# aliftffd/ViT-vs-Raw-IQ

Measured on AMD Instinct MI355X. Metric: IQ frames/sec training (fwd+loss+bwd+clip+AdamW), higher is better.
Workload: dtype bf16; 1 GPU; ViT-Tiny/16 224x224 C=1 19cls (BASELINE configs[1]); config_id=B, per_gpu_batch=256, global_batch=256, parallelism=dp1, hipgraph=True

## Files before the change

### include/iqvit.h

```cpp
#ifndef IQVIT_H
#define IQVIT_H
#include <stddef.h>
#include <stdint.h>

#ifdef __cplusplus
extern "C" {
#endif

typedef void* iq_stream_t;

enum { IQ_STATUS_OK = 0, IQ_STATUS_ARG = 1, IQ_STATUS_UNSUPPORTED = 2, IQ_STATUS_LAUNCH = 3 };

typedef struct iq_dropout {
  uint64_t seed;
  uint32_t step;
  uint32_t site;
  float p;
  const uint32_t* step_dev;
} iq_dropout_t;

int iq_ln_supported(int D);
int iq_ln_fwd(const void* z, const float* gamma, const float* beta, void* x, float* mean, float* rstd, int M, int D,
              float eps, iq_stream_t stream);
size_t iq_ln_bwd_ws_bytes(int D);
int iq_ln_bwd(const void* dx, const void* z, const float* mean, const float* rstd, const float* gamma, void* dz,
              void* dy, const iq_dropout_t* drop, float* dgamma, float* dbeta, float* ws, int accumulate, int M,
              int D, iq_stream_t stream);
int iq_ln_bwd_partial_rows(int M, int D);

typedef struct iq_epilogue {
  const float* bias;
  int relu;
  const float* pe;
  int tok, seq, cls_off;
  iq_dropout_t drop;
  const void* gate;
  int ldg;
  float gate_scale;
  const void* residual;
  int ldr;
} iq_epilogue_t;
int iq_gemm_bf16_nt(const void* A, int lda, const void* B, int ldb, void* C, int ldc, int M, int N, int K,
                    const iq_epilogue_t* epi, iq_stream_t stream);

int iq_gemm_ln_supported(int D, int K);
int iq_gemm_bf16_ln(const void* A, int lda, const void* W, int ldw, const float* bias, const void* residual, int ldr,
                    const iq_dropout_t* drop, const float* gamma, const float* beta, float eps, void* Z, void* X,
                    float* mean, float* rstd, int M, int D, int K, iq_stream_t stream);

int iq_gemm_lnbwd_supported(int D, int K);
int iq_gemm_lnbwd_partial_rows(int M);
int iq_gemm_bf16_lnbwd(const void* A, int lda, const void* Wt, int ldw, const void* residual, int ldr, const void* z,
                       const float* mean, const float* rstd, const float* gamma, const iq_dropout_t* drop, void* dz,
                       void* dy, float* partial, int M, int D, int K, iq_stream_t stream);

int iq_ffn_chain_supported(int S, int D, int F);
int iq_ffn_chain_bwd_partial_rows(int M);
size_t iq_ffn_chain_gate_bytes(int M, int F);
int iq_ffn_chain_bwd(const void* dO, const void* W2t, const void* gate_bits, float gate_scale, void* gH, const void* W1t,
                     const void* residual, const void* z1, const float* mean, const float* rstd, const float* gamma,
                     const iq_dropout_t* drop, void* dz, void* dy, float* partial, const void* Wot, void* dA, int frames, int S,
                     int D, int F, iq_stream_t stream);
int iq_qkv_dgrad_ffn_chain_bwd(const void* gQKV, const void* Wqkv_t, const void* residual0, const void* z2, const float* mean2,
                               const float* rstd2, const float* gamma2, const iq_dropout_t* drop2, void* dz2, void* dy2, float* partial2,
                               const void* W2t, const void* gate_bits, float gate_scale, void* gH, const void* W1t, const void* residual,
                               const void* z1, const float* mean, const float* rstd, const float* gamma, const iq_dropout_t* drop, void* dz,
                               void* dy, float* partial, const void* Wot, void* dA, int frames, int S, int D, int F, iq_stream_t stream);
int iq_ffn_chain_fwd(const void* X1, const void* W1, const float* b1, const iq_dropout_t* drop1, void* H, const void* W2,
                     const float* b2, const iq_dropout_t* drop2, const float* gamma, const float* beta, float eps, void* Z,
                     void* X, float* mean, float* rstd, void* gate_bits, int frames, int S, int D, int F, iq_stream_t stream);
int iq_attn_out_ffn_chain_fwd(const void* A, const void* Wo, const float* bo, const iq_dropout_t* drop0, const void* R,
                              const float* gamma1, const float* beta1, void* Z1, void* X1, float* mean1, float* rstd1,
                              const void* W1, const float* b1, const iq_dropout_t* drop1, void* H, const void* W2, const float* b2,
                              const iq_dropout_t* drop2, const float* gamma2, const float* beta2, float eps, void* Z2, void* X,
                              float* mean2, float* rstd2, void* gate_bits, const void* Wq, const float* bq, void* Yq, int frames,
                              int S, int D, int F, iq_stream_t stream);

size_t iq_wgrad_ws_bytes(int M, int N, int K);
int iq_gemm_bf16_wgrad(const void* dY, int ldy, const void* X, int ldx, float* dW, float* dbias, int M, int N, int K,
                       float* ws, size_t ws_bytes, int accumulate, iq_stream_t stream);

typedef struct iq_wgrad_problem {
  const void* dY;
  int ldy;
  const void* X;
  int ldx;
  float* dW;
  float* dbias;
  int N, K;
} iq_wgrad_problem_t;
typedef struct iq_reduce_seg {
  const float* partials;
  int rows;
  int64_t row_stride;
  float* out;
  int64_t n;
} iq_reduce_seg_t;
size_t iq_wgrad_grouped_ws_bytes(const iq_wgrad_problem_t* probs, int nprob, int M, int max_workgroups);
int iq_gemm_bf16_wgrad_grouped(const iq_wgrad_problem_t* probs, int nprob, int M, float* ws, size_t ws_bytes,
                               int accumulate, int max_workgroups, const iq_reduce_seg_t* extra, int nextra,
                               iq_stream_t stream);

int iq_attn_supported(int S, int dh);
int iq_attn_fwd(const void* qkv, void* out, float* lse, int B, int S, int H, int dh, iq_stream_t stream);
int iq_attn_bwd(const void* qkv, const void* out, const void* dout, const float* lse, void* dqkv, int B, int S, int H,
                int dh, iq_stream_t stream);
int iq_attn_fwd_masked(const void* qkv, void* out, float* lse, const uint8_t* mask, long mask_hstride, int B, int S,
                       int H, int dh, iq_stream_t stream);
int iq_attn_bwd_masked(const void* qkv, const void* out, const void* dout, const float* lse, void* dqkv,
                       const uint8_t* mask, long mask_hstride, int B, int S, int H, int dh, iq_stream_t stream);
int iq_attn_probs(const void* qkv, const float* lse, float* out, long out_bstride, int B, int S, int H, int dh,
                  int rows, int heads, iq_stream_t stream);
int iq_attn_grad_probs(const void* qkv, const float* lse, const void* dout, float* out, long out_bstride, int B, int S,
                       int H, int dh, int rows, int heads, int positive, iq_stream_t stream);
int iq_attn_relevance_step(const void* qkv, const float* lse, const void* dout, const float* r_in, float* r_out, int B,
                           int S, int H, int dh, iq_stream_t stream);

int iq_frames_preprocess(const float* raw, float* out, int n_frames, int len, int take, const float* stats,
                         iq_stream_t stream);
int iq_patchify(const float* src, void* patches, int kind, int B, int C, int H, int W, int p, int Kpad,
                iq_stream_t stream);
int iq_cls_rows(const float* cls, const float* pe, void* x0, int B, int S, int D, const iq_dropout_t* drop,
                iq_stream_t stream);
int iq_embed_bwd_gather(const void* dx0, void* demb, float* dcls, int B, int S, int tok, int D, int has_cls,
                        const iq_dropout_t* drop, int accumulate, iq_stream_t stream);
int iq_embed_dgrad(const void* demb, const void* w_bf16, int Kpad, float* dsrc, int kind, int B, int C, int H, int W, int p,
                   int D, iq_stream_t stream);
int iq_linf_step(float* x_adv, const float* grad, const float* x0, float alpha, float eps, float lo, float hi, size_t n,
                 iq_stream_t stream);

int iq_head_fwd(const void* x, const float* ln_g, const float* ln_b, const float* W, const float* b, float* featn,
                float* hstat, float* logits, int B, int S, int D, int K, int pool, iq_stream_t stream);
int iq_ce_fwd_bwd(const float* logits, const int64_t* labels, int B, int K, float smoothing, float denom,
                  float* loss_sum, int32_t* n_correct, float* dlogits, iq_stream_t stream);
int iq_head_bwd(const float* dlogits, const float* featn, const float* hstat, const float* ln_g, const float* ln_b,
                const float* W, float* dW, float* db, float* dln_g, float* dln_b, void* dx, int B, int S, int D, int K,
                int pool, int accumulate, iq_stream_t stream);

size_t iq_gradnorm_ws_bytes(size_t n);
int iq_gradnorm_sq(const float* g, size_t n, float grad_scale, float* ws, float* out, iq_stream_t stream);
int iq_adamw_step(float* p, const float* g, float* m, float* v, void* shadow_bf16, size_t n, float lr, float beta1,
                  float beta2, float eps, float weight_decay, int step, const float* gnorm_sq, float max_norm,
                  float grad_scale, const float* dyn, iq_stream_t stream);
int iq_counter_add(uint32_t* ctr_u32, uint32_t inc_u32, float* ctr_f32, float inc_f32, iq_stream_t stream);
int iq_cast_bf16(const float* src, void* dst, size_t n, iq_stream_t stream);
int iq_transpose_cast_bf16(const float* src, void* dst, int rows, int cols, iq_stream_t stream);

typedef struct iq_model_cfg {
  int kind;
  int in_channels;
  int img_h, img_w, patch;
  int seq_length, conv_k, use_cls;
  int num_classes, d_model, n_head, n_layers, ffn_hidden;
  float drop_prob;
} iq_model_cfg_t;

typedef struct iq_model iq_model_t;

int iq_model_create(const iq_model_cfg_t* cfg, iq_model_t** out);
void iq_model_destroy(iq_model_t* m);
const char* iq_model_last_error(const iq_model_t* m);
int iq_model_tokens(const iq_model_t* m);
size_t iq_model_param_floats(const iq_model_t* m);
int iq_model_param_entries(const iq_model_t* m);
int iq_model_param_entry(const iq_model_t* m, int i, char* name, int name_cap, size_t* offset, int* ndim, int* dims);
size_t iq_model_shadow_bytes(const iq_model_t* m);
size_t iq_model_workspace_bytes(const iq_model_t* m, int batch, int training);
int iq_model_bind(iq_model_t* m, float* params, float* grads, const float* pe, void* shadow);
int iq_model_bind_step_counter(iq_model_t* m, uint32_t* counter);
int iq_model_refresh_shadow(iq_model_t* m, iq_stream_t stream);
int iq_model_refresh_transposed(iq_model_t* m, iq_stream_t stream);
int iq_model_forward(iq_model_t* m, const float* src, int batch, void* workspace, size_t ws_bytes, int training,
                     uint64_t seed, uint32_t step, float* enc_out, float* logits, iq_stream_t stream);
int iq_model_backward(iq_model_t* m, const float* dlogits, const float* denc, int batch, void* workspace,
                      size_t ws_bytes, int accumulate, int stage_hi, int stage_lo, iq_stream_t stream);
int iq_model_grad_range(const iq_model_t* m, int stage_hi, int stage_lo, size_t* off, size_t* len);
#define IQ_BWD_PARAM_GRADS 1
int iq_model_backward_input(iq_model_t* m, const float* dlogits, const float* denc, int batch, void* workspace,
                            size_t ws_bytes, float* dsrc, int flags, iq_stream_t stream);
int iq_model_attention(iq_model_t* m, const void* workspace, size_t ws_bytes, int batch, int layer, int rows,
                       int heads, float* out, long out_bstride, iq_stream_t stream);
int iq_model_attention_rollout(iq_model_t* m, const void* workspace, size_t ws_bytes, int batch, float alpha,
                               float* out, iq_stream_t stream);
int iq_model_attention_relevance(iq_model_t* m, const float* dlogits, int batch, void* workspace, size_t ws_bytes,
                                 float* rel, float* const* maps, int rows, int heads, int positive, long out_bstride,
                                 iq_stream_t stream);

#define IQ_PROF_FAMILIES 8
int iq_prof_enable(int on);
int iq_prof_collect(double* ms, long long* count);
size_t iq_prof_kernels(char* out, size_t cap, int reset);

#ifdef __cplusplus
}
#endif
#endif
```

### vit-vs-raw-iq_amd/_native.py

```python
from __future__ import annotations

import ctypes as C
import os

_HERE = os.path.dirname(os.path.abspath(__file__))
LIB_PATH = os.environ.get("IQ_LIBIQVIT") or os.path.join(_HERE, "libiqvit.so")

BWD_PARAM_GRADS = 1

STATUS = {0: "ok", 1: "invalid argument", 2: "unsupported shape/configuration", 3: "HIP launch error"}


class IqError(RuntimeError):
    pass


class Dropout(C.Structure):
    _fields_ = [("seed", C.c_uint64), ("step", C.c_uint32), ("site", C.c_uint32), ("p", C.c_float),
                ("step_dev", C.c_void_p)]


class Epilogue(C.Structure):
    _fields_ = [("bias", C.c_void_p), ("relu", C.c_int), ("pe", C.c_void_p), ("tok", C.c_int), ("seq", C.c_int),
                ("cls_off", C.c_int), ("drop", Dropout), ("gate", C.c_void_p), ("ldg", C.c_int),
                ("gate_scale", C.c_float), ("residual", C.c_void_p), ("ldr", C.c_int)]


class WgradProblem(C.Structure):
    _fields_ = [("dY", C.c_void_p), ("ldy", C.c_int), ("X", C.c_void_p), ("ldx", C.c_int), ("dW", C.c_void_p),
                ("dbias", C.c_void_p), ("N", C.c_int), ("K", C.c_int)]


class ReduceSeg(C.Structure):
    _fields_ = [("partials", C.c_void_p), ("rows", C.c_int), ("row_stride", C.c_int64), ("out", C.c_void_p),
                ("n", C.c_int64)]


class ModelCfg(C.Structure):
    _fields_ = [("kind", C.c_int), ("in_channels", C.c_int), ("img_h", C.c_int), ("img_w", C.c_int),
                ("patch", C.c_int), ("seq_length", C.c_int), ("conv_k", C.c_int), ("use_cls", C.c_int),
                ("num_classes", C.c_int), ("d_model", C.c_int), ("n_head", C.c_int), ("n_layers", C.c_int),
                ("ffn_hidden", C.c_int), ("drop_prob", C.c_float)]


_P, _I, _Z, _F = C.c_void_p, C.c_int, C.c_size_t, C.c_float
_U64, _U32 = C.c_uint64, C.c_uint32

SIGNATURES = {
    "iq_ln_supported": (_I, [_I]),
    "iq_ln_fwd": (_I, [_P, _P, _P, _P, _P, _P, _I, _I, _F, _P]),
    "iq_ln_bwd_ws_bytes": (_Z, [_I]),
    "iq_ln_bwd_partial_rows": (_I, [_I, _I]),
    "iq_ln_bwd": (_I, [_P, _P, _P, _P, _P, _P, _P, C.POINTER(Dropout), _P, _P, _P, _I, _I, _I, _P]),
    "iq_gemm_bf16_nt": (_I, [_P, _I, _P, _I, _P, _I, _I, _I, _I, C.POINTER(Epilogue), _P]),
    "iq_gemm_ln_supported": (_I, [_I, _I]),
    "iq_gemm_bf16_ln": (_I, [_P, _I, _P, _I, _P, _P, _I, C.POINTER(Dropout), _P, _P, _F, _P, _P, _P, _P, _I, _I, _I, _P]),
    "iq_gemm_lnbwd_supported": (_I, [_I, _I]),
    "iq_gemm_lnbwd_partial_rows": (_I, [_I]),
    "iq_gemm_bf16_lnbwd": (_I, [_P, _I, _P, _I, _P, _I, _P, _P, _P, _P, C.POINTER(Dropout), _P, _P, _P, _I, _I, _I, _P]),
    "iq_ffn_chain_supported": (_I, [_I, _I, _I]),
    "iq_ffn_chain_bwd_partial_rows": (_I, [_I]),
    "iq_ffn_chain_bwd": (_I, [_P, _P, _P, _F, _P, _P, _P, _P, _P, _P, _P, C.POINTER(Dropout), _P, _P, _P, _P, _P, _I, _I, _I, _I, _P]),
    "iq_qkv_dgrad_ffn_chain_bwd": (_I, [_P, _P, _P, _P, _P, _P, _P, C.POINTER(Dropout), _P, _P, _P,
                                        _P, _P, _F, _P, _P, _P, _P, _P, _P, _P, C.POINTER(Dropout), _P, _P, _P, _P, _P, _I, _I, _I, _I, _P]),
    "iq_ffn_chain_gate_bytes": (_Z, [_I, _I]),
    "iq_ffn_chain_fwd": (_I, [_P, _P, _P, C.POINTER(Dropout), _P, _P, _P, C.POINTER(Dropout), _P, _P, _F, _P, _P, _P, _P, _P, _I, _I,
                              _I, _I, _P]),
    "iq_attn_out_ffn_chain_fwd": (_I, [_P, _P, _P, C.POINTER(Dropout), _P, _P, _P, _P, _P, _P, _P,
                                       _P, _P, C.POINTER(Dropout), _P, _P, _P, C.POINTER(Dropout), _P, _P, _F, _P, _P, _P, _P, _P,
                                       _P, _P, _P, _I, _I, _I, _I, _P]),
    "iq_wgrad_ws_bytes": (_Z, [_I, _I, _I]),
    "iq_gemm_bf16_wgrad": (_I, [_P, _I, _P, _I, _P, _P, _I, _I, _I, _P, _Z, _I, _P]),
    "iq_wgrad_grouped_ws_bytes": (_Z, [_P, _I, _I, _I]),
    "iq_gemm_bf16_wgrad_grouped": (_I, [_P, _I, _I, _P, _Z, _I, _I, _P, _I, _P]),
    "iq_attn_supported": (_I, [_I, _I]),
    "iq_attn_fwd": (_I, [_P, _P, _P, _I, _I, _I, _I, _P]),
    "iq_attn_bwd": (_I, [_P, _P, _P, _P, _P, _I, _I, _I, _I, _P]),
    "iq_attn_fwd_masked": (_I, [_P, _P, _P, _P, C.c_long, _I, _I, _I, _I, _P]),
    "iq_attn_bwd_masked": (_I, [_P, _P, _P, _P, _P, _P, C.c_long, _I, _I, _I, _I, _P]),
    "iq_attn_probs": (_I, [_P, _P, _P, C.c_long, _I, _I, _I, _I, _I, _I, _P]),
    "iq_attn_grad_probs": (_I, [_P, _P, _P, _P, C.c_long, _I, _I, _I, _I, _I, _I, _I, _P]),
    "iq_attn_relevance_step": (_I, [_P, _P, _P, _P, _P, _I, _I, _I, _I, _P]),
    "iq_frames_preprocess": (_I, [_P, _P, _I, _I, _I, C.POINTER(C.c_float), _P]),
    "iq_patchify": (_I, [_P, _P, _I, _I, _I, _I, _I, _I, _I, _P]),
    "iq_cls_rows": (_I, [_P, _P, _P, _I, _I, _I, C.POINTER(Dropout), _P]),
    "iq_embed_bwd_gather": (_I, [_P, _P, _P, _I, _I, _I, _I, _I, C.POINTER(Dropout), _I, _P]),
    "iq_embed_dgrad": (_I, [_P, _P, _I, _P, _I, _I, _I, _I, _I, _I, _I, _P]),
    "iq_linf_step": (_I, [_P, _P, _P, _F, _F, _F, _F, _Z, _P]),
    "iq_head_fwd": (_I, [_P, _P, _P, _P, _P, _P, _P, _P, _I, _I, _I, _I, _I, _P]),
    "iq_ce_fwd_bwd": (_I, [_P, _P, _I, _I, _F, _F, _P, _P, _P, _P]),
    "iq_head_bwd": (_I, [_P, _P, _P, _P, _P, _P, _P, _P, _P, _P, _P, _I, _I, _I, _I, _I, _I, _P]),
    "iq_gradnorm_ws_bytes": (_Z, [_Z]),
    "iq_gradnorm_sq": (_I, [_P, _Z, _F, _P, _P, _P]),
    "iq_adamw_step": (_I, [_P, _P, _P, _P, _P, _Z, _F, _F, _F, _F, _F, _I, _P, _F, _F, _P, _P]),
    "iq_counter_add": (_I, [_P, _U32, _P, _F, _P]),
    "iq_cast_bf16": (_I, [_P, _P, _Z, _P]),
    "iq_transpose_cast_bf16": (_I, [_P, _P, _I, _I, _P]),
    "iq_model_create": (_I, [C.POINTER(ModelCfg), C.POINTER(_P)]),
    "iq_model_destroy": (None, [_P]),
    "iq_model_last_error": (C.c_char_p, [_P]),
    "iq_model_tokens": (_I, [_P]),
    "iq_model_param_floats": (_Z, [_P]),
    "iq_model_param_entries": (_I, [_P]),
    "iq_model_param_entry": (_I, [_P, _I, C.c_char_p, _I, C.POINTER(_Z), C.POINTER(_I), C.POINTER(_I)]),
    "iq_model_shadow_bytes": (_Z, [_P]),
    "iq_model_workspace_bytes": (_Z, [_P, _I, _I]),
    "iq_model_bind": (_I, [_P, _P, _P, _P, _P]),
    "iq_model_bind_step_counter": (_I, [_P, _P]),
    "iq_model_refresh_shadow": (_I, [_P, _P]),
    "iq_model_refresh_transposed": (_I, [_P, _P]),
    "iq_model_forward": (_I, [_P, _P, _I, _P, _Z, _I, _U64, _U32, _P, _P, _P]),
    "iq_model_backward": (_I, [_P, _P, _P, _I, _P, _Z, _I, _I, _I, _P]),
    "iq_model_grad_range": (_I, [_P, _I, _I, C.POINTER(_Z), C.POINTER(_Z)]),
    "iq_model_backward_input": (_I, [_P, _P, _P, _I, _P, _Z, _P, _I, _P]),
    "iq_model_attention": (_I, [_P, _P, _Z, _I, _I, _I, _I, _P, C.c_long, _P]),
    "iq_model_attention_rollout": (_I, [_P, _P, _Z, _I, _F, _P, _P]),
    "iq_model_attention_relevance": (_I, [_P, _P, _I, _P, _Z, _P, C.POINTER(_P), _I, _I, _I, C.c_long, _P]),
    "iq_prof_enable": (_I, [_I]),
    "iq_prof_collect": (_I, [C.POINTER(C.c_double), C.POINTER(C.c_longlong)]),
    "iq_prof_kernels": (_Z, [C.c_char_p, _Z, _I]),
}

_lib = None


def lib():
    global _lib
    if _lib is None:
        if not os.path.exists(LIB_PATH):
            raise IqError(
                f"{LIB_PATH} not found: the HIP extension is not built. Run "
                "`python -c 'import __graft_entry__ as g; g.build()'` (or `make -C vit-vs-raw-iq_amd/csrc`). "
                "There is no CPU fallback.")
        L = C.CDLL(LIB_PATH)
        for name, (res, args) in SIGNATURES.items():
            fn = getattr(L, name)
            fn.restype = res
            fn.argtypes = args
        _lib = L
    return _lib


def check(rc, what, model=None):
    if rc != 0:
        detail = ""
        if model is not None:
            msg = lib().iq_model_last_error(model)
            if msg:
                detail = ": " + msg.decode()
        raise IqError(f"{what} failed: {STATUS.get(rc, rc)}{detail}")


def ptr(t):
    return None if t is None else t.data_ptr()


def stream_handle():
    import torch
    return torch.cuda.current_stream().cuda_stream
```

### vit-vs-raw-iq_amd/csrc/common.h

```cpp
#pragma once
#include <hip/hip_runtime.h>
#include <stdint.h>

typedef __bf16 bf16;
typedef __attribute__((ext_vector_type(8))) __bf16 bf16x8;
typedef __attribute__((ext_vector_type(4))) __bf16 bf16x4;
typedef __attribute__((ext_vector_type(4))) short s16x4;
typedef __attribute__((ext_vector_type(8))) short s16x8;
typedef __attribute__((ext_vector_type(4))) float f32x4;
typedef __attribute__((ext_vector_type(4))) uint32_t u32x4;

#define IQ_OK 0
#define IQ_ERR_ARG 1
#define IQ_ERR_UNSUPPORTED 2
#define IQ_ERR_LAUNCH 3

#define IQ_WAVE 64

static inline int iq_launch_status() {
  hipError_t e = hipGetLastError();
  return e == hipSuccess ? IQ_OK : IQ_ERR_LAUNCH;
}

__device__ __forceinline__ float bf2f(bf16 v) { return (float)v; }
__device__ __forceinline__ bf16 f2bf(float v) { return (bf16)v; }

__device__ __forceinline__ void unpack8(const bf16x8& v, float* f) {
#pragma unroll
  for (int i = 0; i < 8; ++i) f[i] = (float)v[i];
}
__device__ __forceinline__ bf16x8 pack8(const float* f) {
  bf16x8 v;
#pragma unroll
  for (int i = 0; i < 8; ++i) v[i] = (bf16)f[i];
  return v;
}

struct IqRng {
  uint64_t seed;
  uint32_t step;
  uint32_t site;
  const uint32_t* step_dev;
};

__device__ __forceinline__ IqRng rng_resolve(IqRng r) {
  if (r.step_dev) r.step = *r.step_dev;
  return r;
}

#ifndef IQ_PHILOX_ROUNDS
#define IQ_PHILOX_ROUNDS 7
#endif
__device__ __forceinline__ u32x4 philox4x32(uint32_t c0, uint32_t c1, uint32_t c2, uint32_t c3,
                                            uint32_t k0, uint32_t k1) {
  const uint32_t M0 = 0xD2511F53u, M1 = 0xCD9E8D57u, W0 = 0x9E3779B9u, W1 = 0xBB67AE85u;
#pragma unroll
  for (int r = 0; r < IQ_PHILOX_ROUNDS; ++r) {
    const uint64_t p0 = (uint64_t)M0 * (uint64_t)c0;
    const uint64_t p1 = (uint64_t)M1 * (uint64_t)c2;
    const uint32_t n0 = (uint32_t)(p1 >> 32) ^ c1 ^ k0, n1 = (uint32_t)p1;
    const uint32_t n2 = (uint32_t)(p0 >> 32) ^ c3 ^ k1, n3 = (uint32_t)p0;
    c0 = n0; c1 = n1; c2 = n2; c3 = n3;
    k0 += W0; k1 += W1;
  }
  u32x4 o = {c0, c1, c2, c3};
  return o;
}

__device__ __forceinline__ uint32_t dropout_keep8(const IqRng& r, uint64_t group, uint32_t thresh) {
  u32x4 b = philox4x32((uint32_t)group, (uint32_t)(group >> 32), r.site, r.step,
                          (uint32_t)r.seed, (uint32_t)(r.seed >> 32));
  uint32_t m = 0;
#pragma unroll
  for (int i = 0; i < 4; ++i) {
    m |= ((b[i] & 0xFFFFu) >= thresh ? 1u : 0u) << (2 * i);
    m |= ((b[i] >> 16) >= thresh ? 1u : 0u) << (2 * i + 1);
  }
  return m;
}

__host__ __device__ inline uint32_t dropout_thresh(float p) {
  float t = p * 65536.0f + 0.5f;
  if (t < 0.f) t = 0.f;
  if (t > 65535.f) t = 65535.f;
  return (uint32_t)t;
}
__host__ __device__ inline float dropout_scale(float p) {
  uint32_t t = dropout_thresh(p);
  return 65536.0f / (65536.0f - (float)t);
}

__device__ __forceinline__ int xcd_remap(int bid, int nwg) {
  const int NX = 8;
  int q = nwg / NX, r = nwg % NX;
  int xcd = bid % NX, idx = bid / NX;
  int base = (xcd < r) ? xcd * (q + 1) : r * (q + 1) + (xcd - r) * q;
  return base + idx;
}

__device__ __forceinline__ float wave_sum(float v) {
#pragma unroll
  for (int o = 32; o > 0; o >>= 1) v += __shfl_xor(v, o, 64);
  return v;
}
__device__ __forceinline__ float wave_max(float v) {
#pragma unroll
  for (int o = 32; o > 0; o >>= 1) v = fmaxf(v, __shfl_xor(v, o, 64));
  return v;
}
```

### vit-vs-raw-iq_amd/csrc/misc.hip

```cpp
#include "common.h"
#include "iqvit.h"
#include "prof.h"

namespace {

__global__ void patchify_kernel(const float* __restrict__ src, bf16* __restrict__ dst, int kind, int B, int C, int H,
                                int W, int p, int tok, int P, int Kpad) {
  const long nchunk = (long)B * tok * (Kpad / 8);
  for (long id = (long)blockIdx.x * blockDim.x + threadIdx.x; id < nchunk; id += (long)gridDim.x * blockDim.x) {
    const int ch = (int)(id % (Kpad / 8));
    const long row = id / (Kpad / 8);
    const int b = (int)(row / tok), t = (int)(row % tok);
    float v[8];
    if (kind == 0 && (p & 7) == 0 && (W & 3) == 0 && ch * 8 < P) {
      const int k = ch * 8, gw = W / p;
      const int c = k / (p * p), rem = k % (p * p), py = rem / p, px = rem % p;
      const int gy = t / gw, gx = t % gw;
      const float* sp = src + (((long)b * C + c) * H + gy * p + py) * W + gx * p + px;
      const f32x4 a = *reinterpret_cast<const f32x4*>(sp), bq = *reinterpret_cast<const f32x4*>(sp + 4);
      v[0] = a[0]; v[1] = a[1]; v[2] = a[2]; v[3] = a[3]; v[4] = bq[0]; v[5] = bq[1]; v[6] = bq[2]; v[7] = bq[3];
      *reinterpret_cast<bf16x8*>(dst + row * Kpad + ch * 8) = pack8(v);
      continue;
    }
#pragma unroll
    for (int e = 0; e < 8; ++e) {
      const int k = ch * 8 + e;
      float x = 0.f;
      if (k < P) {
        if (kind == 0) {
          const int gw = W / p;
          const int c = k / (p * p), rem = k % (p * p), py = rem / p, px = rem % p;
          const int gy = t / gw, gx = t % gw;
          x = src[(((long)b * C + c) * H + gy * p + py) * W + gx * p + px];
        } else {
          const int c = k / p, j = k % p;
          x = src[((long)b * C + c) * H + (long)t * p + j];
        }
      }
      v[e] = x;
    }
    *reinterpret_cast<bf16x8*>(dst + row * Kpad + ch * 8) = pack8(v);
  }
}

__global__ void cls_rows_kernel(const float* __restrict__ cls, const float* __restrict__ pe, bf16* __restrict__ x0,
                                int B, int S, int D, int drop_on, IqRng rng, uint32_t thresh, float dscale) {
  const int nch = D / 8;
  const int id = blockIdx.x * blockDim.x + threadIdx.x;
  if (id >= B * nch) return;
  if (drop_on) rng = rng_resolve(rng);
  const int b = id / nch, ch = id % nch;
  float v[8];
#pragma unroll
  for (int e = 0; e < 8; ++e) v[e] = cls[ch * 8 + e] + pe[ch * 8 + e];
  const long off = (long)b * S * D + ch * 8;
  if (drop_on) {
    const uint32_t keep = dropout_keep8(rng, (uint64_t)off >> 3, thresh);
#pragma unroll
    for (int e = 0; e < 8; ++e) v[e] = ((keep >> e) & 1u) ? v[e] * dscale : 0.f;
  }
  *reinterpret_cast<bf16x8*>(x0 + off) = pack8(v);
}

__global__ void embed_bwd_gather_kernel(const bf16* __restrict__ dx0, bf16* __restrict__ demb, int B, int S, int tok,
                                        int D, int cls_off, int drop_on, IqRng rng, uint32_t thresh, float dscale) {
  const int nch = D / 8;
  const long n = (long)B * tok * nch;
  if (drop_on) rng = rng_resolve(rng);
  for (long id = (long)blockIdx.x * blockDim.x + threadIdx.x; id < n; id += (long)gridDim.x * blockDim.x) {
    const int ch = (int)(id % nch);
    const long row = id / nch;
    const int b = (int)(row / tok), t = (int)(row % tok);
    const long off = ((long)b * S + cls_off + t) * D + ch * 8;
    bf16x8 v = *reinterpret_cast<const bf16x8*>(dx0 + off);
    if (drop_on) {
      const uint32_t keep = dropout_keep8(rng, (uint64_t)off >> 3, thresh);
      float f[8];
      unpack8(v, f);
#pragma unroll
      for (int e = 0; e < 8; ++e) f[e] = ((keep >> e) & 1u) ? f[e] * dscale : 0.f;
      v = pack8(f);
    }
    *reinterpret_cast<bf16x8*>(demb + row * D + ch * 8) = v;
  }
}

__global__ __launch_bounds__(256) void dcls_kernel(const bf16* __restrict__ dx0, float* __restrict__ dcls, int B, int S, int D,
                                                   int drop_on, IqRng rng, uint32_t thresh, float dscale, int accumulate) {
  __shared__ float part[4][8];
  const int ch = blockIdx.x, lane = threadIdx.x & 63, wave = threadIdx.x >> 6;
  if (drop_on) rng = rng_resolve(rng);
  float s[8] = {0.f, 0.f, 0.f, 0.f, 0.f, 0.f, 0.f, 0.f};
  for (int b = threadIdx.x; b < B; b += 256) {
    const long off = (long)b * S * D + ch * 8;
    float v[8];
    unpack8(*reinterpret_cast<const bf16x8*>(dx0 + off), v);
    uint32_t keep = 0xffu;
    if (drop_on) keep = dropout_keep8(rng, (uint64_t)off >> 3, thresh);
#pragma unroll
    for (int e = 0; e < 8; ++e) s[e] += ((keep >> e) & 1u) ? (drop_on ? v[e] * dscale : v[e]) : 0.f;
  }
#pragma unroll
  for (int e = 0; e < 8; ++e) {
    const float t = wave_sum(s[e]);
    if (lane == 0) part[wave][e] = t;
  }
  __syncthreads();
  if (threadIdx.x < 8) {
    const float t = part[0][threadIdx.x] + part[1][threadIdx.x] + part[2][threadIdx.x] + part[3][threadIdx.x];
    float* dst = dcls + ch * 8 + threadIdx.x;
    *dst = accumulate ? *dst + t : t;
  }
}

__global__ __launch_bounds__(64) void head_fwd_kernel(const bf16* __restrict__ x, const float* __restrict__ ln_g,
                                                      const float* __restrict__ ln_b, const float* __restrict__ W,
                                                      const float* __restrict__ bias, float* __restrict__ feat_hat,
                                                      float* __restrict__ hstat, float* __restrict__ logits, int S,
                                                      int D, int K, int pool) {
  const int b = blockIdx.x, lane = threadIdx.x;
  const bf16* xb = x + (long)b * S * D;
  float* fh = feat_hat + (long)b * D;
  float s1 = 0.f;
  for (int d = lane; d < D; d += 64) {
    float f;
    if (pool == 0) {
      f = (float)xb[d];
    } else {
      f = 0.f;
      for (int s = 0; s < S; ++s) f += (float)xb[(long)s * D + d];
      f /= (float)S;
    }
    fh[d] = f;
    s1 += f;
  }
  if (ln_g) {
    const float mean = wave_sum(s1) / (float)D;
    float s2 = 0.f;
    for (int d = lane; d < D; d += 64) { const float c = fh[d] - mean; s2 += c * c; }
    const float rstd = 1.0f / sqrtf(wave_sum(s2) / (float)D + 1e-5f);
    for (int d = lane; d < D; d += 64) fh[d] = (fh[d] - mean) * rstd;
    if (lane == 0) { hstat[2 * b] = mean; hstat[2 * b + 1] = rstd; }
  }
  __syncthreads();
  if (D % 4 == 0 && D <= 1024) {
    __shared__ float fs[1024];
    for (int d = lane; d < D; d += 64) fs[d] = ln_g ? ln_g[d] * fh[d] + ln_b[d] : fh[d];
    __syncthreads();
    int lpk = 64;
    while (lpk * 4 > D) lpk >>= 1;
    if (lpk >= 1) {
      const int kpar = 64 / lpk, kk = lane / lpk, dl = lane % lpk;
      for (int k0 = 0; k0 < K; k0 += kpar * 4) {
        float a[4] = {0.f, 0.f, 0.f, 0.f};
#pragma unroll
        for (int u = 0; u < 4; ++u) {
          const int k = min(k0 + u * kpar + kk, K - 1);
          for (int d = 4 * dl; d < D; d += 4 * lpk) {
            const f32x4 w = *reinterpret_cast<const f32x4*>(W + (long)k * D + d);
            const f32x4 f = *reinterpret_cast<const f32x4*>(fs + d);
            a[u] += w[0] * f[0] + w[1] * f[1] + w[2] * f[2] + w[3] * f[3];
          }
        }
#pragma unroll
        for (int u = 0; u < 4; ++u) {
          float t = a[u];
          for (int o = lpk >> 1; o > 0; o >>= 1) t += __shfl_xor(t, o, 64);
          const int k = k0 + u * kpar + kk;
          if (dl == 0 && k < K) logits[(long)b * K + k] = t + bias[k];
        }
      }
      return;
    }
  }
  for (int k = 0; k < K; ++k) {
    float a = 0.f;
    for (int d = lane; d < D; d += 64) {
      const float f = ln_g ? ln_g[d] * fh[d] + ln_b[d] : fh[d];
      a += f * W[(long)k * D + d];
    }
    a = wave_sum(a);
    if (lane == 0) logits[(long)b * K + k] = a + bias[k];
  }
}

template <int KMAX>
__global__ __launch_bounds__(256) void ce_kernel(const float* __restrict__ logits, const int64_t* __restrict__ labels,
                                                 int B, int K, float smoothing, float denom,
                                                 float* __restrict__ loss_sum, int32_t* __restrict__ n_correct,
                                                 float* __restrict__ dlogits) {
  __shared__ float sl[256];
  __shared__ int sc[256];
  float lacc = 0.f;
  int cacc = 0;
  for (int b = threadIdx.x; b < B; b += blockDim.x) {
    const float* z = logits + (long)b * K;
    const int y = (int)labels[b];
    const bool y_ok = y >= 0 && y < K;
    if constexpr (KMAX > 0) {
      float zr[KMAX];
#pragma unroll
      for (int k = 0; k < KMAX; ++k) zr[k] = k < K ? z[k] : -3.0e38f;
      float mx = zr[0];
      int am = 0;
#pragma unroll
      for (int k = 1; k < KMAX; ++k)
        if (zr[k] > mx) { mx = zr[k]; am = k; }
      float se = 0.f, sz = 0.f, zy = 0.f;
      float ek[KMAX];
#pragma unroll
      for (int k = 0; k < KMAX; ++k) {
        ek[k] = k < K ? expf(zr[k] - mx) : 0.f;
        se += ek[k];
        sz += k < K ? zr[k] : 0.f;
        zy = k == y ? zr[k] : zy;
      }
      const float lse = mx + logf(se);
      const float sum_logp = sz - (float)K * lse;
      const float nll = y_ok ? -(zy - lse) : __builtin_nanf("");
      lacc += (1.0f - smoothing) * nll + smoothing * (-sum_logp / (float)K);
      cacc += (am == y) ? 1 : 0;
      if (dlogits) {
        const float inv = 1.0f / se;
#pragma unroll
        for (int k = 0; k < KMAX; ++k) {
          if (k < K) {
            const float tgt = (k == y ? 1.0f - smoothing : 0.f) + smoothing / (float)K;
            dlogits[(long)b * K + k] = y_ok ? (ek[k] * inv - tgt) / denom : __builtin_nanf("");
          }
        }
      }
    } else {
      float mx = z[0];
      int am = 0;
      for (int k = 1; k < K; ++k)
        if (z[k] > mx) { mx = z[k]; am = k; }
      float se = 0.f;
      for (int k = 0; k < K; ++k) se += expf(z[k] - mx);
      const float lse = mx + logf(se);
      float sum_logp = 0.f;
      for (int k = 0; k < K; ++k) sum_logp += z[k] - lse;
      const float nll = y_ok ? -(z[y] - lse) : __builtin_nanf("");
      lacc += (1.0f - smoothing) * nll + smoothing * (-sum_logp / (float)K);
      cacc += (am == y) ? 1 : 0;
      if (dlogits) {
        for (int k = 0; k < K; ++k) {
          const float pk = expf(z[k] - lse);
          const float tgt = (k == y ? 1.0f - smoothing : 0.f) + smoothing / (float)K;
          dlogits[(long)b * K + k] = y_ok ? (pk - tgt) / denom : __builtin_nanf("");
        }
      }
    }
  }
  sl[threadIdx.x] = lacc;
  sc[threadIdx.x] = cacc;
  __syncthreads();
  for (int o = 128; o > 0; o >>= 1) {
    if ((int)threadIdx.x < o) { sl[threadIdx.x] += sl[threadIdx.x + o]; sc[threadIdx.x] += sc[threadIdx.x + o]; }
    __syncthreads();
  }
  if (threadIdx.x == 0) {
    if (loss_sum) *loss_sum += sl[0];
    if (n_correct) *n_correct += sc[0];
  }
}

__global__ __launch_bounds__(256) void head_bwd_dx_kernel(const float* __restrict__ dlogits, const float* __restrict__ feat_hat,
                                                         const float* __restrict__ hstat, const float* __restrict__ ln_g,
                                                         const float* __restrict__ W, bf16* __restrict__ dx, int S,
                                                         int D, int K, int pool) {
  extern __shared__ float df[];
  const int b = blockIdx.x, lane = threadIdx.x & 63;
  const float* dl = dlogits + (long)b * K;
  const float* fh = feat_hat + (long)b * D;
  if (threadIdx.x < 64) {
    float s1 = 0.f, s2 = 0.f;
    for (int d = lane; d < D; d += 64) {
      float a = 0.f;
      for (int k = 0; k < K; ++k) a += dl[k] * W[(long)k * D + d];
      if (ln_g) {
        a *= ln_g[d];
        s1 += a;
        s2 += a * fh[d];
      }
      df[d] = a;
    }
    if (ln_g) {
      const float c1 = wave_sum(s1) / (float)D, c2 = wave_sum(s2) / (float)D;
      const float rstd = hstat[2 * b + 1];
      for (int d = lane; d < D; d += 64) df[d] = rstd * (df[d] - c1 - fh[d] * c2);
    }
  }
  __syncthreads();
  bf16* dxb = dx + (long)b * S * D;
  const float inv = 1.0f / (float)S;
  for (long i = threadIdx.x; i < (long)S * (D / 8); i += 256) {
    const int s = (int)(i / (D / 8)), ch = (int)(i % (D / 8));
    float v[8];
#pragma unroll
    for (int e = 0; e < 8; ++e) v[e] = pool == 0 ? (s == 0 ? df[ch * 8 + e] : 0.f) : df[ch * 8 + e] * inv;
    *reinterpret_cast<bf16x8*>(dxb + (long)s * D + ch * 8) = pack8(v);
  }
}

__global__ __launch_bounds__(256) void head_bwd_w_kernel(const float* __restrict__ dlogits, const float* __restrict__ feat_hat,
                                                         const float* __restrict__ ln_g, const float* __restrict__ ln_b,
                                                         const float* __restrict__ W, float* __restrict__ dW, float* __restrict__ db,
                                                         float* __restrict__ dln_g, float* __restrict__ dln_b, int B, int D, int K,
                                                         int accumulate) {
  __shared__ float sa[8][33], sb[8][33];
  const int ol = threadIdx.x & 31, sl = threadIdx.x >> 5;
  const int id = blockIdx.x * 32 + ol;
  const int k = id / D, d = id % D;
  const bool live = k < K || (k == K && ln_g);
  float a = 0.f, b2 = 0.f;
  if (live) {
    if (k < K) {
      const float g = ln_g ? ln_g[d] : 1.f, be = ln_g ? ln_b[d] : 0.f;
#pragma unroll 4
      for (int b = sl; b < B; b += 8) {
        const float dl = dlogits[(long)b * K + k];
        a += dl * (g * feat_hat[(long)b * D + d] + be);
        b2 += dl;
      }
    } else {
      for (int b = sl; b < B; b += 8) {
        float dfn = 0.f;
        for (int kk = 0; kk < K; ++kk) dfn += dlogits[(long)b * K + kk] * W[(long)kk * D + d];
        a += dfn * feat_hat[(long)b * D + d];
        b2 += dfn;
      }
    }
  }
  sa[sl][ol] = a;
  sb[sl][ol] = b2;
  __syncthreads();
  if (sl == 0 && live) {
    float ta = 0.f, tb = 0.f;
#pragma unroll
    for (int i = 0; i < 8; ++i) { ta += sa[i][ol]; tb += sb[i][ol]; }
    if (k < K) {
      dW[(long)k * D + d] = accumulate ? dW[(long)k * D + d] + ta : ta;
      if (d == 0) db[k] = accumulate ? db[k] + tb : tb;
    } else {
      dln_g[d] = accumulate ? dln_g[d] + ta : ta;
      dln_b[d] = accumulate ? dln_b[d] + tb : tb;
    }
  }
}

template <int KMAX>
__global__ __launch_bounds__(256) void head_bwd_w2_kernel(const float* __restrict__ dlogits, const float* __restrict__ feat_hat,
                                                          const float* __restrict__ ln_g, const float* __restrict__ ln_b,
                                                          const float* __restrict__ W, float* __restrict__ dW, float* __restrict__ db,
                                                          float* __restrict__ dln_g, float* __restrict__ dln_b, int B, int D, int K,
                                                          int accumulate) {
  __shared__ float sT[8][KMAX][33];
  __shared__ float sS[8][KMAX];
  __shared__ float sdl[64][KMAX];
  const int ol = threadIdx.x & 31, sl = threadIdx.x >> 5;
  const int d = blockIdx.x * 32 + ol;
  const bool live = d < D;
  float T[KMAX], sd[KMAX];
#pragma unroll
  for (int k = 0; k < KMAX; ++k) { T[k] = 0.f; sd[k] = 0.f; }
  for (int b0 = 0; b0 < B; b0 += 64) {
    __syncthreads();
    for (int i = threadIdx.x; i < 64 * KMAX; i += 256) {
      const int bb = i / KMAX, k = i - bb * KMAX;
      sdl[bb][k] = (b0 + bb < B && k < K) ? dlogits[(long)(b0 + bb) * K + k] : 0.f;
    }
    __syncthreads();
    float fv[8];
#pragma unroll
    for (int i = 0; i < 8; ++i) {
      const int bb = sl + 8 * i;
      fv[i] = (live && b0 + bb < B) ? feat_hat[(long)(b0 + bb) * D + d] : 0.f;
    }
#pragma unroll
    for (int i = 0; i < 8; ++i) {
      const int bb = sl + 8 * i;
#pragma unroll
      for (int k = 0; k < KMAX; ++k) {
        const float dl = sdl[bb][k];
        T[k] += dl * fv[i];
        sd[k] += dl;
      }
    }
  }
#pragma unroll
  for (int k = 0; k < KMAX; ++k) {
    sT[sl][k][ol] = T[k];
    if (ol == 0) sS[sl][k] = sd[k];
  }
  __syncthreads();
  if (sl == 0 && live) {
    const float g = ln_g ? ln_g[d] : 1.f, be = ln_g ? ln_b[d] : 0.f;
    float lg = 0.f, lb = 0.f;
    for (int k = 0; k < K; ++k) {
      float t = 0.f, sk = 0.f;
#pragma unroll
      for (int i = 0; i < 8; ++i) { t += sT[i][k][ol]; sk += sS[i][k]; }
      const float v = g * t + be * sk;
      dW[(long)k * D + d] = accumulate ? dW[(long)k * D + d] + v : v;
      if (d == 0) db[k] = accumulate ? db[k] + sk : sk;
      const float w = W[(long)k * D + d];
      lg += w * t;
      lb += w * sk;
    }
    if (ln_g) {
      dln_g[d] = accumulate ? dln_g[d] + lg : lg;
      dln_b[d] = accumulate ? dln_b[d] + lb : lb;
    }
  }
}

constexpr int GN_BLOCKS = 1024;

__global__ __launch_bounds__(256) void gradnorm_partial_kernel(const float* __restrict__ g, size_t n, float scale,
                                                               float* __restrict__ partial) {
  __shared__ float sm[4];
  float s = 0.f;
  const size_t n4 = n / 4;
  for (size_t i = (size_t)blockIdx.x * blockDim.x + threadIdx.x; i < n4; i += (size_t)gridDim.x * blockDim.x) {
    const f32x4 v = reinterpret_cast<const f32x4*>(g)[i];
    s += v[0] * v[0] + v[1] * v[1] + v[2] * v[2] + v[3] * v[3];
  }
  if (blockIdx.x == 0 && threadIdx.x < (n & 3)) { const float v = g[n4 * 4 + threadIdx.x]; s += v * v; }
  s = wave_sum(s);
  if ((threadIdx.x & 63) == 0) sm[threadIdx.x >> 6] = s;
  __syncthreads();
  if (threadIdx.x == 0) partial[blockIdx.x] = (sm[0] + sm[1] + sm[2] + sm[3]) * scale * scale;
}
__global__ __launch_bounds__(256) void gradnorm_final_kernel(const float* __restrict__ partial, int n, float* __restrict__ out) {
  __shared__ float sm[4];
  float s = 0.f;
  for (int i = threadIdx.x; i < n; i += 256) s += partial[i];
  s = wave_sum(s);
  if ((threadIdx.x & 63) == 0) sm[threadIdx.x >> 6] = s;
  __syncthreads();
  if (threadIdx.x == 0) out[0] = sm[0] + sm[1] + sm[2] + sm[3];
}

struct AdamParams {
  float lr, b1, b2, eps, wd, max_norm, grad_scale;
  int step;
  const float* gnorm_sq;
  const float* dyn;
};

__global__ __launch_bounds__(256) void adamw_kernel(float* __restrict__ p, const float* __restrict__ g,
                                                    float* __restrict__ m, float* __restrict__ v,
                                                    bf16* __restrict__ shadow, size_t n, AdamParams a) {
  float lr = a.lr;
  int step = a.step;
  if (a.dyn) { lr = a.dyn[0]; step = (int)a.dyn[1]; }
  float coef = a.grad_scale;
  if (a.gnorm_sq && a.max_norm > 0.f) {
    const float total = sqrtf(a.gnorm_sq[0]);
    coef *= fminf(1.0f, a.max_norm / (total + 1e-6f));
  }
  const float bc1 = 1.0f - powf(a.b1, (float)step);
  const float bc2 = 1.0f - powf(a.b2, (float)step);
  const float step_size = lr / bc1, inv_sqrt_bc2 = 1.0f / sqrtf(bc2), decay = 1.0f - lr * a.wd;
  const size_t n4 = n / 4;
  for (size_t i = (size_t)blockIdx.x * blockDim.x + threadIdx.x; i < n4; i += (size_t)gridDim.x * blockDim.x) {
    f32x4 pv = reinterpret_cast<f32x4*>(p)[i];
    const f32x4 gv = reinterpret_cast<const f32x4*>(g)[i];
    f32x4 mv = reinterpret_cast<f32x4*>(m)[i];
    f32x4 vv = reinterpret_cast<f32x4*>(v)[i];
    bf16x4 sh;
#pragma unroll
    for (int e = 0; e < 4; ++e) {
      const float gg = gv[e] * coef;
      float x = pv[e] * decay;
      mv[e] = a.b1 * mv[e] + (1.0f - a.b1) * gg;
      vv[e] = a.b2 * vv[e] + (1.0f - a.b2) * gg * gg;
      const float den = sqrtf(vv[e]) * inv_sqrt_bc2 + a.eps;
      x -= step_size * (mv[e] / den);
      pv[e] = x;
      sh[e] = (bf16)x;
    }
    reinterpret_cast<f32x4*>(p)[i] = pv;
    reinterpret_cast<f32x4*>(m)[i] = mv;
    reinterpret_cast<f32x4*>(v)[i] = vv;
    if (shadow) reinterpret_cast<bf16x4*>(shadow)[i] = sh;
  }
}

__global__ void counter_add_kernel(uint32_t* cu, uint32_t iu, float* cf, float incf) {
  if (threadIdx.x == 0 && blockIdx.x == 0) {
    if (cu) *cu += iu;
    if (cf) *cf += incf;
  }
}

__global__ __launch_bounds__(256) void cast_kernel(const float* __restrict__ src, bf16* __restrict__ dst, size_t n) {
  const size_t n4 = n / 4;
  for (size_t i = (size_t)blockIdx.x * blockDim.x + threadIdx.x; i < n4; i += (size_t)gridDim.x * blockDim.x) {
    const f32x4 v = reinterpret_cast<const f32x4*>(src)[i];
    bf16x4 o;
#pragma unroll
    for (int e = 0; e < 4; ++e) o[e] = (bf16)v[e];
    reinterpret_cast<bf16x4*>(dst)[i] = o;
  }
  if (blockIdx.x == 0 && threadIdx.x < (n & 3)) dst[n4 * 4 + threadIdx.x] = (bf16)src[n4 * 4 + threadIdx.x];
}

__global__ __launch_bounds__(256) void transpose_cast_kernel(const float* __restrict__ src, bf16* __restrict__ dst,
                                                             int rows, int cols) {
  __shared__ float t[32][33];
  const int bx = blockIdx.x * 32, by = blockIdx.y * 32;
  const int tx = threadIdx.x & 31, ty = threadIdx.x >> 5;
  for (int i = ty; i < 32; i += 8) {
    const int r = by + i, c = bx + tx;
    t[i][tx] = (r < rows && c < cols) ? src[(long)r * cols + c] : 0.f;
  }
  __syncthreads();
  for (int i = ty; i < 32; i += 8) {
    const int c = bx + i, r = by + tx;
    if (c < cols && r < rows) dst[(long)c * rows + r] = (bf16)t[tx][i];
  }
}

inline int grid_for(size_t n, int per_block, int cap) {
  size_t b = (n + per_block - 1) / per_block;
  if (b > (size_t)cap) b = cap;
  if (b < 1) b = 1;
  return (int)b;
}

inline void fill_rng(const iq_dropout_t* d, int* on, IqRng* r, uint32_t* th, float* sc) {
  *on = 0; r->seed = 0; r->step = 0; r->site = 0; r->step_dev = nullptr; *th = 0; *sc = 1.f;
  if (d && d->p > 0.f) {
    *on = 1; r->seed = d->seed; r->step = d->step; r->site = d->site; r->step_dev = d->step_dev;
    *th = dropout_thresh(d->p); *sc = dropout_scale(d->p);
  }
}

}

extern "C" int iq_patchify(const float* src, void* patches, int kind, int B, int C, int H, int W, int p, int Kpad,
                           iq_stream_t stream) {
  IQ_PROF(IQ_FAM_MISC, stream);
  if (B <= 0) return IQ_OK;
  if (!src || !patches || C <= 0 || H <= 0 || p <= 0 || (Kpad % 8)) return IQ_ERR_ARG;
  int tok, P;
  if (kind == 0) {
    if (W <= 0) return IQ_ERR_ARG;
    tok = (H / p) * (W / p); P = C * p * p;
  } else if (kind == 1) {
    tok = H / p; P = C * p;
  } else {
    return IQ_ERR_ARG;
  }
  if (tok <= 0 || Kpad < P) return IQ_ERR_ARG;
  const size_t n = (size_t)B * tok * (Kpad / 8);
  patchify_kernel<<<grid_for(n, 256, 4096), 256, 0, (hipStream_t)stream>>>(src, (bf16*)patches, kind, B, C, H, W, p, tok,
                                                                          P, Kpad);
  return iq_launch_status();
}

extern "C" int iq_cls_rows(const float* cls, const float* pe, void* x0, int B, int S, int D, const iq_dropout_t* drop,
                           iq_stream_t stream) {
  IQ_PROF(IQ_FAM_MISC, stream);
  if (B <= 0) return IQ_OK;
  if (!cls || !pe || !x0 || (D % 8)) return IQ_ERR_ARG;
  int on; IqRng r; uint32_t th; float sc;
  fill_rng(drop, &on, &r, &th, &sc);
  const int n = B * (D / 8);
  cls_rows_kernel<<<(n + 255) / 256, 256, 0, (hipStream_t)stream>>>(cls, pe, (bf16*)x0, B, S, D, on, r, th, sc);
  return iq_launch_status();
}

extern "C" int iq_embed_bwd_gather(const void* dx0, void* demb, float* dcls, int B, int S, int tok, int D, int has_cls,
                                   const iq_dropout_t* drop, int accumulate, iq_stream_t stream) {
  IQ_PROF(IQ_FAM_MISC, stream);
  if (B <= 0) return IQ_OK;
  if (!dx0 || !demb || (D % 8) || (has_cls && !dcls)) return IQ_ERR_ARG;
  int on; IqRng r; uint32_t th; float sc;
  fill_rng(drop, &on, &r, &th, &sc);
  const size_t n = (size_t)B * tok * (D / 8);
  hipStream_t st = (hipStream_t)stream;
  embed_bwd_gather_kernel<<<grid_for(n, 256, 4096), 256, 0, st>>>((const bf16*)dx0, (bf16*)demb, B, S, tok, D,
                                                                  has_cls ? 1 : 0, on, r, th, sc);
  if (has_cls) dcls_kernel<<<D / 8, 256, 0, st>>>((const bf16*)dx0, dcls, B, S, D, on, r, th, sc, accumulate);
  return iq_launch_status();
}

extern "C" int iq_head_fwd(const void* x, const float* ln_g, const float* ln_b, const float* W, const float* b,
                           float* featn, float* hstat, float* logits, int B, int S, int D, int K, int pool,
                           iq_stream_t stream) {
  IQ_PROF(IQ_FAM_MISC, stream);
  if (B <= 0) return IQ_OK;
  if (!x || !W || !b || !featn || !logits || (ln_g && (!ln_b || !hstat))) return IQ_ERR_ARG;
  head_fwd_kernel<<<B, 64, 0, (hipStream_t)stream>>>((const bf16*)x, ln_g, ln_b, W, b, featn, hstat, logits, S, D, K, pool);
  return iq_launch_status();
}

extern "C" int iq_ce_fwd_bwd(const float* logits, const int64_t* labels, int B, int K, float smoothing, float denom,
                             float* loss_sum, int32_t* n_correct, float* dlogits, iq_stream_t stream) {
  IQ_PROF(IQ_FAM_MISC, stream);
  if (B <= 0) return IQ_OK;
  if (!logits || !labels || K <= 0 || denom <= 0.f) return IQ_ERR_ARG;
  if (K <= 32) ce_kernel<32><<<1, 256, 0, (hipStream_t)stream>>>(logits, labels, B, K, smoothing, denom, loss_sum, n_correct, dlogits);
  else ce_kernel<0><<<1, 256, 0, (hipStream_t)stream>>>(logits, labels, B, K, smoothing, denom, loss_sum, n_correct, dlogits);
  return iq_launch_status();
}

extern "C" int iq_head_bwd(const float* dlogits, const float* featn, const float* hstat, const float* ln_g,
                           const float* ln_b, const float* W, float* dW, float* db, float* dln_g, float* dln_b,
                           void* dx, int B, int S, int D, int K, int pool, int accumulate, iq_stream_t stream) {
  IQ_PROF(IQ_FAM_MISC, stream);
  if (B <= 0) return IQ_OK;
  if (!dlogits || !featn || !W || !dW || !db || !dx || (D % 8)) return IQ_ERR_ARG;
  if (ln_g && (!ln_b || !hstat || !dln_g || !dln_b)) return IQ_ERR_ARG;
  hipStream_t st = (hipStream_t)stream;
  head_bwd_dx_kernel<<<B, 256, D * sizeof(float), st>>>(dlogits, featn, hstat, ln_g, W, (bf16*)dx, S, D, K, pool);
  if (K <= 32) {
    head_bwd_w2_kernel<32><<<(D + 31) / 32, 256, 0, st>>>(dlogits, featn, ln_g, ln_b, W, dW, db, dln_g, dln_b, B, D, K, accumulate);
  } else {
    const int n = (K + 1) * D;
    head_bwd_w_kernel<<<(n + 31) / 32, 256, 0, st>>>(dlogits, featn, ln_g, ln_b, W, dW, db, dln_g, dln_b, B, D, K, accumulate);
  }
  return iq_launch_status();
}

extern "C" size_t iq_gradnorm_ws_bytes(size_t n) { (void)n; return GN_BLOCKS * sizeof(float); }

extern "C" int iq_gradnorm_sq(const float* g, size_t n, float grad_scale, float* ws, float* out, iq_stream_t stream) {
  IQ_PROF(IQ_FAM_OPT, stream);
  if (!g || !ws || !out || ((uintptr_t)g & 15)) return IQ_ERR_ARG;
  hipStream_t st = (hipStream_t)stream;
  const int nb = grid_for(n / 4 + 1, 256 * 4, GN_BLOCKS);
  gradnorm_partial_kernel<<<nb, 256, 0, st>>>(g, n, grad_scale, ws);
  gradnorm_final_kernel<<<1, 256, 0, st>>>(ws, nb, out);
  return iq_launch_status();
}

extern "C" int iq_adamw_step(float* p, const float* g, float* m, float* v, void* shadow_bf16, size_t n, float lr,
                             float beta1, float beta2, float eps, float weight_decay, int step, const float* gnorm_sq,
                             float max_norm, float grad_scale, const float* dyn, iq_stream_t stream) {
  IQ_PROF(IQ_FAM_OPT, stream);
  if (!p || !g || !m || !v || (n % 4)) return IQ_ERR_ARG;
  if (((uintptr_t)p | (uintptr_t)g | (uintptr_t)m | (uintptr_t)v) & 15) return IQ_ERR_ARG;
  if (step < 1 && !dyn) return IQ_ERR_ARG;
  AdamParams a = {lr, beta1, beta2, eps, weight_decay, max_norm, grad_scale, step, gnorm_sq, dyn};
  adamw_kernel<<<grid_for(n / 4, 256, 2048), 256, 0, (hipStream_t)stream>>>(p, g, m, v, (bf16*)shadow_bf16, n, a);
  return iq_launch_status();
}

extern "C" int iq_counter_add(uint32_t* ctr_u32, uint32_t inc_u32, float* ctr_f32, float inc_f32, iq_stream_t stream) {
  counter_add_kernel<<<1, 64, 0, (hipStream_t)stream>>>(ctr_u32, inc_u32, ctr_f32, inc_f32);
  return iq_launch_status();
}

extern "C" int iq_cast_bf16(const float* src, void* dst, size_t n, iq_stream_t stream) {
  IQ_PROF(IQ_FAM_MISC, stream);
  if (n == 0) return IQ_OK;
  if (!src || !dst || ((uintptr_t)src & 15) || ((uintptr_t)dst & 7)) return IQ_ERR_ARG;
  cast_kernel<<<grid_for(n / 4 + 1, 256, 2048), 256, 0, (hipStream_t)stream>>>(src, (bf16*)dst, n);
  return iq_launch_status();
}

extern "C" int iq_transpose_cast_bf16(const float* src, void* dst, int rows, int cols, iq_stream_t stream) {
  IQ_PROF(IQ_FAM_MISC, stream);
  if (rows <= 0 || cols <= 0) return IQ_OK;
  if (!src || !dst) return IQ_ERR_ARG;
  dim3 grid((cols + 31) / 32, (rows + 31) / 32);
  transpose_cast_kernel<<<grid, 256, 0, (hipStream_t)stream>>>(src, (bf16*)dst, rows, cols);
  return iq_launch_status();
}

__global__ __launch_bounds__(256) void frames_preprocess_kernel(const float* __restrict__ raw, float* __restrict__ out, long n_samp,
                                                                int len, int take, float i_mean, float i_std, float q_mean,
                                                                float q_std) {
  for (long id = (long)blockIdx.x * blockDim.x + threadIdx.x; id < n_samp; id += (long)gridDim.x * blockDim.x) {
    const long f = id / take;
    const int t = (int)(id - f * take);
    const float2 v = *reinterpret_cast<const float2*>(raw + (f * len + t) * 2);
    out[f * 2 * take + t] = (v.x - i_mean) / i_std;
    out[f * 2 * take + take + t] = (v.y - q_mean) / q_std;
  }
}

extern "C" int iq_frames_preprocess(const float* raw, float* out, int n_frames, int len, int take, const float* stats,
                                    iq_stream_t stream) {
  if (n_frames <= 0) return IQ_OK;
  if (!raw || !out || !stats || len <= 0 || take <= 0 || take > len) return IQ_ERR_ARG;
  if (!(stats[1] > 0.f) || !(stats[3] > 0.f)) return IQ_ERR_ARG;
  if ((uintptr_t)raw & 7) return IQ_ERR_ARG;
  hipStream_t st = (hipStream_t)stream;
  IQ_PROF(IQ_FAM_MISC, st);
  const long n = (long)n_frames * take;
  long nb = (n + 255) / 256;
  if (nb > 8192) nb = 8192;
  frames_preprocess_kernel<<<(int)nb, 256, 0, st>>>(raw, out, n, len, take, stats[0], stats[1], stats[2], stats[3]);
  return iq_launch_status();
}

int head_bwd_dx_launch(const float* dlogits, const float* featn, const float* hstat, const float* ln_g, const float* W, void* dx,
                       int B, int S, int D, int K, int pool, hipStream_t st) {
  IQ_PROF(IQ_FAM_MISC, st);
  if (B <= 0) return IQ_OK;
  head_bwd_dx_kernel<<<B, 256, D * sizeof(float), st>>>(dlogits, featn, hstat, ln_g, W, (bf16*)dx, S, D, K, pool);
  return iq_launch_status();
}

int embed_bwd_gather_launch(const void* dx0, void* demb, int B, int S, int tok, int D, int has_cls, const iq_dropout_t* drop,
                            hipStream_t st) {
  IQ_PROF(IQ_FAM_MISC, st);
  if (B <= 0) return IQ_OK;
  int on; IqRng r; uint32_t th; float sc;
  fill_rng(drop, &on, &r, &th, &sc);
  const size_t n = (size_t)B * tok * (D / 8);
  embed_bwd_gather_kernel<<<grid_for(n, 256, 4096), 256, 0, st>>>((const bf16*)dx0, (bf16*)demb, B, S, tok, D, has_cls ? 1 : 0,
                                                                  on, r, th, sc);
  return iq_launch_status();
}

__global__ __launch_bounds__(256) void linf_step_kernel(float* __restrict__ x, const float* __restrict__ g, const float* __restrict__ x0,
                                                        float alpha, float eps, float lo, float hi, int has_lo, int has_hi, long n) {
  for (long i = (long)blockIdx.x * blockDim.x + threadIdx.x; i < n; i += (long)gridDim.x * blockDim.x) {
    const float gv = g[i];
    const float s = gv > 0.f ? 1.f : gv < 0.f ? -1.f : 0.f;
    float v = __fadd_rn(x[i], __fmul_rn(alpha, s));
    const float c = x0[i];
    v = fminf(fmaxf(v, __fsub_rn(c, eps)), __fadd_rn(c, eps));
    if (has_lo) v = fmaxf(v, lo);
    if (has_hi) v = fminf(v, hi);
    x[i] = v;
  }
}

extern "C" int iq_linf_step(float* x_adv, const float* grad, const float* x0, float alpha, float eps, float lo, float hi, size_t n,
                            iq_stream_t stream) {
  if (!x_adv || !grad || !x0) return IQ_ERR_ARG;
  if (!(alpha >= 0.f) || !(eps >= 0.f) || !(alpha < INFINITY) || !(eps < INFINITY)) return IQ_ERR_ARG;
  const bool has_lo = lo == lo, has_hi = hi == hi;
  if (has_lo && has_hi && lo > hi) return IQ_ERR_ARG;
  if (n == 0) return IQ_OK;
  hipStream_t st = (hipStream_t)stream;
  IQ_PROF(IQ_FAM_MISC, st);
  linf_step_kernel<<<grid_for(n, 256, 8192), 256, 0, st>>>(x_adv, grad, x0, alpha, eps, lo, hi, has_lo ? 1 : 0, has_hi ? 1 : 0,
                                                           (long)n);
  return iq_launch_status();
}
```

### vit-vs-raw-iq_amd/csrc/model.hip

```cpp
#include <hip/hip_runtime.h>
#include <stdio.h>
#include <stdlib.h>
#include <string.h>

#include <string>
#include <vector>

#include "attn_maps.h"
#include "common.h"
#include "iqvit.h"
#include "prof.h"

int head_bwd_dx_launch(const float* dlogits, const float* featn, const float* hstat, const float* ln_g, const float* W, void* dx,
                       int B, int S, int D, int K, int pool, hipStream_t st);
int embed_bwd_gather_launch(const void* dx0, void* demb, int B, int S, int tok, int D, int has_cls, const iq_dropout_t* drop,
                            hipStream_t st);

namespace {

struct Entry {
  std::string name;
  size_t off;
  int ndim;
  int dims[4];
};

struct LayerOff {
  size_t wqkv, bqkv, wo, bo, g1, be1, w1, b1, w2, b2, g2, be2, end;
  size_t t_wqkv, t_wo, t_w1, t_w2;
};

inline size_t align_up(size_t v, size_t a) { return (v + a - 1) / a * a; }

struct WsPlan {
  size_t step_ctr, patches, x0, head_feat, head_stat;
  struct L { size_t qkv, att, lse, z1, mean1, rstd1, x1, hid, gate, z2, mean2, rstd2, x2; };
  std::vector<L> layers;
  size_t gA, gB, gAtt, demb, wgrad_ws, wgrad_ws_bytes, ln_part[2], embw_scratch;
  size_t gZ, gY, gZ1, gY1, gH, gQKV;
  size_t total;
};

__global__ void bf16_to_f32_kernel(const bf16* __restrict__ s, float* __restrict__ d, size_t n8) {
  for (size_t i = (size_t)blockIdx.x * blockDim.x + threadIdx.x; i < n8; i += (size_t)gridDim.x * blockDim.x) {
    const bf16x8 v = reinterpret_cast<const bf16x8*>(s)[i];
    f32x4 a = {(float)v[0], (float)v[1], (float)v[2], (float)v[3]};
    f32x4 b = {(float)v[4], (float)v[5], (float)v[6], (float)v[7]};
    reinterpret_cast<f32x4*>(d)[2 * i] = a;
    reinterpret_cast<f32x4*>(d)[2 * i + 1] = b;
  }
}
__global__ void f32_into_bf16_kernel(const float* __restrict__ s, bf16* __restrict__ d, size_t n8, int add) {
  for (size_t i = (size_t)blockIdx.x * blockDim.x + threadIdx.x; i < n8; i += (size_t)gridDim.x * blockDim.x) {
    const f32x4 a = reinterpret_cast<const f32x4*>(s)[2 * i], b = reinterpret_cast<const f32x4*>(s)[2 * i + 1];
    float f[8] = {a[0], a[1], a[2], a[3], b[0], b[1], b[2], b[3]};
    if (add) {
      const bf16x8 o = reinterpret_cast<const bf16x8*>(d)[i];
#pragma unroll
      for (int e = 0; e < 8; ++e) f[e] += (float)o[e];
    }
    reinterpret_cast<bf16x8*>(d)[i] = pack8(f);
  }
}
__global__ void cast_pad_kernel(const float* __restrict__ s, bf16* __restrict__ d, int rows, int cols, int ld) {
  const long n = (long)rows * ld;
  for (long i = (long)blockIdx.x * blockDim.x + threadIdx.x; i < n; i += (long)gridDim.x * blockDim.x) {
    const int r = (int)(i / ld), c = (int)(i % ld);
    d[i] = (bf16)(c < cols ? s[(long)r * cols + c] : 0.f);
  }
}
__global__ void unpad_kernel(const float* __restrict__ s, float* __restrict__ d, int rows, int cols, int ld, int add) {
  const long n = (long)rows * cols;
  for (long i = (long)blockIdx.x * blockDim.x + threadIdx.x; i < n; i += (long)gridDim.x * blockDim.x) {
    const int r = (int)(i / cols), c = (int)(i % cols);
    const float v = s[(long)r * ld + c];
    d[i] = add ? d[i] + v : v;
  }
}
struct TransDesc { unsigned long long src_off, dst_off; int rows, cols, tile0, tiles_x; };
__global__ __launch_bounds__(256) void transpose_table_kernel(const float* __restrict__ params, unsigned char* __restrict__ shadow,
                                                              const TransDesc* __restrict__ tab, int nent) {
  __shared__ float t[32][33];
  int e = 0;
  while (e + 1 < nent && (int)blockIdx.x >= tab[e + 1].tile0) ++e;
  const TransDesc d = tab[e];
  const int local = blockIdx.x - d.tile0;
  const int bx = (local % d.tiles_x) * 32, by = (local / d.tiles_x) * 32;
  const float* src = params + d.src_off;
  bf16* dst = reinterpret_cast<bf16*>(shadow + d.dst_off);
  const int tx = threadIdx.x & 31, ty = threadIdx.x >> 5;
  for (int i = ty; i < 32; i += 8) {
    const int r = by + i, c = bx + tx;
    t[i][tx] = (r < d.rows && c < d.cols) ? src[(long)r * d.cols + c] : 0.f;
  }
  __syncthreads();
  for (int i = ty; i < 32; i += 8) {
    const int c = bx + i, r = by + tx;
    if (c < d.cols && r < d.rows) dst[(long)c * d.rows + r] = (bf16)t[tx][i];
  }
}

__global__ void rel_start_kernel(float* r, int n, int S, int cls) {
  for (int i = blockIdx.x * blockDim.x + threadIdx.x; i < n; i += gridDim.x * blockDim.x) {
    const int k = i % S;
    r[i] = cls ? (k == 0 ? 1.f : 0.f) : 1.0f / S;
  }
}

struct RelHook {
  float* const* maps;
  int rows, heads, positive;
  long bstride;
  float* rel;
  float* r[2];
};

__global__ void set_u32_kernel(uint32_t* p, uint32_t v, int bump) {
  if (threadIdx.x == 0 && blockIdx.x == 0) *p = bump ? *p + 1u : v;
}

inline int blocks_for(size_t n, int cap = 4096) {
  size_t b = (n + 255) / 256;
  if (b > (size_t)cap) b = cap;
  if (b < 1) b = 1;
  return (int)b;
}

}

struct iq_model {
  iq_model_cfg_t c;
  int S, tok, has_cls, P, Ppad, dh, pool, head_ln;
  std::vector<Entry> entries;
  size_t nparam;
  size_t emb_w, emb_b, cls, emb_end;
  std::vector<LayerOff> L;
  size_t hln_g, hln_b, head_w, head_b, head_begin;
  size_t sh_flat, sh_embw, sh_table, shadow_bytes;
  std::vector<TransDesc> ttab;
  int ttiles = 0;
  const void* table_uploaded_to = nullptr;
  float* params = nullptr;
  float* grads = nullptr;
  const float* pe = nullptr;
  unsigned char* shadow = nullptr;
  std::string err;
  uint32_t* step_ctr = nullptr;
  uint64_t last_seed = 0;
  bool last_tr = false;
  bool last_train_fwd = false;
  const void* fwd_ws = nullptr;
  int fwd_batch = 0;

  iq_dropout_t bwd_site(uint32_t id, const uint32_t* step_dev, bool tr) const {
    iq_dropout_t d;
    d.seed = last_seed; d.step = 0; d.site = id; d.p = tr ? c.drop_prob : 0.f; d.step_dev = step_dev;
    return d;
  }

  size_t add(const std::string& name, std::vector<int> dims, size_t& cur, bool aligned = true) {
    if (aligned) cur = align_up(cur, 64);
    Entry e;
    e.name = name; e.off = cur; e.ndim = (int)dims.size();
    size_t n = 1;
    for (int i = 0; i < 4; ++i) { e.dims[i] = i < e.ndim ? dims[i] : 1; n *= (size_t)e.dims[i]; }
    entries.push_back(e);
    cur += n;
    return e.off;
  }
  const bf16* sh(size_t off) const { return reinterpret_cast<const bf16*>(shadow + sh_flat) + off; }
  const bf16* sht(size_t byte_off) const { return reinterpret_cast<const bf16*>(shadow + byte_off); }
};

namespace {

int fail(iq_model* m, int code, const std::string& msg) {
  if (m) m->err = msg;
  return code;
}

WsPlan plan_ws(const iq_model* m, int B) {
  WsPlan w;
  const size_t D = m->c.d_model, F = m->c.ffn_hidden, S = m->S, H = m->c.n_head;
  const size_t M = (size_t)B * S, MT = (size_t)B * m->tok;
  size_t cur = 0;
  auto take = [&](size_t bytes) { size_t o = cur; cur = align_up(cur + bytes, 256); return o; };
  w.step_ctr = take(256);
  w.patches = take(MT * m->Ppad * 2);
  w.x0 = take(M * D * 2);
  w.head_feat = take((size_t)B * D * 4);
  w.head_stat = take((size_t)B * 2 * 4);
  w.layers.resize(m->c.n_layers);
  for (auto& l : w.layers) {
    l.qkv = take(M * 3 * D * 2);
    l.att = take(M * D * 2);
    l.lse = take((size_t)B * H * S * 4);
    l.z1 = take(M * D * 2);
    l.mean1 = take(M * 4);
    l.rstd1 = take(M * 4);
    l.x1 = take(M * D * 2);
    l.hid = take(M * F * 2);
    l.gate = take(iq_ffn_chain_gate_bytes((int)M, (int)F));
    l.z2 = take(M * D * 2);
    l.mean2 = take(M * 4);
    l.rstd2 = take(M * 4);
    l.x2 = take(M * D * 2);
  }
  w.gA = take(M * D * 2);
  w.gB = take(M * D * 2);
  w.gZ = take(M * D * 2);
  w.gY = take(M * D * 2);
  w.gZ1 = take(M * D * 2);
  w.gY1 = take(M * D * 2);
  w.gH = take(M * F * 2);
  w.gQKV = take(M * 3 * D * 2);
  w.gAtt = take(M * D * 2);
  w.demb = take(MT * D * 2);
  size_t wb = 0;
  auto mx = [&](size_t v) { if (v > wb) wb = v; };
  {
    iq_wgrad_problem_t g[4];
    memset(g, 0, sizeof(g));
    g[0].N = (int)D; g[0].K = (int)F;
    g[1].N = (int)F; g[1].K = (int)D;
    g[2].N = (int)D; g[2].K = (int)D;
    g[3].N = (int)(3 * D); g[3].K = (int)D;
    mx(iq_wgrad_grouped_ws_bytes(g, 4, (int)M, 0));
    for (int k = 0; k < 4; ++k) mx(iq_wgrad_grouped_ws_bytes(g + k, 1, (int)M, 0));
  }
  mx(iq_wgrad_ws_bytes((int)MT, (int)D, m->Ppad));
  w.wgrad_ws_bytes = wb;
  w.wgrad_ws = take(wb);
  size_t ln_rows_fused = (size_t)iq_gemm_lnbwd_partial_rows((int)M);
  if ((size_t)iq_ffn_chain_bwd_partial_rows((int)M) > ln_rows_fused) ln_rows_fused = (size_t)iq_ffn_chain_bwd_partial_rows((int)M);
  ln_rows_fused *= 2 * D * sizeof(float);
  const size_t ln_bytes = ln_rows_fused > iq_ln_bwd_ws_bytes((int)D) ? ln_rows_fused : iq_ln_bwd_ws_bytes((int)D);
  for (int k = 0; k < 2; ++k) w.ln_part[k] = take(ln_bytes);
  w.embw_scratch = take((size_t)D * m->Ppad * 4 + 256);
  w.total = cur;
  return w;
}

inline bool use_fused_ln(int D, int K) { return iq_gemm_ln_supported(D, K) && (D <= 192 || K <= 256); }

inline bool use_ffn_chain(int M, int S, int D, int F) {
  static const int tune = [] { const char* e = getenv("IQ_TUNE_FFN_CHAIN"); return e ? atoi(e) : -1; }();
  static const int min_rows = [] { const char* e = getenv("IQ_TUNE_FFN_CHAIN_MIN_ROWS"); return e ? atoi(e) : 8192; }();
  if (!iq_ffn_chain_supported(S, D, F) || tune == 0) return false;
  if (tune == 1) return true;
  return M >= min_rows;
}

inline int use_chain_pre(int M) {
  static const int tune = [] { const char* e = getenv("IQ_TUNE_CHAIN_PRE"); return e ? atoi(e) : -1; }();
  return tune >= 0 ? tune : M <= 32768 ? 3 : 2;
}

#define IQ_TRY(expr, what)                                                              \
  do {                                                                                  \
    int rc_ = (expr);                                                                   \
    if (rc_ != IQ_OK) return fail(m, rc_, std::string(what) + " failed (status " + std::to_string(rc_) + ")"); \
  } while (0)

iq_dropout_t site(const iq_model* m, uint64_t seed, const uint32_t* step_dev, uint32_t id, bool training) {
  iq_dropout_t d;
  d.seed = seed; d.step = 0; d.site = id; d.p = training ? m->c.drop_prob : 0.f; d.step_dev = step_dev;
  return d;
}

}

extern "C" int iq_model_create(const iq_model_cfg_t* cfg, iq_model_t** out) {
  if (!cfg || !out) return IQ_ERR_ARG;
  *out = nullptr;
  iq_model* m = new iq_model();
  m->c = *cfg;
  const iq_model_cfg_t& c = m->c;
  auto bad = [&](const char* msg) { fprintf(stderr, "iq_model_create: %s\n", msg); delete m; return IQ_ERR_UNSUPPORTED; };
  if (c.d_model <= 0 || c.n_head <= 0 || c.n_layers < 0 || c.ffn_hidden <= 0 || c.num_classes <= 0 || c.in_channels <= 0)
    { delete m; return IQ_ERR_ARG; }
  if (c.d_model % c.n_head) return bad("d_model must be divisible by n_head");
  m->dh = c.d_model / c.n_head;
  if (m->dh != 16 && m->dh != 32 && m->dh != 64) return bad("head dim (d_model/n_head) must be 16, 32 or 64");
  if (c.ffn_hidden % 8) return bad("ffn_hidden must be a multiple of 8");
  if (!iq_ln_supported(c.d_model)) return bad("d_model not supported by the LayerNorm kernel");
  if (!(c.drop_prob >= 0.f && c.drop_prob < 1.f)) return bad("drop_prob must be in [0,1)");
  if (c.kind == 0) {
    if (c.patch <= 0 || c.img_h < c.patch || c.img_w < c.patch) return bad("bad image / patch size");
    m->tok = (c.img_h / c.patch) * (c.img_w / c.patch);
    m->has_cls = 1;
    m->P = c.in_channels * c.patch * c.patch;
    m->pool = 0;
    m->head_ln = 0;
  } else if (c.kind == 1) {
    if (c.conv_k <= 0 || c.seq_length < c.conv_k || (c.seq_length % c.conv_k)) return bad("bad seq_length / segment_size");
    m->tok = c.seq_length / c.conv_k;
    m->has_cls = c.use_cls ? 1 : 0;
    m->P = c.in_channels * c.conv_k;
    m->pool = m->has_cls ? 0 : 1;
    m->head_ln = 1;
  } else {
    delete m;
    return IQ_ERR_ARG;
  }
  m->S = m->tok + m->has_cls;
  m->Ppad = (int)align_up((size_t)m->P, 32);
  if (!iq_attn_supported(m->S, m->dh)) return bad("sequence too long for the attention backward kernel at this head dim");

  const int D = c.d_model, F = c.ffn_hidden, K = c.num_classes;
  size_t cur = 0;
  const std::string emb = c.kind == 0 ? "encoder.patch_embedding.projection" : "encoder.sequence_embedding.projection";
  if (c.kind == 0) m->emb_w = m->add(emb + ".weight", {D, c.in_channels, c.patch, c.patch}, cur);
  else m->emb_w = m->add(emb + ".weight", {D, c.in_channels, c.conv_k}, cur);
  m->emb_b = m->add(emb + ".bias", {D}, cur);
  m->cls = 0;
  if (m->has_cls) m->cls = m->add("encoder.cls_token", {1, 1, D}, cur);
  cur = align_up(cur, 64);
  m->emb_end = cur;
  m->L.resize(c.n_layers);
  for (int i = 0; i < c.n_layers; ++i) {
    LayerOff& o = m->L[i];
    const std::string p = "encoder.layers." + std::to_string(i) + ".";
    o.wqkv = m->add(p + "attention.w_q.weight", {D, D}, cur);
    m->add(p + "attention.w_k.weight", {D, D}, cur, false);
    m->add(p + "attention.w_v.weight", {D, D}, cur, false);
    o.bqkv = m->add(p + "attention.w_q.bias", {D}, cur);
    m->add(p + "attention.w_k.bias", {D}, cur, false);
    m->add(p + "attention.w_v.bias", {D}, cur, false);
    o.wo = m->add(p + "attention.w_concat.weight", {D, D}, cur);
    o.bo = m->add(p + "attention.w_concat.bias", {D}, cur);
    o.g1 = m->add(p + "norm1.gamma", {D}, cur);
    o.be1 = m->add(p + "norm1.beta", {D}, cur);
    o.w1 = m->add(p + "ffn.linear1.weight", {F, D}, cur);
    o.b1 = m->add(p + "ffn.linear1.bias", {F}, cur);
    o.w2 = m->add(p + "ffn.linear2.weight", {D, F}, cur);
    o.b2 = m->add(p + "ffn.linear2.bias", {D}, cur);
    o.g2 = m->add(p + "norm2.gamma", {D}, cur);
    o.be2 = m->add(p + "norm2.beta", {D}, cur);
    cur = align_up(cur, 64);
    o.end = cur;
  }
  m->head_begin = cur;
  m->hln_g = m->hln_b = 0;
  if (m->head_ln) {
    m->hln_g = m->add("mlp_head.0.weight", {D}, cur);
    m->hln_b = m->add("mlp_head.0.bias", {D}, cur);
    m->head_w = m->add("mlp_head.1.weight", {K, D}, cur);
    m->head_b = m->add("mlp_head.1.bias", {K}, cur);
  } else {
    m->head_w = m->add("mlp_head.weight", {K, D}, cur);
    m->head_b = m->add("mlp_head.bias", {K}, cur);
  }
  m->nparam = align_up(cur, 64);

  size_t sb = 0;
  m->sh_flat = sb; sb = align_up(sb + m->nparam * 2, 256);
  m->sh_embw = sb; sb = align_up(sb + (size_t)D * m->Ppad * 2, 256);
  for (auto& o : m->L) {
    o.t_wqkv = sb; sb = align_up(sb + (size_t)3 * D * D * 2, 256);
    o.t_wo = sb; sb = align_up(sb + (size_t)D * D * 2, 256);
    o.t_w1 = sb; sb = align_up(sb + (size_t)F * D * 2, 256);
    o.t_w2 = sb; sb = align_up(sb + (size_t)D * F * 2, 256);
  }
  for (auto& o : m->L) {
    auto push = [&](size_t src, size_t dst, int rows, int cols) {
      TransDesc d;
      d.src_off = src; d.dst_off = dst; d.rows = rows; d.cols = cols; d.tile0 = m->ttiles; d.tiles_x = (cols + 31) / 32;
      m->ttiles += d.tiles_x * ((rows + 31) / 32);
      m->ttab.push_back(d);
    };
    push(o.wqkv, o.t_wqkv, 3 * D, D);
    push(o.wo, o.t_wo, D, D);
    push(o.w1, o.t_w1, F, D);
    push(o.w2, o.t_w2, D, F);
  }
  m->sh_table = sb; sb = align_up(sb + m->ttab.size() * sizeof(TransDesc) + 64, 256);
  m->shadow_bytes = sb;
  *out = m;
  return IQ_OK;
}

extern "C" void iq_model_destroy(iq_model_t* m) {
  if (!m) return;
  delete m;
}
extern "C" const char* iq_model_last_error(const iq_model_t* m) { return m ? m->err.c_str() : "null model"; }
extern "C" int iq_model_tokens(const iq_model_t* m) { return m ? m->S : 0; }
extern "C" size_t iq_model_param_floats(const iq_model_t* m) { return m ? m->nparam : 0; }
extern "C" int iq_model_param_entries(const iq_model_t* m) { return m ? (int)m->entries.size() : 0; }
extern "C" int iq_model_param_entry(const iq_model_t* m, int i, char* name, int name_cap, size_t* offset, int* ndim,
                                    int* dims) {
  if (!m || i < 0 || i >= (int)m->entries.size() || !name || name_cap <= 0 || !offset || !ndim || !dims) return IQ_ERR_ARG;
  const Entry& e = m->entries[i];
  snprintf(name, (size_t)name_cap, "%s", e.name.c_str());
  *offset = e.off;
  *ndim = e.ndim;
  for (int k = 0; k < 4; ++k) dims[k] = e.dims[k];
  return IQ_OK;
}
extern "C" size_t iq_model_shadow_bytes(const iq_model_t* m) { return m ? m->shadow_bytes : 0; }
extern "C" size_t iq_model_workspace_bytes(const iq_model_t* m, int batch, int training) {
  (void)training;
  if (!m || batch <= 0) return 0;
  return plan_ws(m, batch).total;
}

extern "C" int iq_model_bind(iq_model_t* m, float* params, float* grads, const float* pe, void* shadow) {
  if (!m) return IQ_ERR_ARG;
  if (!params || !pe || !shadow) return fail(m, IQ_ERR_ARG, "bind: params, pe and shadow are required");
  if (((uintptr_t)params | (uintptr_t)grads | (uintptr_t)shadow) & 255) return fail(m, IQ_ERR_ARG, "bind: buffers must be 256 B aligned");
  m->params = params; m->grads = grads; m->pe = pe; m->shadow = (unsigned char*)shadow;
  if (m->table_uploaded_to != shadow && !m->ttab.empty()) {
    if (hipMemcpy(m->shadow + m->sh_table, m->ttab.data(), m->ttab.size() * sizeof(TransDesc), hipMemcpyHostToDevice) != hipSuccess)
      return fail(m, IQ_ERR_LAUNCH, "bind: uploading the transpose table failed");
    m->table_uploaded_to = shadow;
  }
  return IQ_OK;
}

extern "C" int iq_model_bind_step_counter(iq_model_t* m, uint32_t* counter) {
  if (!m) return IQ_ERR_ARG;
  if ((uintptr_t)counter & 3) return fail(m, IQ_ERR_ARG, "bind_step_counter: counter must be 4 B aligned");
  m->step_ctr = counter;
  return IQ_OK;
}

static int refresh_impl(iq_model_t* m, bool cast_flat, iq_stream_t stream) {
  if (!m || !m->params || !m->shadow) return fail(m, IQ_ERR_ARG, "refresh_shadow: model not bound");
  hipStream_t st = (hipStream_t)stream;
  const int D = m->c.d_model;
  if (cast_flat) IQ_TRY(iq_cast_bf16(m->params, m->shadow + m->sh_flat, m->nparam, stream), "cast params");
  IQ_PROF(IQ_FAM_MISC, st);
  cast_pad_kernel<<<blocks_for((size_t)D * m->Ppad), 256, 0, st>>>(m->params + m->emb_w, (bf16*)(m->shadow + m->sh_embw), D,
                                                                  m->P, m->Ppad);
  if (m->ttiles > 0)
    transpose_table_kernel<<<m->ttiles, 256, 0, st>>>(m->params, m->shadow, (const TransDesc*)(m->shadow + m->sh_table),
                                                     (int)m->ttab.size());
  return iq_launch_status();
}

extern "C" int iq_model_refresh_shadow(iq_model_t* m, iq_stream_t stream) { return refresh_impl(m, true, stream); }
extern "C" int iq_model_refresh_transposed(iq_model_t* m, iq_stream_t stream) { return refresh_impl(m, false, stream); }

extern "C" int iq_model_forward(iq_model_t* m, const float* src, int batch, void* workspace, size_t ws_bytes,
                                int training, uint64_t seed, uint32_t step, float* enc_out, float* logits,
                                iq_stream_t stream) {
  if (!m) return IQ_ERR_ARG;
  if (!m->params || !m->shadow || !m->pe) return fail(m, IQ_ERR_ARG, "forward: model not bound");
  if (!src || !workspace || batch <= 0) return fail(m, IQ_ERR_ARG, "forward: bad arguments");
  if ((uintptr_t)workspace & 255) return fail(m, IQ_ERR_ARG, "forward: workspace must be 256 B aligned");
  const WsPlan w = plan_ws(m, batch);
  if (ws_bytes < w.total) return fail(m, IQ_ERR_ARG, "forward: workspace too small");
  hipStream_t st = (hipStream_t)stream;
  unsigned char* ws = (unsigned char*)workspace;
  const iq_model_cfg_t& c = m->c;
  const int D = c.d_model, F = c.ffn_hidden, S = m->S, H = c.n_head, B = batch;
  const int M = B * S, MT = B * m->tok;
  const bool tr = training != 0 && c.drop_prob > 0.f;
  uint32_t* step_dev = m->step_ctr ? m->step_ctr : (uint32_t*)(ws + w.step_ctr);
  m->last_tr = tr;
  m->last_train_fwd = true;
  if (tr) {
    set_u32_kernel<<<1, 64, 0, st>>>(step_dev, step, step == 0xFFFFFFFFu ? 1 : 0);
    m->last_seed = seed;
  }
  const float* P = m->params;
  m->fwd_ws = nullptr;

  if (c.kind == 0) IQ_TRY(iq_patchify(src, ws + w.patches, 0, B, c.in_channels, c.img_h, c.img_w, c.patch, m->Ppad, stream), "patchify");
  else IQ_TRY(iq_patchify(src, ws + w.patches, 1, B, c.in_channels, c.seq_length, 0, c.conv_k, m->Ppad, stream), "patchify");
  const iq_dropout_t d0 = site(m, seed, step_dev, 0, tr);
  if (m->has_cls) IQ_TRY(iq_cls_rows(P + m->cls, m->pe, ws + w.x0, B, S, D, &d0, stream), "cls rows");
  {
    iq_epilogue_t e;
    memset(&e, 0, sizeof(e));
    e.bias = P + m->emb_b; e.pe = m->pe; e.tok = m->tok; e.seq = S; e.cls_off = m->has_cls; e.drop = d0;
    IQ_TRY(iq_gemm_bf16_nt(ws + w.patches, m->Ppad, m->shadow + m->sh_embw, m->Ppad, ws + w.x0, D, MT, D, m->Ppad, &e, stream),
           "embedding GEMM");
  }
  const unsigned char* x = ws + w.x0;
  bool qkv_done = false;
  for (int l = 0; l < c.n_layers; ++l) {
    const LayerOff& o = m->L[l];
    const WsPlan::L& a = w.layers[l];
    iq_epilogue_t e;
    if (!qkv_done) {
      memset(&e, 0, sizeof(e));
      e.bias = P + o.bqkv;
      IQ_TRY(iq_gemm_bf16_nt(x, D, m->sh(o.wqkv), D, ws + a.qkv, 3 * D, M, 3 * D, D, &e, stream), "qkv GEMM");
    }
    qkv_done = false;
    IQ_TRY(iq_attn_fwd(ws + a.qkv, ws + a.att, (float*)(ws + a.lse), B, S, H, m->dh, stream), "attention fwd");
    const iq_dropout_t dr1 = site(m, seed, step_dev, 1 + 3 * l, tr);
    const iq_dropout_t drh = site(m, seed, step_dev, 2 + 3 * l, tr);
    const iq_dropout_t dr2 = site(m, seed, step_dev, 3 + 3 * l, tr);
    if (use_ffn_chain(M, S, D, F) && use_chain_pre(M)) {
      const bool next = l + 1 < c.n_layers && use_chain_pre(M) >= 2;
      IQ_TRY(iq_attn_out_ffn_chain_fwd(ws + a.att, m->sh(o.wo), P + o.bo, &dr1, x, P + o.g1, P + o.be1, ws + a.z1, ws + a.x1,
                                       (float*)(ws + a.mean1), (float*)(ws + a.rstd1), m->sh(o.w1), P + o.b1, &drh, ws + a.hid,
                                       m->sh(o.w2), P + o.b2, &dr2, P + o.g2, P + o.be2, 1e-12f, ws + a.z2, ws + a.x2,
                                       (float*)(ws + a.mean2), (float*)(ws + a.rstd2), ws + a.gate,
                                       next ? m->sh(m->L[l + 1].wqkv) : nullptr, next ? P + m->L[l + 1].bqkv : nullptr,
                                       next ? ws + w.layers[l + 1].qkv : nullptr, B, S, D, F, stream),
             "out-proj + norm1 + ffn chain + norm2 (+ next q,k,v)");
      qkv_done = next;
      x = ws + a.x2;
      continue;
    }
    if (use_fused_ln(D, D)) {
      IQ_TRY(iq_gemm_bf16_ln(ws + a.att, D, m->sh(o.wo), D, P + o.bo, x, D, &dr1, P + o.g1, P + o.be1, 1e-12f, ws + a.z1,
                             ws + a.x1, (float*)(ws + a.mean1), (float*)(ws + a.rstd1), M, D, D, stream), "out-proj GEMM + norm1");
    } else {
      memset(&e, 0, sizeof(e));
      e.bias = P + o.bo; e.drop = dr1; e.residual = x; e.ldr = D;
      IQ_TRY(iq_gemm_bf16_nt(ws + a.att, D, m->sh(o.wo), D, ws + a.z1, D, M, D, D, &e, stream), "out-proj GEMM");
      IQ_TRY(iq_ln_fwd(ws + a.z1, P + o.g1, P + o.be1, ws + a.x1, (float*)(ws + a.mean1), (float*)(ws + a.rstd1), M, D, 1e-12f, stream), "norm1");
    }
    if (use_ffn_chain(M, S, D, F)) {
      IQ_TRY(iq_ffn_chain_fwd(ws + a.x1, m->sh(o.w1), P + o.b1, &drh, ws + a.hid, m->sh(o.w2), P + o.b2, &dr2, P + o.g2, P + o.be2,
                              1e-12f, ws + a.z2, ws + a.x2, (float*)(ws + a.mean2), (float*)(ws + a.rstd2), ws + a.gate, B, S, D, F, stream),
             "ffn chain + norm2");
    } else {
      memset(&e, 0, sizeof(e));
      e.bias = P + o.b1; e.relu = 1; e.drop = drh;
      IQ_TRY(iq_gemm_bf16_nt(ws + a.x1, D, m->sh(o.w1), D, ws + a.hid, F, M, F, D, &e, stream), "ffn1 GEMM");
      if (use_fused_ln(D, F)) {
        IQ_TRY(iq_gemm_bf16_ln(ws + a.hid, F, m->sh(o.w2), F, P + o.b2, ws + a.x1, D, &dr2, P + o.g2, P + o.be2, 1e-12f,
                               ws + a.z2, ws + a.x2, (float*)(ws + a.mean2), (float*)(ws + a.rstd2), M, D, F, stream), "ffn2 GEMM + norm2");
      } else {
        memset(&e, 0, sizeof(e));
        e.bias = P + o.b2; e.drop = dr2; e.residual = ws + a.x1; e.ldr = D;
        IQ_TRY(iq_gemm_bf16_nt(ws + a.hid, F, m->sh(o.w2), F, ws + a.z2, D, M, D, F, &e, stream), "ffn2 GEMM");
        IQ_TRY(iq_ln_fwd(ws + a.z2, P + o.g2, P + o.be2, ws + a.x2, (float*)(ws + a.mean2), (float*)(ws + a.rstd2), M, D, 1e-12f, stream), "norm2");
      }
    }
    x = ws + a.x2;
  }
  if (logits) {
    IQ_TRY(iq_head_fwd(x, m->head_ln ? P + m->hln_g : nullptr, m->head_ln ? P + m->hln_b : nullptr, P + m->head_w,
                       P + m->head_b, (float*)(ws + w.head_feat), (float*)(ws + w.head_stat), logits, B, S, D,
                       c.num_classes, m->pool, stream), "head");
  }
  if (enc_out) bf16_to_f32_kernel<<<blocks_for((size_t)M * D / 8), 256, 0, st>>>((const bf16*)x, enc_out, (size_t)M * D / 8);
  const int rc = iq_launch_status();
  if (rc == IQ_OK) { m->fwd_ws = workspace; m->fwd_batch = batch; }
  return rc;
}

static int maps_check(iq_model_t* m, const void* workspace, size_t ws_bytes, int batch, const char* what, WsPlan* w) {
  if (!workspace || batch <= 0) return fail(m, IQ_ERR_ARG, std::string(what) + ": bad arguments");
  if (!m->fwd_ws) return fail(m, IQ_ERR_ARG, std::string(what) + ": no forward has run in a workspace");
  if (m->fwd_ws != workspace) return fail(m, IQ_ERR_ARG, std::string(what) + ": the last forward ran in another workspace");
  if (m->fwd_batch != batch)
    return fail(m, IQ_ERR_ARG, std::string(what) + ": the last forward in this workspace had batch " + std::to_string(m->fwd_batch) +
                                   ", not " + std::to_string(batch));
  *w = plan_ws(m, batch);
  if (ws_bytes < w->total) return fail(m, IQ_ERR_ARG, std::string(what) + ": workspace too small");
  return IQ_OK;
}

extern "C" int iq_model_attention(iq_model_t* m, const void* workspace, size_t ws_bytes, int batch, int layer, int rows,
                                  int heads, float* out, long out_bstride, iq_stream_t stream) {
  if (!m) return IQ_ERR_ARG;
  WsPlan w;
  const int rc = maps_check(m, workspace, ws_bytes, batch, "attention", &w);
  if (rc != IQ_OK) return rc;
  if (layer < 0 || layer >= m->c.n_layers) return fail(m, IQ_ERR_ARG, "attention: layer index out of range");
  if (rows < 0 || rows > 2 || heads < 0 || heads > 1) return fail(m, IQ_ERR_ARG, "attention: rows must be 0, 1 or 2 and heads 0 or 1");
  if (!out) return fail(m, IQ_ERR_ARG, "attention: out is NULL");
  const int S = m->S, H = m->c.n_head;
  if (out_bstride < (long)(heads ? 1 : H) * S * (rows == 0 ? S : 1)) return fail(m, IQ_ERR_ARG, "attention: out_bstride too small");
  const unsigned char* ws = (const unsigned char*)workspace;
  const WsPlan::L& a = w.layers[layer];
  IQ_TRY(iq_attn_probs(ws + a.qkv, (const float*)(ws + a.lse), out, out_bstride, batch, S, H, m->dh, rows, heads, stream),
         "attention probabilities");
  return IQ_OK;
}

extern "C" int iq_model_attention_rollout(iq_model_t* m, const void* workspace, size_t ws_bytes, int batch, float alpha,
                                          float* out, iq_stream_t stream) {
  if (!m) return IQ_ERR_ARG;
  WsPlan w;
  const int rc = maps_check(m, workspace, ws_bytes, batch, "attention rollout", &w);
  if (rc != IQ_OK) return rc;
  if (!(alpha >= 0.f && alpha <= 1.f)) return fail(m, IQ_ERR_ARG, "attention rollout: alpha must be in [0, 1]");
  if (!out) return fail(m, IQ_ERR_ARG, "attention rollout: out is NULL");
  const unsigned char* ws = (const unsigned char*)workspace;
  const int L = m->c.n_layers;
  const long qs = L > 1 ? (long)(w.layers[1].qkv - w.layers[0].qkv) : 0, ls = L > 1 ? (long)(w.layers[1].lse - w.layers[0].lse) : 0;
  for (int l = 0; l < L; ++l)
    if ((long)(w.layers[l].qkv - w.layers[0].qkv) != l * qs || (long)(w.layers[l].lse - w.layers[0].lse) != l * ls)
      return fail(m, IQ_ERR_UNSUPPORTED, "attention rollout: workspace layers are not evenly spaced");
  const size_t q0 = L ? w.layers[0].qkv : 0, l0 = L ? w.layers[0].lse : 0;
  IQ_TRY(attn_rollout_launch(ws + q0, qs, ws + l0, ls, L, out, batch, m->S, m->c.n_head, m->dh, m->has_cls, alpha,
                             (hipStream_t)stream),
         "attention rollout");
  return IQ_OK;
}

extern "C" int iq_model_grad_range(const iq_model_t* m, int stage_hi, int stage_lo, size_t* off, size_t* len) {
  if (!m || !off || !len) return IQ_ERR_ARG;
  const int Lr = m->c.n_layers;
  if (stage_lo < 0 || stage_hi > Lr + 1 || stage_lo > stage_hi) return IQ_ERR_ARG;
  auto begin = [&](int s) { return s == 0 ? (size_t)0 : (s <= Lr ? (s == 1 ? m->emb_end : m->L[s - 2].end) : m->head_begin); };
  auto end = [&](int s) { return s == 0 ? m->emb_end : (s <= Lr ? m->L[s - 1].end : m->nparam); };
  *off = begin(stage_lo);
  *len = end(stage_hi) - *off;
  return IQ_OK;
}

static int backward_impl(iq_model_t* m, const float* dlogits, const float* denc, int batch, void* workspace, size_t ws_bytes,
                         int accumulate, int stage_hi, int stage_lo, bool pgrads, iq_stream_t stream,
                         const RelHook* rh = nullptr) {
  if (!m->params || (pgrads && !m->grads) || !m->shadow) return fail(m, IQ_ERR_ARG, "backward: model not bound (grads required)");
  if (!workspace || batch <= 0) return fail(m, IQ_ERR_ARG, "backward: bad arguments");
  const iq_model_cfg_t& c = m->c;
  const int Lr = c.n_layers;
  if (stage_lo < 0 || stage_hi > Lr + 1 || stage_lo > stage_hi) return fail(m, IQ_ERR_ARG, "backward: bad stage range");
  const WsPlan w = plan_ws(m, batch);
  if (ws_bytes < w.total) return fail(m, IQ_ERR_ARG, "backward: workspace too small");
  hipStream_t st = (hipStream_t)stream;
  unsigned char* ws = (unsigned char*)workspace;
  const int D = c.d_model, F = c.ffn_hidden, S = m->S, H = c.n_head, B = batch, K = c.num_classes;
  const int M = B * S, MT = B * m->tok;
  const bool tr = m->last_tr;
  const uint32_t* step_dev = m->step_ctr ? m->step_ctr : (const uint32_t*)(ws + w.step_ctr);
  const float* P = m->params;
  float* G = m->grads;
  float* wws = (float*)(ws + w.wgrad_ws);
  const float dscale = tr ? dropout_scale(c.drop_prob) : 1.f;

  if (stage_hi == Lr + 1) {
    if (!dlogits && !denc) return fail(m, IQ_ERR_ARG, "backward: dlogits or denc required at the head stage");
    if (dlogits && !pgrads) {
      IQ_TRY(head_bwd_dx_launch(dlogits, (const float*)(ws + w.head_feat), (const float*)(ws + w.head_stat),
                                m->head_ln ? P + m->hln_g : nullptr, P + m->head_w, ws + w.gA, B, S, D, K, m->pool, st), "head bwd (dx)");
    } else if (dlogits) {
      IQ_TRY(iq_head_bwd(dlogits, (const float*)(ws + w.head_feat), (const float*)(ws + w.head_stat),
                         m->head_ln ? P + m->hln_g : nullptr, m->head_ln ? P + m->hln_b : nullptr, P + m->head_w,
                         G + m->head_w, G + m->head_b, m->head_ln ? G + m->hln_g : nullptr,
                         m->head_ln ? G + m->hln_b : nullptr, ws + w.gA, B, S, D, K, m->pool, accumulate, stream), "head bwd");
    } else if (!accumulate && pgrads) {
      (void)hipMemsetAsync(G + m->head_begin, 0, (m->nparam - m->head_begin) * sizeof(float), st);
    }
    if (denc) f32_into_bf16_kernel<<<blocks_for((size_t)M * D / 8), 256, 0, st>>>(denc, (bf16*)(ws + w.gA), (size_t)M * D / 8, dlogits ? 1 : 0);
  }
  const bool fuse1 = iq_gemm_lnbwd_supported(D, F) != 0, fuse2 = iq_gemm_lnbwd_supported(D, 3 * D) != 0;
  bool deferred = false;
  for (int sidx = (stage_hi > Lr ? Lr : stage_hi); sidx >= 1 && sidx >= stage_lo; --sidx) {
    const int l = sidx - 1;
    const LayerOff& o = m->L[l];
    const WsPlan::L& a = w.layers[l];
    const unsigned char* xin = l == 0 ? ws + w.x0 : ws + w.layers[l - 1].x2;
    unsigned char *gZ = ws + w.gZ, *gY = ws + w.gY, *gZ1 = ws + w.gZ1, *gY1 = ws + w.gY1;
    unsigned char *gH = ws + w.gH, *gQKV = ws + w.gQKV;
    iq_epilogue_t e;
    float* lp2 = (float*)(ws + w.ln_part[0]);
    float* lp1 = (float*)(ws + w.ln_part[1]);
    const bool norm2_here = l == Lr - 1 || !fuse2;
    if (norm2_here) {
      const iq_dropout_t dr2 = m->bwd_site(3 + 3 * l, step_dev, tr);
      IQ_TRY(iq_ln_bwd(ws + w.gA, ws + a.z2, (const float*)(ws + a.mean2), (const float*)(ws + a.rstd2), P + o.g2,
                       gZ, gY, &dr2, nullptr, nullptr, lp2, accumulate, M, D, stream), "norm2 bwd");
    }
    const unsigned char* dO2 = tr ? gY : gZ;
    const unsigned char* dAo = tr ? gY1 : gZ1;
    const iq_wgrad_problem_t wg[4] = {
        {dO2, D, ws + a.hid, F, G + o.w2, G + o.b2, D, F},
        {gH, F, ws + a.x1, D, G + o.w1, G + o.b1, F, D},
        {dAo, D, ws + a.att, D, G + o.wo, G + o.bo, D, D},
        {gQKV, 3 * D, xin, D, G + o.wqkv, G + o.bqkv, 3 * D, D}};
    const int rows2 = norm2_here ? iq_ln_bwd_partial_rows(M, D) : deferred ? iq_ffn_chain_bwd_partial_rows(M) : iq_gemm_lnbwd_partial_rows(M);
    const bool chain = fuse1 && m->last_train_fwd && use_ffn_chain(M, S, D, F);
    const int rows1 = chain ? iq_ffn_chain_bwd_partial_rows(M) : fuse1 ? iq_gemm_lnbwd_partial_rows(M) : iq_ln_bwd_partial_rows(M, D);
    const iq_reduce_seg_t lnseg[4] = {{lp2, rows2, 2L * D, G + o.g2, D}, {lp2 + D, rows2, 2L * D, G + o.be2, D},
                                      {lp1, rows1, 2L * D, G + o.g1, D}, {lp1 + D, rows1, 2L * D, G + o.be1, D}};
    const iq_dropout_t dr1 = m->bwd_site(1 + 3 * l, step_dev, tr);
    const bool post = chain && use_chain_pre(M) >= 2;
    if (chain && deferred) {
      const LayerOff& ou = m->L[l + 1];
      const iq_dropout_t dr2b = m->bwd_site(3 + 3 * l, step_dev, tr);
      IQ_TRY(iq_qkv_dgrad_ffn_chain_bwd(gQKV, m->sht(ou.t_wqkv), gZ1, ws + a.z2, (const float*)(ws + a.mean2), (const float*)(ws + a.rstd2),
                                        P + o.g2, &dr2b, gZ, gY, lp2, m->sht(o.t_w2), ws + a.gate, dscale, gH, m->sht(o.t_w1), gZ, ws + a.z1,
                                        (const float*)(ws + a.mean1), (const float*)(ws + a.rstd1), P + o.g1, &dr1, gZ1, gY1, lp1,
                                        m->sht(o.t_wo), ws + w.gAtt, B, S, D, F, stream),
             "qkv dgrad of the layer above + norm2 bwd + ffn chain bwd + norm1 bwd + out-proj dgrad");
    } else if (chain) {
      IQ_TRY(iq_ffn_chain_bwd(dO2, m->sht(o.t_w2), ws + a.gate, dscale, gH, m->sht(o.t_w1), gZ, ws + a.z1, (const float*)(ws + a.mean1),
                              (const float*)(ws + a.rstd1), P + o.g1, &dr1, gZ1, gY1, lp1, post ? m->sht(o.t_wo) : nullptr,
                              post ? ws + w.gAtt : nullptr, B, S, D, F, stream), "ffn chain bwd + norm1 bwd (+ out-proj dgrad)");
    } else {
      memset(&e, 0, sizeof(e));
      e.gate = ws + a.hid; e.ldg = F; e.gate_scale = dscale;
      IQ_TRY(iq_gemm_bf16_nt(dO2, D, m->sht(o.t_w2), D, gH, F, M, F, D, &e, stream), "ffn2 dgrad");
      if (fuse1) {
        IQ_TRY(iq_gemm_bf16_lnbwd(gH, F, m->sht(o.t_w1), F, gZ, D, ws + a.z1, (const float*)(ws + a.mean1),
                                  (const float*)(ws + a.rstd1), P + o.g1, &dr1, gZ1, gY1, lp1, M, D, F, stream), "ffn1 dgrad + norm1 bwd");
      } else {
        memset(&e, 0, sizeof(e));
        e.residual = gZ; e.ldr = D;
        IQ_TRY(iq_gemm_bf16_nt(gH, F, m->sht(o.t_w1), F, ws + w.gB, D, M, D, F, &e, stream), "ffn1 dgrad");
        IQ_TRY(iq_ln_bwd(ws + w.gB, ws + a.z1, (const float*)(ws + a.mean1), (const float*)(ws + a.rstd1), P + o.g1,
                         gZ1, gY1, &dr1, nullptr, nullptr, lp1, accumulate, M, D, stream), "norm1 bwd");
      }
    }
    if (!post) IQ_TRY(iq_gemm_bf16_nt(dAo, D, m->sht(o.t_wo), D, ws + w.gAtt, D, M, D, D, nullptr, stream), "out-proj dgrad");
    if (rh) {
      const float* lse = (const float*)(ws + a.lse);
      if (rh->maps && rh->maps[l])
        IQ_TRY(iq_attn_grad_probs(ws + a.qkv, lse, ws + w.gAtt, rh->maps[l], rh->bstride, B, S, H, m->dh, rh->rows, rh->heads,
                                  rh->positive, stream), "gradient-weighted attention map");
      if (rh->rel) {
        const int i = Lr - 1 - l;
        IQ_TRY(attn_relevance_step_launch(ws + a.qkv, lse, ws + w.gAtt, i ? rh->r[(i - 1) & 1] : nullptr, l ? rh->r[i & 1] : rh->rel,
                                          B, S, H, m->dh, i ? 0 : m->has_cls ? 1 : 2, st), "relevance step");
      }
      if (l == 0) break;
    }
    IQ_TRY(iq_attn_bwd(ws + a.qkv, ws + a.att, ws + w.gAtt, (const float*)(ws + a.lse), gQKV, B, S, H, m->dh, stream), "attention bwd");
    if (pgrads) IQ_TRY(iq_gemm_bf16_wgrad_grouped(wg, 4, M, wws, w.wgrad_ws_bytes, accumulate, 0, lnseg, 4, stream), "layer weight gradients");
    deferred = l > 0 && fuse2 && chain && post && use_chain_pre(M) >= 3 && sidx - 1 >= stage_lo;
    if (deferred) continue;
    if (l > 0 && fuse2) {
      const LayerOff& ob = m->L[l - 1];
      const WsPlan::L& ab = w.layers[l - 1];
      const iq_dropout_t dr2b = m->bwd_site(3 + 3 * (l - 1), step_dev, tr);
      IQ_TRY(iq_gemm_bf16_lnbwd(gQKV, 3 * D, m->sht(o.t_wqkv), 3 * D, gZ1, D, ws + ab.z2, (const float*)(ws + ab.mean2),
                                (const float*)(ws + ab.rstd2), P + ob.g2, &dr2b, gZ, gY, lp2, M, D, 3 * D, stream),
             "qkv dgrad + norm2 bwd of the layer below");
    } else {
      memset(&e, 0, sizeof(e));
      e.residual = gZ1; e.ldr = D;
      IQ_TRY(iq_gemm_bf16_nt(gQKV, 3 * D, m->sht(o.t_wqkv), 3 * D, ws + w.gA, D, M, D, 3 * D, &e, stream), "qkv dgrad");
    }
  }
  if (stage_lo == 0) {
    const iq_dropout_t dr0 = m->bwd_site(0, step_dev, tr);
    if (!pgrads) {
      IQ_TRY(embed_bwd_gather_launch(ws + w.gA, ws + w.demb, B, S, m->tok, D, m->has_cls, &dr0, st), "embedding bwd gather");
      return iq_launch_status();
    }
    IQ_TRY(iq_embed_bwd_gather(ws + w.gA, ws + w.demb, m->has_cls ? G + m->cls : nullptr, B, S, m->tok, D, m->has_cls,
                               &dr0, accumulate, stream), "embedding bwd gather");
    if (m->Ppad == m->P) {
      IQ_TRY(iq_gemm_bf16_wgrad(ws + w.demb, D, ws + w.patches, m->Ppad, G + m->emb_w, G + m->emb_b, MT, D, m->Ppad, wws,
                                w.wgrad_ws_bytes, accumulate, stream), "embedding wgrad");
    } else {
      float* scratch = (float*)(ws + w.embw_scratch);
      if (accumulate) (void)hipMemsetAsync(scratch, 0, (size_t)D * m->Ppad * sizeof(float), st);
      IQ_TRY(iq_gemm_bf16_wgrad(ws + w.demb, D, ws + w.patches, m->Ppad, scratch, G + m->emb_b, MT, D, m->Ppad, wws,
                                w.wgrad_ws_bytes, accumulate, stream), "embedding wgrad");
      unpad_kernel<<<blocks_for((size_t)D * m->P), 256, 0, st>>>(scratch, G + m->emb_w, D, m->P, m->Ppad, accumulate);
    }
  }
  return iq_launch_status();
}

extern "C" int iq_model_backward(iq_model_t* m, const float* dlogits, const float* denc, int batch, void* workspace,
                                 size_t ws_bytes, int accumulate, int stage_hi, int stage_lo, iq_stream_t stream) {
  if (!m) return IQ_ERR_ARG;
  return backward_impl(m, dlogits, denc, batch, workspace, ws_bytes, accumulate, stage_hi, stage_lo, true, stream);
}

extern "C" int iq_model_backward_input(iq_model_t* m, const float* dlogits, const float* denc, int batch, void* workspace,
                                       size_t ws_bytes, float* dsrc, int flags, iq_stream_t stream) {
  if (!m) return IQ_ERR_ARG;
  if (flags & ~IQ_BWD_PARAM_GRADS) return fail(m, IQ_ERR_ARG, "backward_input: unknown flags");
  if (!dsrc) return fail(m, IQ_ERR_ARG, "backward_input: dsrc is NULL");
  if (!dlogits && !denc) return fail(m, IQ_ERR_ARG, "backward_input: dlogits or denc required");
  const bool pgrads = (flags & IQ_BWD_PARAM_GRADS) != 0;
  if (!m->params || !m->shadow || !m->pe) return fail(m, IQ_ERR_ARG, "backward_input: model not bound");
  if (pgrads && !m->grads) return fail(m, IQ_ERR_ARG, "backward_input: IQ_BWD_PARAM_GRADS needs a bound gradient buffer");
  WsPlan w;
  const int rc = maps_check(m, workspace, ws_bytes, batch, "backward_input", &w);
  if (rc != IQ_OK) return rc;
  const int rb = backward_impl(m, dlogits, denc, batch, workspace, ws_bytes, 0, m->c.n_layers + 1, 0, pgrads, stream);
  if (rb != IQ_OK) return rb;
  const iq_model_cfg_t& c = m->c;
  unsigned char* ws = (unsigned char*)workspace;
  const int kind = c.kind, H = kind == 0 ? c.img_h : c.seq_length, W = kind == 0 ? c.img_w : 0, p = kind == 0 ? c.patch : c.conv_k;
  IQ_TRY(iq_embed_dgrad(ws + w.demb, m->shadow + m->sh_embw, m->Ppad, dsrc, kind, batch, c.in_channels, H, W, p, c.d_model, stream),
         "embedding data gradient");
  return IQ_OK;
}

extern "C" int iq_model_attention_relevance(iq_model_t* m, const float* dlogits, int batch, void* workspace, size_t ws_bytes,
                                            float* rel, float* const* maps, int rows, int heads, int positive, long out_bstride,
                                            iq_stream_t stream) {
  if (!m) return IQ_ERR_ARG;
  if (!m->params || !m->shadow || !m->pe) return fail(m, IQ_ERR_ARG, "attention relevance: model not bound");
  if (!dlogits) return fail(m, IQ_ERR_ARG, "attention relevance: dlogits is NULL");
  WsPlan w;
  const int rc = maps_check(m, workspace, ws_bytes, batch, "attention relevance", &w);
  if (rc != IQ_OK) return rc;
  if (rows < 0 || rows > 2 || heads < 0 || heads > 1)
    return fail(m, IQ_ERR_ARG, "attention relevance: rows must be 0, 1 or 2 and heads 0 or 1");
  if (positive < 0 || positive > 1) return fail(m, IQ_ERR_ARG, "attention relevance: positive must be 0 or 1");
  const int L = m->c.n_layers, S = m->S, H = m->c.n_head;
  bool any_map = false;
  for (int l = 0; maps && l < L; ++l) any_map = any_map || maps[l];
  if (!rel && !any_map) return fail(m, IQ_ERR_ARG, "attention relevance: rel and every map are NULL");
  if (any_map && out_bstride < (long)(heads ? 1 : H) * S * (rows == 0 ? S : 1))
    return fail(m, IQ_ERR_ARG, "attention relevance: out_bstride too small");
  RelHook h;
  h.maps = maps; h.rows = rows; h.heads = heads; h.positive = positive; h.bstride = out_bstride; h.rel = rel;
  h.r[0] = (float*)((unsigned char*)workspace + w.demb);
  h.r[1] = h.r[0] + (size_t)batch * S;
  if (2 * (size_t)batch * S * sizeof(float) > (size_t)batch * m->tok * m->c.d_model * 2)
    return fail(m, IQ_ERR_UNSUPPORTED, "attention relevance: no room for the relevance vectors");
  if (L == 0) {
    if (rel) rel_start_kernel<<<blocks_for((size_t)batch * S), 256, 0, (hipStream_t)stream>>>(rel, batch * S, S, m->has_cls);
    return iq_launch_status() == IQ_OK ? IQ_OK : fail(m, IQ_ERR_LAUNCH, "attention relevance: start vector launch failed");
  }
  return backward_impl(m, dlogits, nullptr, batch, workspace, ws_bytes, 0, L + 1, 1, false, stream, &h);
}
```

### vit-vs-raw-iq_amd/modules.py

```python
from __future__ import annotations

import ctypes as C
import math
import weakref
from typing import Dict, Optional

import torch
from torch import nn
from torch.autograd.function import once_differentiable

from . import _native as N
from . import functional as NF


class LayerNorm(nn.Module):

    def __init__(self, d_model, eps=1e-12):
        super().__init__()
        self.gamma = nn.Parameter(torch.ones(d_model))
        self.beta = nn.Parameter(torch.zeros(d_model))
        self.eps = eps

    def forward(self, x):
        return NF.layer_norm(x, self.gamma, self.beta, self.eps)


class ScaleDotProductAttention(nn.Module):

    def forward(self, q, k, v, mask=None, e=1e-12, need_score=True):
        out = NF.attention(q, k, v, mask)
        score = NF.attention_probabilities(q, k, mask) if need_score else None
        return out, score


class MultiHeadAttention(nn.Module):

    def __init__(self, d_model, n_head):
        super().__init__()
        self.n_head = n_head
        self.attention = ScaleDotProductAttention()
        self.w_q = nn.Linear(d_model, d_model)
        self.w_k = nn.Linear(d_model, d_model)
        self.w_v = nn.Linear(d_model, d_model)
        self.w_concat = nn.Linear(d_model, d_model)

    def forward(self, q, k, v, mask=None):
        q = NF.linear(q, self.w_q.weight, self.w_q.bias)
        k = NF.linear(k, self.w_k.weight, self.w_k.bias)
        v = NF.linear(v, self.w_v.weight, self.w_v.bias)
        q, k, v = self.split(q), self.split(k), self.split(v)
        out, _ = self.attention(q, k, v, mask=mask, need_score=False)
        out = self.concat(out)
        return NF.linear(out, self.w_concat.weight, self.w_concat.bias)

    def split(self, tensor):
        batch_size, length, d_model = tensor.size()
        d_tensor = d_model // self.n_head
        return tensor.view(batch_size, length, self.n_head, d_tensor).transpose(1, 2)

    def concat(self, tensor):
        batch_size, head, length, d_tensor = tensor.size()
        return tensor.transpose(1, 2).contiguous().view(batch_size, length, head * d_tensor)


class PositionwiseFeedForward(nn.Module):

    def __init__(self, d_model, hidden, drop_prob=0.1):
        super().__init__()
        self.linear1 = nn.Linear(d_model, hidden)
        self.linear2 = nn.Linear(hidden, d_model)
        self.relu = nn.ReLU()
        self.dropout = nn.Dropout(p=drop_prob)

    def forward(self, x):
        x = NF.linear(x, self.linear1.weight, self.linear1.bias, relu=True)
        x = self.dropout(x)
        return NF.linear(x, self.linear2.weight, self.linear2.bias)


class EncoderLayer(nn.Module):

    def __init__(self, d_model, ffn_hidden, n_head, drop_prob):
        super().__init__()
        self.attention = MultiHeadAttention(d_model=d_model, n_head=n_head)
        self.norm1 = LayerNorm(d_model=d_model)
        self.dropout1 = nn.Dropout(p=drop_prob)
        self.ffn = PositionwiseFeedForward(d_model=d_model, hidden=ffn_hidden, drop_prob=drop_prob)
        self.norm2 = LayerNorm(d_model=d_model)
        self.dropout2 = nn.Dropout(p=drop_prob)

    def forward(self, x, src_mask=None):
        _x = x
        x = self.attention(q=x, k=x, v=x, mask=src_mask)
        x = self.dropout1(x)
        x = self.norm1(x + _x)
        _x = x
        x = self.ffn(x)
        x = self.dropout2(x)
        return self.norm2(x + _x)


class PatchEmbedding(nn.Module):

    def __init__(self, in_channels, patch_size, embedding_dim):
        super().__init__()
        self.projection = nn.Conv2d(in_channels, embedding_dim, kernel_size=patch_size, stride=patch_size)
        self._patch = patch_size

    def forward(self, x):
        return NF.patch_embed(x, self.projection.weight, self.projection.bias, 0, self._patch)


class SequenceEmbedding(nn.Module):

    def __init__(self, in_channels=2, embedding_dim=256, method="conv1d", segment_size=None):
        super().__init__()
        self.in_channels = in_channels
        self.embedding_dim = embedding_dim
        self.method = method
        self.segment_size = segment_size
        if method == "conv1d":
            self.projection = nn.Conv1d(in_channels, embedding_dim, kernel_size=1)
        elif method == "segment":
            if segment_size is None:
                raise ValueError("segment_size is required for 'segment' method")
            self.projection = nn.Conv1d(in_channels, embedding_dim, kernel_size=segment_size, stride=segment_size)
        else:
            raise ValueError(f"Unknown method: {method}. Use 'conv1d' or 'segment'")

    def forward(self, x):
        k = 1 if self.method == "conv1d" else self.segment_size
        return NF.patch_embed(x, self.projection.weight, self.projection.bias, 1, k)


class PositionalEncodingViT(nn.Module):

    def __init__(self, d_model, max_len=5000, device="cpu"):
        super().__init__()
        enc = torch.zeros(max_len, d_model)
        pos = torch.arange(0, max_len).float().unsqueeze(1)
        two_i = torch.arange(0, d_model, step=2).float()
        den = torch.pow(10000.0, two_i / d_model)
        enc[:, 0::2] = torch.sin(pos / den)
        enc[:, 1::2] = torch.cos(pos / den)
        self.register_buffer("encoding", enc)

    def forward(self, x):
        return x + self.encoding[: x.size(1), :].unsqueeze(0)


class PositionalEncodingRawIQ(nn.Module):

    def __init__(self, d_model, max_len=5000, device="cpu", dropout=0.0):
        super().__init__()
        enc = torch.zeros(max_len, d_model)
        position = torch.arange(0, max_len, dtype=torch.float32).unsqueeze(1)
        div_term = torch.exp(torch.arange(0, d_model, 2, dtype=torch.float32) * -(math.log(10000.0) / d_model))
        enc[:, 0::2] = torch.sin(position * div_term)
        enc[:, 1::2] = torch.cos(position * div_term)
        self.register_buffer("encoding", enc)
        self.dropout = nn.Dropout(p=dropout) if dropout > 0 else None

    def forward(self, x):
        seq_len = x.size(1)
        if seq_len > self.encoding.size(0):
            raise ValueError(f"Sequence length {seq_len} exceeds maximum length {self.encoding.size(0)}. "
                             "Increase max_len parameter.")
        x = x + self.encoding[:seq_len, :].unsqueeze(0)
        return self.dropout(x) if self.dropout is not None else x


class NativePlan:
    _count = 0

    def __init__(self, owner: nn.Module, cfg: N.ModelCfg, prefix_strip: str = ""):
        self._owner = weakref.ref(owner)
        self.cfg = cfg
        self.strip = prefix_strip
        self.L = N.lib()
        h = C.c_void_p()
        rc = self.L.iq_model_create(C.byref(cfg), C.byref(h))
        if rc != 0:
            raise N.IqError(
                "configuration not supported by the MI355X kernels "
                f"(d_model={cfg.d_model}, n_head={cfg.n_head}, ffn_hidden={cfg.ffn_hidden}): requires "
                "d_model % n_head == 0, d_model/n_head in {16,32,64}, d_model % 8 == 0, ffn_hidden % 8 == 0 and a "
                "sequence that fits the attention kernel's LDS")
        self.h = h
        self.S = self.L.iq_model_tokens(h)
        self.nparam = self.L.iq_model_param_floats(h)
        self.entries = []
        name = C.create_string_buffer(256)
        off, nd, dims = C.c_size_t(), C.c_int(), (C.c_int * 4)()
        for i in range(self.L.iq_model_param_entries(h)):
            N.check(self.L.iq_model_param_entry(h, i, name, 256, C.byref(off), C.byref(nd), dims), "param_entry")
            self.entries.append((name.value.decode(), off.value, tuple(dims[k] for k in range(nd.value))))
        self.flat: Optional[torch.Tensor] = None
        self.gflat: Optional[torch.Tensor] = None
        self.shadow: Optional[torch.Tensor] = None
        self.ws: Optional[torch.Tensor] = None
        self.ws_batch = 0
        self.shadow_version = -1
        self.generation = 0
        NativePlan._count += 1
        self.seed = (torch.initial_seed() * 0x9E3779B97F4A7C15 + NativePlan._count * 0xD1B54A32D192ED03) & ((1 << 62) - 1)
        self.step = 0
        self.step_ctr: Optional[torch.Tensor] = None
        self.ctr_value = -1
        self._probe = None

    def __deepcopy__(self, memo):
        return None

    def __reduce__(self):
        return (type(None), ())

    def __del__(self):
        try:
            if getattr(self, "h", None):
                self.L.iq_model_destroy(self.h)
                self.h = None
        except Exception:
            pass

    def _named(self) -> Dict[str, nn.Parameter]:
        owner = self._owner()
        return dict(owner.named_parameters())

    def _pe(self) -> torch.Tensor:
        owner = self._owner()
        enc = owner.encoder if hasattr(owner, "encoder") else owner
        return enc.positional_encoding.encoding

    def bind(self, device: torch.device):
        named = self._named()
        flat = torch.zeros(self.nparam, dtype=torch.float32, device=device)
        first = None
        bound = []
        with torch.no_grad():
            for name, off, shape in self.entries:
                key = name[len(self.strip):] if self.strip and name.startswith(self.strip) else name
                p = named.get(key)
                if p is None:
                    continue
                if tuple(p.shape) != shape:
                    raise N.IqError(f"parameter {key} has shape {tuple(p.shape)}, native layout expects {shape}")
                n = p.numel()
                view = flat[off:off + n].view(shape)
                view.copy_(p.data.to(device=device, dtype=torch.float32))
                p.data = view
                bound.append(p)
                if first is None:
                    first = p
        self.flat = flat
        self._probe = first
        self._bound = bound
        pe = self._pe()
        if pe.device != device or pe.dtype != torch.float32 or not pe.is_contiguous():
            raise N.IqError("positional encoding buffer must be a contiguous fp32 tensor on the model's device")
        self.shadow = torch.empty(self.L.iq_model_shadow_bytes(self.h), dtype=torch.uint8, device=device)
        self.gflat = None
        self.shadow_version = -1
        self.step_ctr = torch.zeros(1, dtype=torch.int32, device=device)
        self.ctr_value = 0
        N.check(self.L.iq_model_bind_step_counter(self.h, N.ptr(self.step_ctr)), "iq_model_bind_step_counter", self.h)
        self._bind_native(None)

    def _bind_native(self, gflat):
        N.check(self.L.iq_model_bind(self.h, N.ptr(self.flat), N.ptr(gflat), N.ptr(self._pe()), N.ptr(self.shadow)),
                "iq_model_bind", self.h)
        self.gflat = gflat

    def is_bound(self, device=None) -> bool:
        p = self._probe
        return not (self.flat is None or (device is not None and self.flat.device != device) or p is None
                    or p.data.untyped_storage().data_ptr() != self.flat.untyped_storage().data_ptr())

    def ensure(self, device: torch.device):
        if not self.is_bound(device):
            self.bind(device)
        v = 0
        for q in self._bound:
            v += q._version
        if v != self.shadow_version:
            N.check(self.L.iq_model_refresh_shadow(self.h, N.stream_handle()), "refresh_shadow", self.h)
            self.shadow_version = v

    def mark_dirty(self):
        self.shadow_version = -1

    def workspace(self, batch: int, device) -> torch.Tensor:
        need = self.L.iq_model_workspace_bytes(self.h, batch, 1)
        if self.ws is None or self.ws.numel() < need or self.ws.device != device:
            self.ws = None
            self.ws = torch.empty(need, dtype=torch.uint8, device=device)
        self.ws_batch = batch
        return self.ws

    def forward(self, src: torch.Tensor, training: bool, want_logits: bool, want_enc: bool):
        dev = src.device
        self.ensure(dev)
        B = src.shape[0]
        ws = self.workspace(B, dev)
        logits = torch.empty(B, self.cfg.num_classes, dtype=torch.float32, device=dev) if want_logits else None
        enc = torch.empty(B, self.S, self.cfg.d_model, dtype=torch.float32, device=dev) if want_enc else None
        if training:
            self.step += 1
            self.ctr_value = self.step & 0x7FFFFFFF
        self.generation += 1
        N.check(self.L.iq_model_forward(self.h, N.ptr(src), B, N.ptr(ws), ws.numel(), 1 if training else 0,
                                        self.seed, self.step & 0x7FFFFFFF, N.ptr(enc), N.ptr(logits),
                                        N.stream_handle()), "iq_model_forward", self.h)
        return logits, enc

    def backward(self, batch: int, dlogits, denc, gflat: torch.Tensor, accumulate=False, stage_hi=None, stage_lo=0):
        if gflat is not self.gflat:
            self._bind_native(gflat)
        hi = self.cfg.n_layers + 1 if stage_hi is None else stage_hi
        N.check(self.L.iq_model_backward(self.h, N.ptr(dlogits), N.ptr(denc), batch, N.ptr(self.ws), self.ws.numel(),
                                         1 if accumulate else 0, hi, stage_lo, N.stream_handle()),
                "iq_model_backward", self.h)

    def backward_input(self, batch: int, dlogits, denc, dsrc: torch.Tensor, gflat=None):
        if gflat is not None and gflat is not self.gflat:
            self._bind_native(gflat)
        N.check(self.L.iq_model_backward_input(self.h, N.ptr(dlogits), N.ptr(denc), batch, N.ptr(self.ws), self.ws.numel(),
                                               N.ptr(dsrc), N.BWD_PARAM_GRADS if gflat is not None else 0,
                                               N.stream_handle()), "iq_model_backward_input", self.h)

    def grad_range(self, stage_hi: int, stage_lo: int):
        off, ln = C.c_size_t(), C.c_size_t()
        N.check(self.L.iq_model_grad_range(self.h, stage_hi, stage_lo, C.byref(off), C.byref(ln)), "grad_range")
        return off.value, ln.value

    def grad_views(self, gflat: torch.Tensor, params_in_order):
        index = {}
        for name, off, shape in self.entries:
            key = name[len(self.strip):] if self.strip and name.startswith(self.strip) else name
            index[key] = (off, shape)
        out = []
        for name, p in params_in_order:
            off, shape = index[name]
            out.append(gflat[off:off + p.numel()].view(shape))
        return out


class _PlanFn(torch.autograd.Function):

    @staticmethod
    def forward(ctx, plan: NativePlan, src, training, want, names, *params):
        logits, enc = plan.forward(src, training, want == "logits", want == "enc")
        ctx.plan = plan
        ctx.want = want
        ctx.names = names
        ctx.batch = src.shape[0]
        ctx.generation = plan.generation
        ctx.nparams = len(params)
        ctx.src_shape = src.shape
        ctx.set_materialize_grads(False)
        return logits if want == "logits" else enc

    @staticmethod
    def backward(ctx, gout):
        if torch.is_grad_enabled():
            raise RuntimeError("the fused model's backward is not differentiable: backward(create_graph=True) / "
                               "torch.autograd.grad(..., create_graph=True) through it is not supported (no double backward)")
        return _plan_backward(ctx, gout)


@once_differentiable
def _plan_backward(ctx, gout):
    plan: NativePlan = ctx.plan
    none = (None,) * 5
    if gout is None:
        return none + (None,) * ctx.nparams
    if ctx.generation != plan.generation:
        raise RuntimeError(
            "backward() after a later forward() on the same model: the native workspace holding the saved "
            "activations has been overwritten. Call backward before running the model again.")
    gout = gout.contiguous().float()
    dl, de = (gout, None) if ctx.want == "logits" else (None, gout)
    if ctx.needs_input_grad[1]:
        dsrc = torch.empty(ctx.src_shape, dtype=torch.float32, device=gout.device)
        if not any(ctx.needs_input_grad[5:]):
            plan.backward_input(ctx.batch, dl, de, dsrc)
            return (None, dsrc) + (None,) * (3 + ctx.nparams)
        gflat = torch.empty_like(plan.flat)
        plan.backward_input(ctx.batch, dl, de, dsrc, gflat)
        named = plan._named()
        return (None, dsrc, None, None, None) + tuple(plan.grad_views(gflat, [(n, named[n]) for n in ctx.names]))
    gflat = torch.empty_like(plan.flat)
    if ctx.want == "logits":
        plan.backward(ctx.batch, gout, None, gflat)
    else:
        plan.backward(ctx.batch, None, gout, gflat)
    named = plan._named()
    grads = plan.grad_views(gflat, [(n, named[n]) for n in ctx.names])
    return none + tuple(grads)


def _check_src(src, ndim, what):
    if not isinstance(src, torch.Tensor) or src.dim() != ndim:
        raise ValueError(f"expected a {ndim}-D tensor {what}, got {tuple(src.shape) if hasattr(src, 'shape') else src}")
    if not src.is_cuda:
        raise N.IqError(
            "this framework runs on MI355X only: the input is a CPU tensor and there is no CPU fallback "
            "(the CPU restatement used for parity checks lives in oracle/ and is test infrastructure)")
    return src.contiguous().float()


class _WeakLink:

    def __init__(self, target=None):
        self._ref = weakref.ref(target) if target is not None else None

    def __call__(self):
        return self._ref() if self._ref is not None else None

    def __deepcopy__(self, memo):
        return _WeakLink()

    def __reduce__(self):
        return (_WeakLink, ())


def _link(parent):
    object.__setattr__(parent.encoder, "_parent_ref", _WeakLink(parent))


def _parent_of(encoder):
    ref = getattr(encoder, "_parent_ref", None)
    parent = ref() if ref is not None else None
    return parent if parent is not None and getattr(parent, "encoder", None) is encoder else None


def _run(plan: NativePlan, owner: nn.Module, src, want, training=None):
    training = owner.training if training is None else bool(training)
    names, params = [], []
    for n, p in owner.named_parameters():
        names.append(n)
        params.append(p)
    needs_grad = torch.is_grad_enabled() and (src.requires_grad or any(p.requires_grad for p in params))
    if needs_grad:
        plan.ensure(src.device)
        return _PlanFn.apply(plan, src, training, want, tuple(names), *params)
    logits, enc = plan.forward(src, training, want == "logits", want == "enc")
    return logits if want == "logits" else enc


class EncoderViT(nn.Module):

    def __init__(self, in_channels, img_size_h, img_size_w, patch_size, d_model, ffn_hidden, n_head, n_layers,
                 drop_prob, device):
        super().__init__()
        self.device = device
        self.patch_embedding = PatchEmbedding(in_channels=in_channels, patch_size=patch_size, embedding_dim=d_model)
        num_patches = (img_size_h // patch_size) * (img_size_w // patch_size)
        self.positional_encoding = PositionalEncodingViT(d_model=d_model, max_len=num_patches + 1, device=device)
        self.cls_token = nn.Parameter(torch.randn(1, 1, d_model))
        self.layers = nn.ModuleList([EncoderLayer(d_model=d_model, ffn_hidden=ffn_hidden, n_head=n_head,
                                                  drop_prob=drop_prob) for _ in range(n_layers)])
        self.dropout = nn.Dropout(p=drop_prob)
        self._geom = dict(kind=0, in_channels=in_channels, img_h=img_size_h, img_w=img_size_w, patch=patch_size,
                          seq_length=0, conv_k=0, use_cls=1, d_model=d_model, n_head=n_head, n_layers=n_layers,
                          ffn_hidden=ffn_hidden, drop_prob=float(drop_prob))
        self._plan: Optional[NativePlan] = None

    def _cfg(self, num_classes=1):
        return N.ModelCfg(num_classes=num_classes, **self._geom)

    def _forward_layers(self, src, src_mask):
        x = self.patch_embedding(src)
        cls = self.cls_token.repeat(x.shape[0], 1, 1)
        x = torch.cat([cls, x], dim=1)
        x = self.dropout(self.positional_encoding(x))
        for layer in self.layers:
            x = layer(x, src_mask)
        return x

    def _expect(self, src):
        g = self._geom
        src = _check_src(src, 4, "(batch, in_channels, img_size_h, img_size_w)")
        if tuple(src.shape[1:]) != (g["in_channels"], g["img_h"], g["img_w"]):
            raise RuntimeError(f"input shape {tuple(src.shape)} does not match the model geometry "
                               f"(B, {g['in_channels']}, {g['img_h']}, {g['img_w']})")
        return src

    def forward(self, src, src_mask=None):
        if src_mask is not None:
            return self._forward_layers(src, src_mask)
        src = self._expect(src)
        parent = _parent_of(self)
        if parent is not None:
            return _run(parent.native_plan(), parent, src, "enc", training=self.training)
        if self._plan is None:
            self._plan = NativePlan(self, self._cfg(), prefix_strip="encoder.")
        return _run(self._plan, self, src, "enc")


class AMCTransformerViT(nn.Module):

    def __init__(self, in_channels, img_size_h, img_size_w, patch_size, num_classes, d_model, n_head, n_layers,
                 ffn_hidden, drop_prob, device):
        super().__init__()
        self.encoder = EncoderViT(in_channels=in_channels, img_size_h=img_size_h, img_size_w=img_size_w,
                                  patch_size=patch_size, d_model=d_model, n_head=n_head, ffn_hidden=ffn_hidden,
                                  drop_prob=drop_prob, n_layers=n_layers, device=device)
        self.mlp_head = nn.Linear(d_model, num_classes)
        self._num_classes = num_classes
        self._plan: Optional[NativePlan] = None
        _link(self)

    def __setstate__(self, state):
        super().__setstate__(state)
        _link(self)

    def native_plan(self) -> NativePlan:
        if self._plan is None:
            _link(self)
            self._plan = NativePlan(self, self.encoder._cfg(self._num_classes))
        return self._plan

    def forward(self, src):
        src = self.encoder._expect(src)
        return _run(self.native_plan(), self, src, "logits")


class EncoderRawIQ(nn.Module):

    def __init__(self, in_channels, seq_length, d_model, ffn_hidden, n_head, n_layers, drop_prob, device,
                 use_cls_token=True, embedding_type="conv1d", segment_size=64):
        super().__init__()
        self.device = device
        self.use_cls_token = use_cls_token
        self.embedding_type = embedding_type
        if embedding_type == "conv1d":
            self.sequence_embedding = SequenceEmbedding(in_channels=in_channels, embedding_dim=d_model, method="conv1d")
            num_tokens = seq_length
            conv_k = 1
        elif embedding_type == "segment":
            if seq_length % segment_size != 0:
                raise ValueError(f"seq_length ({seq_length}) must be divisible by segment_size ({segment_size})")
            self.sequence_embedding = SequenceEmbedding(in_channels=in_channels, embedding_dim=d_model,
                                                        segment_size=segment_size, method="segment")
            num_tokens = seq_length // segment_size
            conv_k = segment_size
        else:
            raise ValueError(f"Unknown embedding_type: {embedding_type}")
        max_len = num_tokens + (1 if use_cls_token else 0)
        self.positional_encoding = PositionalEncodingRawIQ(d_model=d_model, max_len=max_len, device=device, dropout=0.0)
        if use_cls_token:
            self.cls_token = nn.Parameter(torch.randn(1, 1, d_model))
        self.layers = nn.ModuleList([EncoderLayer(d_model=d_model, ffn_hidden=ffn_hidden, n_head=n_head,
                                                  drop_prob=drop_prob) for _ in range(n_layers)])
        self.dropout = nn.Dropout(p=drop_prob)
        self._geom = dict(kind=1, in_channels=in_channels, img_h=0, img_w=0, patch=0, seq_length=seq_length,
                          conv_k=conv_k, use_cls=1 if use_cls_token else 0, d_model=d_model, n_head=n_head,
                          n_layers=n_layers, ffn_hidden=ffn_hidden, drop_prob=float(drop_prob))
        self._plan: Optional[NativePlan] = None

    def _cfg(self, num_classes=1):
        return N.ModelCfg(num_classes=num_classes, **self._geom)

    def _forward_layers(self, src, src_mask):
        x = self.sequence_embedding(src)
        if self.use_cls_token:
            x = torch.cat([self.cls_token.repeat(x.shape[0], 1, 1), x], dim=1)
        x = self.dropout(self.positional_encoding(x))
        for layer in self.layers:
            x = layer(x, src_mask)
        return x

    def _expect(self, src):
        g = self._geom
        src = _check_src(src, 3, "(batch, in_channels, seq_length)")
        if src.shape[1] != g["in_channels"]:
            raise RuntimeError(f"expected {g['in_channels']} input channels, got {src.shape[1]}")
        n_tok = src.shape[2] // g["conv_k"] + g["use_cls"]
        max_len = self.positional_encoding.encoding.size(0)
        if n_tok > max_len:
            raise ValueError(f"Sequence length {n_tok} exceeds maximum length {max_len}. Increase max_len parameter.")
        if src.shape[2] != g["seq_length"]:
            raise RuntimeError(f"input length {src.shape[2]} does not match seq_length {g['seq_length']} the native "
                               "plan was built for")
        return src

    def forward(self, src, src_mask=None):
        if src_mask is not None:
            return self._forward_layers(src, src_mask)
        src = self._expect(src)
        parent = _parent_of(self)
        if parent is not None:
            return _run(parent.native_plan(), parent, src, "enc", training=self.training)
        if self._plan is None:
            self._plan = NativePlan(self, self._cfg(), prefix_strip="encoder.")
        return _run(self._plan, self, src, "enc")

    def get_cls_token_output(self, src, src_mask=None):
        if not self.use_cls_token:
            raise ValueError("CLS token is not enabled. Set use_cls_token=True")
        return self.forward(src, src_mask)[:, 0, :]

    def get_sequence_output(self, src, src_mask=None):
        x = self.forward(src, src_mask)
        return x[:, 1:, :] if self.use_cls_token else x


class AMCTransformerRawIQ(nn.Module):

    def __init__(self, in_channels, seq_length, num_classes, d_model, n_head, n_layers, ffn_hidden, drop_prob, device,
                 use_cls_token=True, embedding_type="segment", segment_size=64):
        super().__init__()
        self.use_cls_token = use_cls_token
        self.d_model = d_model
        self.encoder = EncoderRawIQ(in_channels=in_channels, seq_length=seq_length, d_model=d_model, n_head=n_head,
                                    ffn_hidden=ffn_hidden, drop_prob=drop_prob, n_layers=n_layers, device=device,
                                    use_cls_token=use_cls_token, embedding_type=embedding_type,
                                    segment_size=segment_size)
        self.mlp_head = nn.Sequential(nn.LayerNorm(d_model), nn.Linear(d_model, num_classes))
        self._num_classes = num_classes
        self._plan: Optional[NativePlan] = None
        _link(self)

    def __setstate__(self, state):
        super().__setstate__(state)
        _link(self)

    def native_plan(self) -> NativePlan:
        if self._plan is None:
            _link(self)
            self._plan = NativePlan(self, self.encoder._cfg(self._num_classes))
        return self._plan

    def forward(self, src):
        src = self.encoder._expect(src)
        return _run(self.native_plan(), self, src, "logits")
```

### vit-vs-raw-iq_amd/trainer.py

```python
from __future__ import annotations

import ctypes as C
import math
from typing import List, Optional, Sequence, Tuple

import torch
import torch.distributed as dist

from . import _native as N
from .modules import NativePlan


def make_buckets(n_layers: int, n_buckets: int) -> List[Tuple[int, int]]:
    stages = list(range(n_layers + 1, -1, -1))
    n_buckets = max(1, min(n_buckets, len(stages)))
    per = math.ceil(len(stages) / n_buckets)
    out = []
    for i in range(0, len(stages), per):
        chunk = stages[i:i + per]
        out.append((chunk[0], chunk[-1]))
    return out


class BucketReducer:

    def __init__(self, group=None):
        self.group = group
        self.pending = []

    @property
    def world(self) -> int:
        return dist.get_world_size(self.group) if dist.is_available() and dist.is_initialized() else 1

    def launch(self, flat: torch.Tensor, off: int, length: int):
        if self.world == 1 or length == 0:
            return
        self.pending.append(dist.all_reduce(flat[off:off + length], op=dist.ReduceOp.SUM, group=self.group,
                                            async_op=True))

    def wait(self):
        for w in self.pending:
            w.wait()
        self.pending = []


def shard_indices(n: int, rank: int, world: int, epoch: int, seed: int = 0) -> torch.Tensor:
    g = torch.Generator().manual_seed(seed * 1_000_003 + epoch)
    perm = torch.randperm(n, generator=g)
    per = math.ceil(n / world)
    total = per * world
    if total > n:
        perm = torch.cat([perm, perm[: total - n]])
    return perm[rank:total:world]


class FusedTrainer:

    def __init__(self, model, lr=1e-4, weight_decay=1e-3, betas=(0.9, 0.99), eps=1e-8, label_smoothing=0.1,
                 max_norm=1.0, device=None, group=None, n_buckets: int = 4, use_graph: bool = False,
                 dropout_seed: Optional[int] = None, sync_params: bool = True):
        self.model = model
        self.device = torch.device(device) if device is not None else next(model.parameters()).device
        if self.device.type != "cuda":
            raise N.IqError("FusedTrainer needs the model on an MI355X (cuda) device; there is no CPU fallback")
        self.plan: NativePlan = model.native_plan()
        self.L = N.lib()
        self.lr, self.wd, self.betas, self.eps = lr, weight_decay, betas, eps
        self.smoothing, self.max_norm = label_smoothing, max_norm
        self.reducer = BucketReducer(group)
        self.world = self.reducer.world
        self.rank = dist.get_rank(group) if self.world > 1 else 0
        if dropout_seed is not None:
            self.plan.seed = int(dropout_seed)
        self.plan.seed = (self.plan.seed + 0x9E3779B97F4A7C15 * self.rank) & ((1 << 63) - 1)
        with torch.cuda.device(self.device):
            self.plan.ensure(self.device)
            if self.world > 1 and sync_params:
                self._sync_parameters()
        n = self.plan.nparam
        d = self.device
        self.gflat = torch.zeros(n, dtype=torch.float32, device=d)
        self.exp_avg = torch.zeros(n, dtype=torch.float32, device=d)
        self.exp_avg_sq = torch.zeros(n, dtype=torch.float32, device=d)
        self.loss_sum = torch.zeros(1, dtype=torch.float32, device=d)
        self.n_correct = torch.zeros(1, dtype=torch.int32, device=d)
        self.gnorm_sq = torch.zeros(1, dtype=torch.float32, device=d)
        self.gn_ws = torch.empty(self.L.iq_gradnorm_ws_bytes(n), dtype=torch.uint8, device=d)
        self.dyn = torch.tensor([lr, 0.0], dtype=torch.float32, device=d)
        self.frames_seen = 0
        self.steps = 0
        self.buckets = make_buckets(self.plan.cfg.n_layers, n_buckets if self.world > 1 else 1)
        self.ranges = [self.plan.grad_range(hi, lo) for hi, lo in self.buckets]
        self.use_graph = bool(use_graph)
        self._slots = {}
        self._slot = None
        self._logits = None
        self._dlogits = None
        self._batch = 0

    def _sync_parameters(self):
        plan, g = self.plan, self.reducer.group
        dist.broadcast(plan.flat, src=dist.get_global_rank(g, 0) if g is not None else 0, group=g)
        plan.mark_dirty()
        plan.ensure(self.device)
        flat = plan.flat.double()
        sig = torch.stack([flat.sum(), flat.abs().sum(), (flat * flat).sum()])
        lo, hi = sig.clone(), sig.clone()
        dist.all_reduce(lo, op=dist.ReduceOp.MIN, group=g)
        dist.all_reduce(hi, op=dist.ReduceOp.MAX, group=g)
        if not torch.equal(lo, hi):
            raise N.IqError(f"rank {self.rank}: parameters differ across ranks after the start-up broadcast "
                            f"(checksums {sig.tolist()} vs min {lo.tolist()} / max {hi.tolist()})")

    def set_lr(self, lr: float):
        self.lr = float(lr)
        self.dyn[0] = self.lr

    MAX_SLOTS = 4

    @property
    def _graphs(self):
        return self._slot["graphs"] if self._slot is not None else None

    @_graphs.setter
    def _graphs(self, value):
        if value is None:
            for sl in self._slots.values():
                sl["graphs"] = None
        elif self._slot is not None:
            self._slot["graphs"] = value

    def _buffers(self, B: int):
        if self._batch != B:
            sl = self._slots.pop(B, None)
            if sl is None:
                K = self.plan.cfg.num_classes
                sl = {"logits": torch.empty(B, K, dtype=torch.float32, device=self.device),
                      "dlogits": torch.empty(B, K, dtype=torch.float32, device=self.device),
                      "static": None, "graphs": None, "captured": None}
                while len(self._slots) >= self.MAX_SLOTS:
                    self._slots.pop(next(iter(self._slots)))
            self._slots[B] = sl
            self._slot = sl
            self._logits, self._dlogits = sl["logits"], sl["dlogits"]
            self._batch = B
        self.plan.workspace(B, self.device)

    def _pointers(self):
        p = self.plan
        return (p.ws.data_ptr(), p.ws.numel(), p.flat.data_ptr(), p.shadow.data_ptr(), p.step_ctr.data_ptr(),
                self._logits.data_ptr(), self._dlogits.data_ptr(), self.gflat.data_ptr(), self._batch)

    def _segments(self, x: torch.Tensor, y: torch.Tensor, auto_step: bool):
        plan, L = self.plan, self.L
        B = x.shape[0]
        ws = plan.ws
        step_arg = 0xFFFFFFFF if auto_step else (self.steps + 1) & 0x7FFFFFFF

        def fwd_and_first_bucket():
            st = N.stream_handle()
            N.check(L.iq_model_forward(plan.h, x.data_ptr(), B, ws.data_ptr(), ws.numel(), 1, plan.seed, step_arg, None,
                                       self._logits.data_ptr(), st), "iq_model_forward", plan.h)
            N.check(L.iq_ce_fwd_bwd(self._logits.data_ptr(), y.data_ptr(), B, plan.cfg.num_classes, self.smoothing,
                                    float(B), self.loss_sum.data_ptr(), self.n_correct.data_ptr(),
                                    self._dlogits.data_ptr(), st), "iq_ce_fwd_bwd")
            bwd(0)()

        def bwd(i):
            hi, lo = self.buckets[i]

            def run():
                N.check(L.iq_model_backward(plan.h, self._dlogits.data_ptr(), None, B, ws.data_ptr(), ws.numel(), 0, hi,
                                            lo, N.stream_handle()), "iq_model_backward", plan.h)
            return run

        def optimizer():
            st = N.stream_handle()
            gscale = 1.0 / self.world
            N.check(L.iq_gradnorm_sq(self.gflat.data_ptr(), plan.nparam, gscale, self.gn_ws.data_ptr(),
                                     self.gnorm_sq.data_ptr(), st), "iq_gradnorm_sq")
            N.check(L.iq_counter_add(None, 0, self.dyn.data_ptr() + 4, 1.0, st), "iq_counter_add")
            N.check(L.iq_adamw_step(plan.flat.data_ptr(), self.gflat.data_ptr(), self.exp_avg.data_ptr(),
                                    self.exp_avg_sq.data_ptr(), plan.shadow.data_ptr(), plan.nparam, self.lr,
                                    self.betas[0], self.betas[1], self.eps, self.wd, 0, self.gnorm_sq.data_ptr(),
                                    self.max_norm, gscale, self.dyn.data_ptr(), st), "iq_adamw_step")
            N.check(L.iq_model_refresh_transposed(plan.h, st), "iq_model_refresh_transposed", plan.h)

        return [fwd_and_first_bucket] + [bwd(i) for i in range(1, len(self.buckets))] + [optimizer]

    def _run_segments(self, runners):
        nb = len(self.buckets)
        for i, run in enumerate(runners):
            if i == nb:
                self.reducer.wait()
            run()
            if i < nb:
                off, ln = self.ranges[i]
                self.reducer.launch(self.gflat, off, ln)

    def step(self, x: torch.Tensor, y: torch.Tensor):
        if not x.is_cuda or not y.is_cuda:
            raise N.IqError("FusedTrainer.step expects device tensors (batch resident in HBM)")
        x = x.contiguous().float()
        y = y.contiguous().long()
        B = x.shape[0]
        plan = self.plan
        if not plan.is_bound(self.device):
            plan.ensure(self.device)
        self._buffers(B)
        if self.gflat is not plan.gflat:
            plan._bind_native(self.gflat)
        plan.generation += 1
        if self.use_graph:
            sl = self._slot
            if sl["graphs"] is not None and sl["captured"] != self._pointers():
                sl["graphs"] = None
            if plan.ctr_value != self.steps:
                plan.step_ctr.fill_(self.steps)
                plan.ctr_value = self.steps
            if sl["graphs"] is None:
                if sl["static"] is None or sl["static"][0].shape != x.shape:
                    sl["static"] = (torch.empty_like(x), torch.empty_like(y))
                static = sl["static"]
                static[0].copy_(x)
                static[1].copy_(y)
                self._run_segments(self._segments(static[0], static[1], auto_step=True))
                torch.cuda.synchronize()
                graphs = []
                for seg in self._segments(static[0], static[1], auto_step=True):
                    g = torch.cuda.CUDAGraph()
                    with torch.cuda.graph(g, capture_error_mode="thread_local"):
                        seg()
                    graphs.append(g)
                sl["graphs"] = graphs
                sl["captured"] = self._pointers()
            else:
                sl["static"][0].copy_(x, non_blocking=True)
                sl["static"][1].copy_(y, non_blocking=True)
                self._run_segments([g.replay for g in sl["graphs"]])
        else:
            self._run_segments(self._segments(x, y, auto_step=False))
        self.steps += 1
        self.frames_seen += B
        plan.step = self.steps
        plan.ctr_value = self.steps

    def read_stats(self, reset=True):
        t = torch.tensor([float(self.loss_sum.item()), float(self.n_correct.item()), float(self.frames_seen)],
                         dtype=torch.float64, device=self.device)
        if self.world > 1:
            dist.all_reduce(t, group=self.reducer.group)
        loss, correct, frames = t.tolist()
        if reset:
            self.loss_sum.zero_()
            self.n_correct.zero_()
            self.frames_seen = 0
        return loss / max(frames, 1.0), correct / max(frames, 1.0), int(frames)

    @torch.no_grad()
    def evaluate(self, x: torch.Tensor, y: torch.Tensor, batch: int = 256):
        was = self.model.training
        self.model.eval()
        K = self.plan.cfg.num_classes
        ls = torch.zeros(1, device=self.device)
        nc = torch.zeros(1, dtype=torch.int32, device=self.device)
        for i in range(0, x.shape[0], batch):
            xb, yb = x[i:i + batch].to(self.device), y[i:i + batch].to(self.device).long()
            logits = self.model(xb)
            N.check(self.L.iq_ce_fwd_bwd(logits.data_ptr(), yb.data_ptr(), xb.shape[0], K, self.smoothing,
                                         float(xb.shape[0]), ls.data_ptr(), nc.data_ptr(), None, N.stream_handle()),
                    "iq_ce_fwd_bwd")
        self.model.train(was)
        t = torch.tensor([ls.item(), float(nc.item()), float(x.shape[0])], dtype=torch.float64, device=self.device)
        if self.world > 1:
            dist.all_reduce(t, group=self.reducer.group)
        loss, correct, frames = t.tolist()
        return loss / frames, correct / frames
```

Before: 51940 frames/s.

## Bind graph inputs via device pointer slot and fold small step kernels

Result: no change. 52230 frames/s, median of 6 (+0.6%).

```diff
diff --git a/include/iqvit.h b/include/iqvit.h
--- a/include/iqvit.h
+++ b/include/iqvit.h
@@ -122,6 +122,10 @@
                 iq_stream_t stream);
 int iq_cls_rows(const float* cls, const float* pe, void* x0, int B, int S, int D, const iq_dropout_t* drop,
                 iq_stream_t stream);
+int iq_embed_front(const float* src, const uint64_t* slot, void* patches, int kind, int B, int C, int H, int W, int p,
+                   int Kpad, const float* cls, const float* pe, void* x0, int S, int D, const iq_dropout_t* drop,
+                   uint32_t* step_ctr, uint32_t step, iq_stream_t stream);
+int iq_inputs_set(uint64_t* slot, const void* x, const void* y, iq_stream_t stream);
 int iq_embed_bwd_gather(const void* dx0, void* demb, float* dcls, int B, int S, int tok, int D, int has_cls,
                         const iq_dropout_t* drop, int accumulate, iq_stream_t stream);
 int iq_embed_dgrad(const void* demb, const void* w_bf16, int Kpad, float* dsrc, int kind, int B, int C, int H, int W, int p,
@@ -133,18 +137,23 @@
                 float* hstat, float* logits, int B, int S, int D, int K, int pool, iq_stream_t stream);
 int iq_ce_fwd_bwd(const float* logits, const int64_t* labels, int B, int K, float smoothing, float denom,
                   float* loss_sum, int32_t* n_correct, float* dlogits, iq_stream_t stream);
+int iq_ce_fwd_bwd_bound(const float* logits, const uint64_t* slot, int B, int K, float smoothing, float denom,
+                        float* loss_sum, int32_t* n_correct, float* dlogits, iq_stream_t stream);
 int iq_head_bwd(const float* dlogits, const float* featn, const float* hstat, const float* ln_g, const float* ln_b,
                 const float* W, float* dW, float* db, float* dln_g, float* dln_b, void* dx, int B, int S, int D, int K,
                 int pool, int accumulate, iq_stream_t stream);
 
 size_t iq_gradnorm_ws_bytes(size_t n);
 int iq_gradnorm_sq(const float* g, size_t n, float grad_scale, float* ws, float* out, iq_stream_t stream);
+int iq_gradnorm_sq_count(const float* g, size_t n, float grad_scale, float* ws, float* out, float* ctr_f32, float inc_f32,
+                         iq_stream_t stream);
 int iq_adamw_step(float* p, const float* g, float* m, float* v, void* shadow_bf16, size_t n, float lr, float beta1,
                   float beta2, float eps, float weight_decay, int step, const float* gnorm_sq, float max_norm,
                   float grad_scale, const float* dyn, iq_stream_t stream);
 int iq_counter_add(uint32_t* ctr_u32, uint32_t inc_u32, float* ctr_f32, float inc_f32, iq_stream_t stream);
 int iq_cast_bf16(const float* src, void* dst, size_t n, iq_stream_t stream);
 int iq_transpose_cast_bf16(const float* src, void* dst, int rows, int cols, iq_stream_t stream);
+int iq_transpose_bf16(const void* src, void* dst, int rows, int cols, iq_stream_t stream);
 
 typedef struct iq_model_cfg {
   int kind;
@@ -168,6 +177,7 @@
 size_t iq_model_workspace_bytes(const iq_model_t* m, int batch, int training);
 int iq_model_bind(iq_model_t* m, float* params, float* grads, const float* pe, void* shadow);
 int iq_model_bind_step_counter(iq_model_t* m, uint32_t* counter);
+int iq_model_bind_inputs(iq_model_t* m, const uint64_t* slot);
 int iq_model_refresh_shadow(iq_model_t* m, iq_stream_t stream);
 int iq_model_refresh_transposed(iq_model_t* m, iq_stream_t stream);
 int iq_model_forward(iq_model_t* m, const float* src, int batch, void* workspace, size_t ws_bytes, int training,
diff --git a/vit-vs-raw-iq_amd/_native.py b/vit-vs-raw-iq_amd/_native.py
--- a/vit-vs-raw-iq_amd/_native.py
+++ b/vit-vs-raw-iq_amd/_native.py
@@ -83,19 +83,24 @@
     "iq_attn_relevance_step": (_I, [_P, _P, _P, _P, _P, _I, _I, _I, _I, _P]),
     "iq_frames_preprocess": (_I, [_P, _P, _I, _I, _I, C.POINTER(C.c_float), _P]),
     "iq_patchify": (_I, [_P, _P, _I, _I, _I, _I, _I, _I, _I, _P]),
+    "iq_embed_front": (_I, [_P, _P, _P, _I, _I, _I, _I, _I, _I, _I, _P, _P, _P, _I, _I, C.POINTER(Dropout), _P, _U32, _P]),
+    "iq_inputs_set": (_I, [_P, _P, _P, _P]),
     "iq_cls_rows": (_I, [_P, _P, _P, _I, _I, _I, C.POINTER(Dropout), _P]),
     "iq_embed_bwd_gather": (_I, [_P, _P, _P, _I, _I, _I, _I, _I, C.POINTER(Dropout), _I, _P]),
     "iq_embed_dgrad": (_I, [_P, _P, _I, _P, _I, _I, _I, _I, _I, _I, _I, _P]),
     "iq_linf_step": (_I, [_P, _P, _P, _F, _F, _F, _F, _Z, _P]),
     "iq_head_fwd": (_I, [_P, _P, _P, _P, _P, _P, _P, _P, _I, _I, _I, _I, _I, _P]),
     "iq_ce_fwd_bwd": (_I, [_P, _P, _I, _I, _F, _F, _P, _P, _P, _P]),
+    "iq_ce_fwd_bwd_bound": (_I, [_P, _P, _I, _I, _F, _F, _P, _P, _P, _P]),
     "iq_head_bwd": (_I, [_P, _P, _P, _P, _P, _P, _P, _P, _P, _P, _P, _I, _I, _I, _I, _I, _I, _P]),
     "iq_gradnorm_ws_bytes": (_Z, [_Z]),
     "iq_gradnorm_sq": (_I, [_P, _Z, _F, _P, _P, _P]),
+    "iq_gradnorm_sq_count": (_I, [_P, _Z, _F, _P, _P, _P, _F, _P]),
     "iq_adamw_step": (_I, [_P, _P, _P, _P, _P, _Z, _F, _F, _F, _F, _F, _I, _P, _F, _F, _P, _P]),
     "iq_counter_add": (_I, [_P, _U32, _P, _F, _P]),
     "iq_cast_bf16": (_I, [_P, _P, _Z, _P]),
     "iq_transpose_cast_bf16": (_I, [_P, _P, _I, _I, _P]),
+    "iq_transpose_bf16": (_I, [_P, _P, _I, _I, _P]),
     "iq_model_create": (_I, [C.POINTER(ModelCfg), C.POINTER(_P)]),
     "iq_model_destroy": (None, [_P]),
     "iq_model_last_error": (C.c_char_p, [_P]),
@@ -107,6 +112,7 @@
     "iq_model_workspace_bytes": (_Z, [_P, _I, _I]),
     "iq_model_bind": (_I, [_P, _P, _P, _P, _P]),
     "iq_model_bind_step_counter": (_I, [_P, _P]),
+    "iq_model_bind_inputs": (_I, [_P, _P]),
     "iq_model_refresh_shadow": (_I, [_P, _P]),
     "iq_model_refresh_transposed": (_I, [_P, _P]),
     "iq_model_forward": (_I, [_P, _P, _I, _P, _Z, _I, _U64, _U32, _P, _P, _P]),
diff --git a/vit-vs-raw-iq_amd/csrc/common.h b/vit-vs-raw-iq_amd/csrc/common.h
--- a/vit-vs-raw-iq_amd/csrc/common.h
+++ b/vit-vs-raw-iq_amd/csrc/common.h
@@ -1,6 +1,7 @@
 #pragma once
 #include <hip/hip_runtime.h>
 #include <stdint.h>
+#include <stdlib.h>
 
 typedef __bf16 bf16;
 typedef __attribute__((ext_vector_type(8))) __bf16 bf16x8;
@@ -16,6 +17,11 @@
 #define IQ_ERR_LAUNCH 3
 
 #define IQ_WAVE 64
+
+static inline int iq_tune_step_tail() {
+  const char* e = getenv("IQ_TUNE_STEP_TAIL");
+  return e ? atoi(e) : 7;
+}
 
 static inline int iq_launch_status() {
   hipError_t e = hipGetLastError();
@@ -90,6 +96,44 @@
   return 65536.0f / (65536.0f - (float)t);
 }
 
+__device__ __forceinline__ void transpose64_tile(const bf16* __restrict__ src, bf16* __restrict__ dst, int rows, int cols, int bx,
+                                                 int by) {
+  __shared__ bf16 t[64][66];
+  const bool vin = (cols % 8) == 0 && ((uintptr_t)src & 15) == 0;
+  const bool vout = (rows % 8) == 0 && ((uintptr_t)dst & 15) == 0;
+  for (int i = threadIdx.x; i < 64 * 8; i += 256) {
+    const int r = i >> 3, c8 = (i & 7) * 8;
+    const int gr = by + r, gc = bx + c8;
+    bf16x8 v;
+    if (vin && gr < rows && gc < cols) {
+      v = *reinterpret_cast<const bf16x8*>(src + (long)gr * cols + gc);
+    } else {
+#pragma unroll
+      for (int e = 0; e < 8; ++e) v[e] = (gr < rows && gc + e < cols) ? src[(long)gr * cols + gc + e] : (bf16)0.f;
+    }
+    const uint32_t* u = reinterpret_cast<const uint32_t*>(&v);
+    uint32_t* d = reinterpret_cast<uint32_t*>(&t[r][c8]);
+#pragma unroll
+    for (int k = 0; k < 4; ++k) d[k] = u[k];
+  }
+  __syncthreads();
+  for (int i = threadIdx.x; i < 64 * 8; i += 256) {
+    const int c = i >> 3, r8 = (i & 7) * 8;
+    const int gc = bx + c, gr = by + r8;
+    if (gc >= cols || gr >= rows) continue;
+    bf16x8 v;
+#pragma unroll
+    for (int e = 0; e < 8; ++e) v[e] = t[r8 + e][c];
+    if (vout) {
+      *reinterpret_cast<bf16x8*>(dst + (long)gc * rows + gr) = v;
+    } else {
+#pragma unroll
+      for (int e = 0; e < 8; ++e)
+        if (gr + e < rows) dst[(long)gc * rows + gr + e] = v[e];
+    }
+  }
+}
+
 __device__ __forceinline__ int xcd_remap(int bid, int nwg) {
   const int NX = 8;
   int q = nwg / NX, r = nwg % NX;
diff --git a/vit-vs-raw-iq_amd/csrc/misc.hip b/vit-vs-raw-iq_amd/csrc/misc.hip
--- a/vit-vs-raw-iq_amd/csrc/misc.hip
+++ b/vit-vs-raw-iq_amd/csrc/misc.hip
@@ -4,10 +4,10 @@
 
 namespace {
 
-__global__ void patchify_kernel(const float* __restrict__ src, bf16* __restrict__ dst, int kind, int B, int C, int H,
-                                int W, int p, int tok, int P, int Kpad) {
+__device__ __forceinline__ void patchify_body(const float* __restrict__ src, bf16* __restrict__ dst, int kind, int B, int C, int H,
+                                              int W, int p, int tok, int P, int Kpad, int bid, int nb) {
   const long nchunk = (long)B * tok * (Kpad / 8);
-  for (long id = (long)blockIdx.x * blockDim.x + threadIdx.x; id < nchunk; id += (long)gridDim.x * blockDim.x) {
+  for (long id = (long)bid * blockDim.x + threadIdx.x; id < nchunk; id += (long)nb * blockDim.x) {
     const int ch = (int)(id % (Kpad / 8));
     const long row = id / (Kpad / 8);
     const int b = (int)(row / tok), t = (int)(row % tok);
@@ -43,12 +43,14 @@
   }
 }
 
-__global__ void cls_rows_kernel(const float* __restrict__ cls, const float* __restrict__ pe, bf16* __restrict__ x0,
-                                int B, int S, int D, int drop_on, IqRng rng, uint32_t thresh, float dscale) {
+__global__ void patchify_kernel(const float* __restrict__ src, bf16* __restrict__ dst, int kind, int B, int C, int H,
+                                int W, int p, int tok, int P, int Kpad) {
+  patchify_body(src, dst, kind, B, C, H, W, p, tok, P, Kpad, blockIdx.x, gridDim.x);
+}
+
+__device__ __forceinline__ void cls_chunk(const float* __restrict__ cls, const float* __restrict__ pe, bf16* __restrict__ x0,
+                                          int id, int S, int D, int drop_on, const IqRng& rng, uint32_t thresh, float dscale) {
   const int nch = D / 8;
-  const int id = blockIdx.x * blockDim.x + threadIdx.x;
-  if (id >= B * nch) return;
-  if (drop_on) rng = rng_resolve(rng);
   const int b = id / nch, ch = id % nch;
   float v[8];
 #pragma unroll
@@ -62,12 +64,62 @@
   *reinterpret_cast<bf16x8*>(x0 + off) = pack8(v);
 }
 
-__global__ void embed_bwd_gather_kernel(const bf16* __restrict__ dx0, bf16* __restrict__ demb, int B, int S, int tok,
-                                        int D, int cls_off, int drop_on, IqRng rng, uint32_t thresh, float dscale) {
+struct FrontTail {
+  const float* cls;
+  const float* pe;
+  bf16* x0;
+  int S, D, drop_on;
+  IqRng rng;
+  uint32_t thresh;
+  float dscale;
+  uint32_t* step_w;
+  uint32_t step_v;
+  int bump;
+};
+__global__ __launch_bounds__(256) void embed_front_kernel(const float* __restrict__ src, const uint64_t* __restrict__ slot,
+                                                          bf16* __restrict__ dst, int kind, int B, int C, int H, int W, int p,
+                                                          int tok, int P, int Kpad, int npb, FrontTail f) {
+  if ((int)blockIdx.x < npb) {
+    if (!src) src = reinterpret_cast<const float*>(slot[0]);
+    patchify_body(src, dst, kind, B, C, H, W, p, tok, P, Kpad, blockIdx.x, npb);
+    return;
+  }
+  __shared__ uint32_t s_step;
+  IqRng rng = f.rng;
+  if (f.step_w) {
+    if (threadIdx.x == 0) {
+      const uint32_t s = f.bump ? *f.step_w + 1u : f.step_v;
+      *f.step_w = s;
+      s_step = s;
+    }
+    __syncthreads();
+    if (rng.step_dev == f.step_w) { rng.step = s_step; rng.step_dev = nullptr; }
+  }
+  if (!f.cls) return;
+  if (f.drop_on) rng = rng_resolve(rng);
+  const int n = B * (f.D / 8);
+  for (int id = threadIdx.x; id < n; id += 256) cls_chunk(f.cls, f.pe, f.x0, id, f.S, f.D, f.drop_on, rng, f.thresh, f.dscale);
+}
+
+__global__ void inputs_set_kernel(uint64_t* slot, uint64_t x, uint64_t y) {
+  if (threadIdx.x == 0 && blockIdx.x == 0) { slot[0] = x; slot[1] = y; }
+}
+
+__global__ void cls_rows_kernel(const float* __restrict__ cls, const float* __restrict__ pe, bf16* __restrict__ x0,
+                                int B, int S, int D, int drop_on, IqRng rng, uint32_t thresh, float dscale) {
+  const int id = blockIdx.x * blockDim.x + threadIdx.x;
+  if (id >= B * (D / 8)) return;
+  if (drop_on) rng = rng_resolve(rng);
+  cls_chunk(cls, pe, x0, id, S, D, drop_on, rng, thresh, dscale);
+}
+
+__device__ __forceinline__ void embed_gather_body(const bf16* __restrict__ dx0, bf16* __restrict__ demb, int B, int S, int tok,
+                                                  int D, int cls_off, int drop_on, IqRng rng, uint32_t thresh, float dscale,
+                                                  int bid, int nb) {
   const int nch = D / 8;
   const long n = (long)B * tok * nch;
   if (drop_on) rng = rng_resolve(rng);
-  for (long id = (long)blockIdx.x * blockDim.x + threadIdx.x; id < n; id += (long)gridDim.x * blockDim.x) {
+  for (long id = (long)bid * blockDim.x + threadIdx.x; id < n; id += (long)nb * blockDim.x) {
     const int ch = (int)(id % nch);
     const long row = id / nch;
     const int b = (int)(row / tok), t = (int)(row % tok);
@@ -85,10 +137,15 @@
   }
 }
 
-__global__ __launch_bounds__(256) void dcls_kernel(const bf16* __restrict__ dx0, float* __restrict__ dcls, int B, int S, int D,
-                                                   int drop_on, IqRng rng, uint32_t thresh, float dscale, int accumulate) {
+__global__ void embed_bwd_gather_kernel(const bf16* __restrict__ dx0, bf16* __restrict__ demb, int B, int S, int tok,
+                                        int D, int cls_off, int drop_on, IqRng rng, uint32_t thresh, float dscale) {
+  embed_gather_body(dx0, demb, B, S, tok, D, cls_off, drop_on, rng, thresh, dscale, blockIdx.x, gridDim.x);
+}
+
+__device__ __forceinline__ void dcls_body(const bf16* __restrict__ dx0, float* __restrict__ dcls, int B, int S, int D, int drop_on,
+                                          IqRng rng, uint32_t thresh, float dscale, int accumulate, int ch) {
   __shared__ float part[4][8];
-  const int ch = blockIdx.x, lane = threadIdx.x & 63, wave = threadIdx.x >> 6;
+  const int lane = threadIdx.x & 63, wave = threadIdx.x >> 6;
   if (drop_on) rng = rng_resolve(rng);
   float s[8] = {0.f, 0.f, 0.f, 0.f, 0.f, 0.f, 0.f, 0.f};
   for (int b = threadIdx.x; b < B; b += 256) {
@@ -111,6 +168,20 @@
     float* dst = dcls + ch * 8 + threadIdx.x;
     *dst = accumulate ? *dst + t : t;
   }
+}
+
+__global__ __launch_bounds__(256) void dcls_kernel(const bf16* __restrict__ dx0, float* __restrict__ dcls, int B, int S, int D,
+                                                   int drop_on, IqRng rng, uint32_t thresh, float dscale, int accumulate) {
+  dcls_body(dx0, dcls, B, S, D, drop_on, rng, thresh, dscale, accumulate, blockIdx.x);
+}
+
+__global__ __launch_bounds__(256) void embed_bwd_gather_dcls_kernel(const bf16* __restrict__ dx0, bf16* __restrict__ demb,
+                                                                    float* __restrict__ dcls, int B, int S, int tok, int D,
+                                                                    int drop_on, IqRng rng, uint32_t thresh, float dscale,
+                                                                    int accumulate, int ngb) {
+  const int ncb = D / 8;
+  if ((int)blockIdx.x < ncb) dcls_body(dx0, dcls, B, S, D, drop_on, rng, thresh, dscale, accumulate, blockIdx.x);
+  else embed_gather_body(dx0, demb, B, S, tok, D, 1, drop_on, rng, thresh, dscale, (int)blockIdx.x - ncb, ngb);
 }
 
 __global__ __launch_bounds__(64) void head_fwd_kernel(const bf16* __restrict__ x, const float* __restrict__ ln_g,
@@ -186,9 +257,10 @@
 
 template <int KMAX>
 __global__ __launch_bounds__(256) void ce_kernel(const float* __restrict__ logits, const int64_t* __restrict__ labels,
-                                                 int B, int K, float smoothing, float denom,
+                                                 const uint64_t* __restrict__ slot, int B, int K, float smoothing, float denom,
                                                  float* __restrict__ loss_sum, int32_t* __restrict__ n_correct,
                                                  float* __restrict__ dlogits) {
+  if (!labels) labels = reinterpret_cast<const int64_t*>(slot[1]);
   __shared__ float sl[256];
   __shared__ int sc[256];
   float lacc = 0.f;
@@ -432,14 +504,18 @@
   __syncthreads();
   if (threadIdx.x == 0) partial[blockIdx.x] = (sm[0] + sm[1] + sm[2] + sm[3]) * scale * scale;
 }
-__global__ __launch_bounds__(256) void gradnorm_final_kernel(const float* __restrict__ partial, int n, float* __restrict__ out) {
+__global__ __launch_bounds__(256) void gradnorm_final_kernel(const float* __restrict__ partial, int n, float* __restrict__ out,
+                                                             float* __restrict__ cf, float incf) {
   __shared__ float sm[4];
   float s = 0.f;
   for (int i = threadIdx.x; i < n; i += 256) s += partial[i];
   s = wave_sum(s);
   if ((threadIdx.x & 63) == 0) sm[threadIdx.x >> 6] = s;
   __syncthreads();
-  if (threadIdx.x == 0) out[0] = sm[0] + sm[1] + sm[2] + sm[3];
+  if (threadIdx.x == 0) {
+    out[0] = sm[0] + sm[1] + sm[2] + sm[3];
+    if (cf) *cf += incf;
+  }
 }
 
 struct AdamParams {
@@ -507,6 +583,10 @@
   if (blockIdx.x == 0 && threadIdx.x < (n & 3)) dst[n4 * 4 + threadIdx.x] = (bf16)src[n4 * 4 + threadIdx.x];
 }
 
+__global__ __launch_bounds__(256) void transpose_bf16_kernel(const bf16* __restrict__ src, bf16* __restrict__ dst, int rows, int cols) {
+  transpose64_tile(src, dst, rows, cols, blockIdx.x * 64, blockIdx.y * 64);
+}
+
 __global__ __launch_bounds__(256) void transpose_cast_kernel(const float* __restrict__ src, bf16* __restrict__ dst,
                                                              int rows, int cols) {
   __shared__ float t[32][33];
@@ -561,6 +641,40 @@
   return iq_launch_status();
 }
 
+extern "C" int iq_embed_front(const float* src, const uint64_t* slot, void* patches, int kind, int B, int C, int H, int W, int p,
+                              int Kpad, const float* cls, const float* pe, void* x0, int S, int D, const iq_dropout_t* drop,
+                              uint32_t* step_ctr, uint32_t step, iq_stream_t stream) {
+  IQ_PROF(IQ_FAM_MISC, stream);
+  if (B <= 0) return IQ_OK;
+  if ((!src && !slot) || !patches || C <= 0 || H <= 0 || p <= 0 || (Kpad % 8)) return IQ_ERR_ARG;
+  if (cls && (!pe || !x0 || D <= 0 || (D % 8) || S <= 0)) return IQ_ERR_ARG;
+  int tok, P;
+  if (kind == 0) {
+    if (W <= 0) return IQ_ERR_ARG;
+    tok = (H / p) * (W / p); P = C * p * p;
+  } else if (kind == 1) {
+    tok = H / p; P = C * p;
+  } else {
+    return IQ_ERR_ARG;
+  }
+  if (tok <= 0 || Kpad < P) return IQ_ERR_ARG;
+  FrontTail f;
+  f.cls = cls; f.pe = pe; f.x0 = (bf16*)x0; f.S = S; f.D = D;
+  fill_rng(drop, &f.drop_on, &f.rng, &f.thresh, &f.dscale);
+  f.step_w = step_ctr; f.step_v = step; f.bump = step == 0xFFFFFFFFu ? 1 : 0;
+  const size_t n = (size_t)B * tok * (Kpad / 8);
+  const int npb = grid_for(n, 256, 4096), extra = (cls || step_ctr) ? 1 : 0;
+  embed_front_kernel<<<npb + extra, 256, 0, (hipStream_t)stream>>>(src, slot, (bf16*)patches, kind, B, C, H, W, p, tok, P, Kpad,
+                                                                   npb, f);
+  return iq_launch_status();
+}
+
+extern "C" int iq_inputs_set(uint64_t* slot, const void* x, const void* y, iq_stream_t stream) {
+  if (!slot || ((uintptr_t)slot & 7)) return IQ_ERR_ARG;
+  inputs_set_kernel<<<1, 64, 0, (hipStream_t)stream>>>(slot, (uint64_t)(uintptr_t)x, (uint64_t)(uintptr_t)y);
+  return iq_launch_status();
+}
+
 extern "C" int iq_cls_rows(const float* cls, const float* pe, void* x0, int B, int S, int D, const iq_dropout_t* drop,
                            iq_stream_t stream) {
   IQ_PROF(IQ_FAM_MISC, stream);
@@ -582,8 +696,13 @@
   fill_rng(drop, &on, &r, &th, &sc);
   const size_t n = (size_t)B * tok * (D / 8);
   hipStream_t st = (hipStream_t)stream;
-  embed_bwd_gather_kernel<<<grid_for(n, 256, 4096), 256, 0, st>>>((const bf16*)dx0, (bf16*)demb, B, S, tok, D,
-                                                                  has_cls ? 1 : 0, on, r, th, sc);
+  const int ngb = grid_for(n, 256, 4096);
+  if (has_cls && (iq_tune_step_tail() & 2)) {
+    embed_bwd_gather_dcls_kernel<<<D / 8 + ngb, 256, 0, st>>>((const bf16*)dx0, (bf16*)demb, dcls, B, S, tok, D, on, r, th, sc,
+                                                              accumulate, ngb);
+    return iq_launch_status();
+  }
+  embed_bwd_gather_kernel<<<ngb, 256, 0, st>>>((const bf16*)dx0, (bf16*)demb, B, S, tok, D, has_cls ? 1 : 0, on, r, th, sc);
   if (has_cls) dcls_kernel<<<D / 8, 256, 0, st>>>((const bf16*)dx0, dcls, B, S, D, on, r, th, sc, accumulate);
   return iq_launch_status();
 }
@@ -598,14 +717,26 @@
   return iq_launch_status();
 }
 
+static int ce_launch(const float* logits, const int64_t* labels, const uint64_t* slot, int B, int K, float smoothing, float denom,
+                     float* loss_sum, int32_t* n_correct, float* dlogits, iq_stream_t stream) {
+  IQ_PROF(IQ_FAM_MISC, stream);
+  if (B <= 0) return IQ_OK;
+  if (!logits || (!labels && !slot) || K <= 0 || denom <= 0.f) return IQ_ERR_ARG;
+  if (K <= 32) ce_kernel<32><<<1, 256, 0, (hipStream_t)stream>>>(logits, labels, slot, B, K, smoothing, denom, loss_sum, n_correct, dlogits);
+  else ce_kernel<0><<<1, 256, 0, (hipStream_t)stream>>>(logits, labels, slot, B, K, smoothing, denom, loss_sum, n_correct, dlogits);
+  return iq_launch_status();
+}
+
 extern "C" int iq_ce_fwd_bwd(const float* logits, const int64_t* labels, int B, int K, float smoothing, float denom,
                              float* loss_sum, int32_t* n_correct, float* dlogits, iq_stream_t stream) {
-  IQ_PROF(IQ_FAM_MISC, stream);
-  if (B <= 0) return IQ_OK;
-  if (!logits || !labels || K <= 0 || denom <= 0.f) return IQ_ERR_ARG;
-  if (K <= 32) ce_kernel<32><<<1, 256, 0, (hipStream_t)stream>>>(logits, labels, B, K, smoothing, denom, loss_sum, n_correct, dlogits);
-  else ce_kernel<0><<<1, 256, 0, (hipStream_t)stream>>>(logits, labels, B, K, smoothing, denom, loss_sum, n_correct, dlogits);
-  return iq_launch_status();
+  if (B > 0 && !labels) return IQ_ERR_ARG;
+  return ce_launch(logits, labels, nullptr, B, K, smoothing, denom, loss_sum, n_correct, dlogits, stream);
+}
+
+extern "C" int iq_ce_fwd_bwd_bound(const float* logits, const uint64_t* slot, int B, int K, float smoothing, float denom,
+                                   float* loss_sum, int32_t* n_correct, float* dlogits, iq_stream_t stream) {
+  if (B > 0 && !slot) return IQ_ERR_ARG;
+  return ce_launch(logits, nullptr, slot, B, K, smoothing, denom, loss_sum, n_correct, dlogits, stream);
 }
 
 extern "C" int iq_head_bwd(const float* dlogits, const float* featn, const float* hstat, const float* ln_g,
@@ -629,12 +760,17 @@
 extern "C" size_t iq_gradnorm_ws_bytes(size_t n) { (void)n; return GN_BLOCKS * sizeof(float); }
 
 extern "C" int iq_gradnorm_sq(const float* g, size_t n, float grad_scale, float* ws, float* out, iq_stream_t stream) {
+  return iq_gradnorm_sq_count(g, n, grad_scale, ws, out, nullptr, 0.f, stream);
+}
+
+extern "C" int iq_gradnorm_sq_count(const float* g, size_t n, float grad_scale, float* ws, float* out, float* ctr_f32,
+                                    float inc_f32, iq_stream_t stream) {
   IQ_PROF(IQ_FAM_OPT, stream);
   if (!g || !ws || !out || ((uintptr_t)g & 15)) return IQ_ERR_ARG;
   hipStream_t st = (hipStream_t)stream;
   const int nb = grid_for(n / 4 + 1, 256 * 4, GN_BLOCKS);
   gradnorm_partial_kernel<<<nb, 256, 0, st>>>(g, n, grad_scale, ws);
-  gradnorm_final_kernel<<<1, 256, 0, st>>>(ws, nb, out);
+  gradnorm_final_kernel<<<1, 256, 0, st>>>(ws, nb, out, ctr_f32, inc_f32);
   return iq_launch_status();
 }
 
@@ -669,6 +805,15 @@
   if (!src || !dst) return IQ_ERR_ARG;
   dim3 grid((cols + 31) / 32, (rows + 31) / 32);
   transpose_cast_kernel<<<grid, 256, 0, (hipStream_t)stream>>>(src, (bf16*)dst, rows, cols);
+  return iq_launch_status();
+}
+
+extern "C" int iq_transpose_bf16(const void* src, void* dst, int rows, int cols, iq_stream_t stream) {
+  IQ_PROF(IQ_FAM_MISC, stream);
+  if (rows <= 0 || cols <= 0) return IQ_OK;
+  if (!src || !dst || (((uintptr_t)src | (uintptr_t)dst) & 1)) return IQ_ERR_ARG;
+  dim3 grid((cols + 63) / 64, (rows + 63) / 64);
+  transpose_bf16_kernel<<<grid, 256, 0, (hipStream_t)stream>>>((const bf16*)src, (bf16*)dst, rows, cols);
   return iq_launch_status();
 }
 
diff --git a/vit-vs-raw-iq_amd/csrc/model.hip b/vit-vs-raw-iq_amd/csrc/model.hip
--- a/vit-vs-raw-iq_amd/csrc/model.hip
+++ b/vit-vs-raw-iq_amd/csrc/model.hip
@@ -77,7 +77,7 @@
     d[i] = add ? d[i] + v : v;
   }
 }
-struct TransDesc { unsigned long long src_off, dst_off; int rows, cols, tile0, tiles_x; };
+struct TransDesc { unsigned long long src_off, dst_off; int rows, cols, tile0, tiles_x, tile0w, tiles_xw; };
 __global__ __launch_bounds__(256) void transpose_table_kernel(const float* __restrict__ params, unsigned char* __restrict__ shadow,
                                                               const TransDesc* __restrict__ tab, int nent) {
   __shared__ float t[32][33];
@@ -100,6 +100,16 @@
   }
 }
 
+__global__ __launch_bounds__(256) void transpose_table64_kernel(const bf16* __restrict__ flat, unsigned char* __restrict__ shadow,
+                                                                const TransDesc* __restrict__ tab, int nent) {
+  int e = 0;
+  while (e + 1 < nent && (int)blockIdx.x >= tab[e + 1].tile0w) ++e;
+  const TransDesc d = tab[e];
+  const int local = blockIdx.x - d.tile0w;
+  transpose64_tile(flat + d.src_off, reinterpret_cast<bf16*>(shadow + d.dst_off), d.rows, d.cols, (local % d.tiles_xw) * 64,
+                   (local / d.tiles_xw) * 64);
+}
+
 __global__ void rel_start_kernel(float* r, int n, int S, int cls) {
   for (int i = blockIdx.x * blockDim.x + threadIdx.x; i < n; i += gridDim.x * blockDim.x) {
     const int k = i % S;
@@ -138,13 +148,14 @@
   size_t hln_g, hln_b, head_w, head_b, head_begin;
   size_t sh_flat, sh_embw, sh_table, shadow_bytes;
   std::vector<TransDesc> ttab;
-  int ttiles = 0;
+  int ttiles = 0, ttiles64 = 0;
   const void* table_uploaded_to = nullptr;
   float* params = nullptr;
   float* grads = nullptr;
   const float* pe = nullptr;
   unsigned char* shadow = nullptr;
   std::string err;
+  const uint64_t* in_slot = nullptr;
   uint32_t* step_ctr = nullptr;
   uint64_t last_seed = 0;
   bool last_tr = false;
@@ -367,6 +378,8 @@
       TransDesc d;
       d.src_off = src; d.dst_off = dst; d.rows = rows; d.cols = cols; d.tile0 = m->ttiles; d.tiles_x = (cols + 31) / 32;
       m->ttiles += d.tiles_x * ((rows + 31) / 32);
+      d.tile0w = m->ttiles64; d.tiles_xw = (cols + 63) / 64;
+      m->ttiles64 += d.tiles_xw * ((rows + 63) / 64);
       m->ttab.push_back(d);
     };
     push(o.wqkv, o.t_wqkv, 3 * D, D);
@@ -425,6 +438,13 @@
   return IQ_OK;
 }
 
+extern "C" int iq_model_bind_inputs(iq_model_t* m, const uint64_t* slot) {
+  if (!m) return IQ_ERR_ARG;
+  if ((uintptr_t)slot & 7) return fail(m, IQ_ERR_ARG, "bind_inputs: slot must be 8 B aligned");
+  m->in_slot = slot;
+  return IQ_OK;
+}
+
 static int refresh_impl(iq_model_t* m, bool cast_flat, iq_stream_t stream) {
   if (!m || !m->params || !m->shadow) return fail(m, IQ_ERR_ARG, "refresh_shadow: model not bound");
   hipStream_t st = (hipStream_t)stream;
@@ -433,7 +453,10 @@
   IQ_PROF(IQ_FAM_MISC, st);
   cast_pad_kernel<<<blocks_for((size_t)D * m->Ppad), 256, 0, st>>>(m->params + m->emb_w, (bf16*)(m->shadow + m->sh_embw), D,
                                                                   m->P, m->Ppad);
-  if (m->ttiles > 0)
+  if (m->ttiles > 0 && (iq_tune_step_tail() & 4))
+    transpose_table64_kernel<<<m->ttiles64, 256, 0, st>>>((const bf16*)(m->shadow + m->sh_flat), m->shadow,
+                                                          (const TransDesc*)(m->shadow + m->sh_table), (int)m->ttab.size());
+  else if (m->ttiles > 0)
     transpose_table_kernel<<<m->ttiles, 256, 0, st>>>(m->params, m->shadow, (const TransDesc*)(m->shadow + m->sh_table),
                                                      (int)m->ttab.size());
   return iq_launch_status();
@@ -447,7 +470,8 @@
                                 iq_stream_t stream) {
   if (!m) return IQ_ERR_ARG;
   if (!m->params || !m->shadow || !m->pe) return fail(m, IQ_ERR_ARG, "forward: model not bound");
-  if (!src || !workspace || batch <= 0) return fail(m, IQ_ERR_ARG, "forward: bad arguments");
+  if (!workspace || batch <= 0) return fail(m, IQ_ERR_ARG, "forward: bad arguments");
+  if (!src && !m->in_slot) return fail(m, IQ_ERR_ARG, "forward: src is NULL and no input slot is bound (iq_model_bind_inputs)");
   if ((uintptr_t)workspace & 255) return fail(m, IQ_ERR_ARG, "forward: workspace must be 256 B aligned");
   const WsPlan w = plan_ws(m, batch);
   if (ws_bytes < w.total) return fail(m, IQ_ERR_ARG, "forward: workspace too small");
@@ -460,17 +484,19 @@
   uint32_t* step_dev = m->step_ctr ? m->step_ctr : (uint32_t*)(ws + w.step_ctr);
   m->last_tr = tr;
   m->last_train_fwd = true;
+  const bool fold = (iq_tune_step_tail() & 1) != 0;
   if (tr) {
-    set_u32_kernel<<<1, 64, 0, st>>>(step_dev, step, step == 0xFFFFFFFFu ? 1 : 0);
+    if (!fold) set_u32_kernel<<<1, 64, 0, st>>>(step_dev, step, step == 0xFFFFFFFFu ? 1 : 0);
     m->last_seed = seed;
   }
   const float* P = m->params;
   m->fwd_ws = nullptr;
 
-  if (c.kind == 0) IQ_TRY(iq_patchify(src, ws + w.patches, 0, B, c.in_channels, c.img_h, c.img_w, c.patch, m->Ppad, stream), "patchify");
-  else IQ_TRY(iq_patchify(src, ws + w.patches, 1, B, c.in_channels, c.seq_length, 0, c.conv_k, m->Ppad, stream), "patchify");
   const iq_dropout_t d0 = site(m, seed, step_dev, 0, tr);
-  if (m->has_cls) IQ_TRY(iq_cls_rows(P + m->cls, m->pe, ws + w.x0, B, S, D, &d0, stream), "cls rows");
+  IQ_TRY(iq_embed_front(src, m->in_slot, ws + w.patches, c.kind, B, c.in_channels, c.kind == 0 ? c.img_h : c.seq_length,
+                        c.kind == 0 ? c.img_w : 0, c.kind == 0 ? c.patch : c.conv_k, m->Ppad, fold && m->has_cls ? P + m->cls : nullptr,
+                        m->pe, ws + w.x0, S, D, &d0, fold && tr ? step_dev : nullptr, step, stream), "patchify (+ step, cls rows)");
+  if (m->has_cls && !fold) IQ_TRY(iq_cls_rows(P + m->cls, m->pe, ws + w.x0, B, S, D, &d0, stream), "cls rows");
   {
     iq_epilogue_t e;
     memset(&e, 0, sizeof(e));
diff --git a/vit-vs-raw-iq_amd/modules.py b/vit-vs-raw-iq_amd/modules.py
--- a/vit-vs-raw-iq_amd/modules.py
+++ b/vit-vs-raw-iq_amd/modules.py
@@ -207,6 +207,7 @@
         self.step = 0
         self.step_ctr: Optional[torch.Tensor] = None
         self.ctr_value = -1
+        self.in_slot: Optional[torch.Tensor] = None
         self._probe = None
 
     def __deepcopy__(self, memo):
@@ -264,6 +265,8 @@
         self.step_ctr = torch.zeros(1, dtype=torch.int32, device=device)
         self.ctr_value = 0
         N.check(self.L.iq_model_bind_step_counter(self.h, N.ptr(self.step_ctr)), "iq_model_bind_step_counter", self.h)
+        self.in_slot = torch.zeros(2, dtype=torch.int64, device=device)
+        N.check(self.L.iq_model_bind_inputs(self.h, N.ptr(self.in_slot)), "iq_model_bind_inputs", self.h)
         self._bind_native(None)
 
     def _bind_native(self, gflat):
diff --git a/vit-vs-raw-iq_amd/trainer.py b/vit-vs-raw-iq_amd/trainer.py
--- a/vit-vs-raw-iq_amd/trainer.py
+++ b/vit-vs-raw-iq_amd/trainer.py
@@ -97,6 +97,7 @@
         self._logits = None
         self._dlogits = None
         self._batch = 0
+        self._held = None
 
     def _sync_parameters(self):
         plan, g = self.plan, self.reducer.group
@@ -137,7 +138,7 @@
                 K = self.plan.cfg.num_classes
                 sl = {"logits": torch.empty(B, K, dtype=torch.float32, device=self.device),
                       "dlogits": torch.empty(B, K, dtype=torch.float32, device=self.device),
-                      "static": None, "graphs": None, "captured": None}
+                      "graphs": None, "captured": None}
                 while len(self._slots) >= self.MAX_SLOTS:
                     self._slots.pop(next(iter(self._slots)))
             self._slots[B] = sl
@@ -149,21 +150,22 @@
     def _pointers(self):
         p = self.plan
         return (p.ws.data_ptr(), p.ws.numel(), p.flat.data_ptr(), p.shadow.data_ptr(), p.step_ctr.data_ptr(),
-                self._logits.data_ptr(), self._dlogits.data_ptr(), self.gflat.data_ptr(), self._batch)
-
-    def _segments(self, x: torch.Tensor, y: torch.Tensor, auto_step: bool):
+                p.in_slot.data_ptr(), self._logits.data_ptr(), self._dlogits.data_ptr(), self.gflat.data_ptr(), self._batch)
+
+    def _segments(self, x: Optional[torch.Tensor], y: Optional[torch.Tensor], B: int, auto_step: bool):
         plan, L = self.plan, self.L
-        B = x.shape[0]
         ws = plan.ws
+        slot = plan.in_slot.data_ptr()
         step_arg = 0xFFFFFFFF if auto_step else (self.steps + 1) & 0x7FFFFFFF
 
         def fwd_and_first_bucket():
             st = N.stream_handle()
-            N.check(L.iq_model_forward(plan.h, x.data_ptr(), B, ws.data_ptr(), ws.numel(), 1, plan.seed, step_arg, None,
+            N.check(L.iq_model_forward(plan.h, N.ptr(x), B, ws.data_ptr(), ws.numel(), 1, plan.seed, step_arg, None,
                                        self._logits.data_ptr(), st), "iq_model_forward", plan.h)
-            N.check(L.iq_ce_fwd_bwd(self._logits.data_ptr(), y.data_ptr(), B, plan.cfg.num_classes, self.smoothing,
-                                    float(B), self.loss_sum.data_ptr(), self.n_correct.data_ptr(),
-                                    self._dlogits.data_ptr(), st), "iq_ce_fwd_bwd")
+            ce = (L.iq_ce_fwd_bwd, y.data_ptr()) if y is not None else (L.iq_ce_fwd_bwd_bound, slot)
+            N.check(ce[0](self._logits.data_ptr(), ce[1], B, plan.cfg.num_classes, self.smoothing,
+                          float(B), self.loss_sum.data_ptr(), self.n_correct.data_ptr(),
+                          self._dlogits.data_ptr(), st), "iq_ce_fwd_bwd")
             bwd(0)()
 
         def bwd(i):
@@ -177,9 +179,8 @@
         def optimizer():
             st = N.stream_handle()
             gscale = 1.0 / self.world
-            N.check(L.iq_gradnorm_sq(self.gflat.data_ptr(), plan.nparam, gscale, self.gn_ws.data_ptr(),
-                                     self.gnorm_sq.data_ptr(), st), "iq_gradnorm_sq")
-            N.check(L.iq_counter_add(None, 0, self.dyn.data_ptr() + 4, 1.0, st), "iq_counter_add")
+            N.check(L.iq_gradnorm_sq_count(self.gflat.data_ptr(), plan.nparam, gscale, self.gn_ws.data_ptr(),
+                                           self.gnorm_sq.data_ptr(), self.dyn.data_ptr() + 4, 1.0, st), "iq_gradnorm_sq_count")
             N.check(L.iq_adamw_step(plan.flat.data_ptr(), self.gflat.data_ptr(), self.exp_avg.data_ptr(),
                                     self.exp_avg_sq.data_ptr(), plan.shadow.data_ptr(), plan.nparam, self.lr,
                                     self.betas[0], self.betas[1], self.eps, self.wd, 0, self.gnorm_sq.data_ptr(),
@@ -218,16 +219,14 @@
             if plan.ctr_value != self.steps:
                 plan.step_ctr.fill_(self.steps)
                 plan.ctr_value = self.steps
+            self._held = (x, y)
+            N.check(self.L.iq_inputs_set(plan.in_slot.data_ptr(), x.data_ptr(), y.data_ptr(), N.stream_handle()),
+                    "iq_inputs_set")
             if sl["graphs"] is None:
-                if sl["static"] is None or sl["static"][0].shape != x.shape:
-                    sl["static"] = (torch.empty_like(x), torch.empty_like(y))
-                static = sl["static"]
-                static[0].copy_(x)
-                static[1].copy_(y)
-                self._run_segments(self._segments(static[0], static[1], auto_step=True))
+                self._run_segments(self._segments(None, None, B, auto_step=True))
                 torch.cuda.synchronize()
                 graphs = []
-                for seg in self._segments(static[0], static[1], auto_step=True):
+                for seg in self._segments(None, None, B, auto_step=True):
                     g = torch.cuda.CUDAGraph()
                     with torch.cuda.graph(g, capture_error_mode="thread_local"):
                         seg()
@@ -235,11 +234,9 @@
                 sl["graphs"] = graphs
                 sl["captured"] = self._pointers()
             else:
-                sl["static"][0].copy_(x, non_blocking=True)
-                sl["static"][1].copy_(y, non_blocking=True)
                 self._run_segments([g.replay for g in sl["graphs"]])
         else:
-            self._run_segments(self._segments(x, y, auto_step=False))
+            self._run_segments(self._segments(x, y, B, auto_step=False))
         self.steps += 1
         self.frames_seen += B
         plan.step = self.steps
```
